# ElijahHyndman/PAPTeam_OpticalFlow

Measured on AMD Instinct MI355X. Metric: Mpix/s per frame-pair (fixed SOR iters) at 1920x1080; max-abs d(u,v) vs ref, higher is better.
Workload: dtype f64

## Files before the change

### papteam_opticalflow_amd/csrc/api.hip

```cpp
#include <algorithm>
#include <chrono>
#include <cmath>
#include <cstdio>
#include <cstdlib>
#include <cstring>
#include <mutex>
#include <random>
#include <thread>

#include "common.h"
#include "flow_internal.h"

namespace papof {

namespace {
thread_local std::string g_last_error;
}

void set_last_error(const char* what, hipError_t e, const char* file, int line) {
    char buf[512];
    std::snprintf(buf, sizeof buf, "%s failed: %s (%s:%d)", what, hipGetErrorString(e), file, line);
    g_last_error = buf;
}
const char* last_error() { return g_last_error.c_str(); }
void set_last_error_text(const std::string& text) { g_last_error = text; }

static double wall() {
    return std::chrono::duration<double>(std::chrono::steady_clock::now().time_since_epoch()).count();
}

size_t arena_bytes_for(int H, int W, int C, int levels, int n_sor_max, double ratio) {
    const size_t np = (size_t)H * W;
    const int fc = (C == 3) ? 5 : (C == 1 ? 3 : C);
    size_t per_level = 0;
    {
        std::vector<Level> L;
        std::vector<PyrPlan> plan;
        if (levels >= 1 && pyramid_plan(H, W, ratio, levels, L, plan) == PAPOF_OK)
            for (const Level& l : L) per_level += ((size_t)l.w * l.h * fc * sizeof(double) + 256) * 3;
    }
    size_t sor_cells = 0, sor_cells_d = 0;
    skew_capacity(H, W, n_sor_max, sor_cells, sor_cells_d);
    size_t planes = 0;
    planes += (size_t)2 * C * 5;
    if (levels > 8) planes += (size_t)2 * C * levels;
    planes += (size_t)2 * C + 2 * C;
    planes += (size_t)7 * fc;
    planes += 8;
    planes += (size_t)3 * C + C;
    planes += (size_t)3 * fc;
    size_t bytes = planes * np * sizeof(double);
    bytes += 3 * (sor_cells + 2 * kLanes) * 16 + (sor_cells_d + 2 * kLanes) * 16 + 10 * np * sizeof(double);
    bytes += per_level + np * fc * sizeof(double);
    bytes += 8 * (std::min<size_t>(kTinyMaxCells, np) * sizeof(double) + 256);
    bytes += (size_t)64 * 4096;
    return bytes;
}

static size_t sor_scratch_bytes(int H, int W, int n_sor) {
    size_t cells = 0, cells_d = 0;
    skew_capacity(H, W, n_sor, cells, cells_d);
    return 4 * (cells + 128) * 16 + (cells_d + 128) * 16;
}

int ensure_arena(papof_handle* h, size_t bytes) {
    if (bytes <= h->arena.cap) return PAPOF_OK;
    PAPOF_HIP(hipStreamSynchronize(h->stream));
    if (h->arena.base) PAPOF_HIP(hipFree(h->arena.base));
    h->arena.base = nullptr;
    h->arena.cap = 0;
    void* p = nullptr;
    hipError_t e = hipMalloc(&p, bytes);
    if (e != hipSuccess) {
        set_last_error("hipMalloc(arena)", e, __FILE__, __LINE__);
        return PAPOF_ENOMEM;
    }
    h->arena.base = static_cast<char*>(p);
    h->arena.cap = bytes;
    return PAPOF_OK;
}

int check_params(const papof_params& P, int levels) {
    if (levels < 1) return PAPOF_EINVAL;
    if (P.n_inner < 1) return PAPOF_EINVAL;
    if (P.n_outer + 0 < 1 || P.n_sor < 1 || P.n_outer_per_level < 0 || P.n_sor_per_level < 0) return PAPOF_EINVAL;
    if (P.sor_mode < PAPOF_SOR_EXACT || P.sor_mode > PAPOF_SOR_JACOBI) return PAPOF_EINVAL;
    if (!(P.alpha > 0) || !(P.omega > 0)) return PAPOF_EINVAL;
    if (P.interpolation != PAPOF_INTERP_BILINEAR && P.interpolation != PAPOF_INTERP_BICUBIC) return PAPOF_EINVAL;
    if (P.noise_model != PAPOF_NOISE_LAPLACIAN && P.noise_model != PAPOF_NOISE_GMIXTURE) return PAPOF_EINVAL;
    return PAPOF_OK;
}

int pyramid_plan(int H, int W, double ratio, int nlev, std::vector<Level>& L, std::vector<PyrPlan>& plan) {
    if (ratio > 0.98 || ratio < 0.4) ratio = 0.75;
    const double base_sigma = 1 / ratio - 1;
    const int n = (int)(std::log(0.25) / std::log(ratio));
    const double n_sigma = base_sigma * n;
    L.assign(nlev, Level{});
    plan.assign(nlev, PyrPlan{});
    L[0].w = W;
    L[0].h = H;
    for (int i = 1; i < nlev; i++) {
        PyrPlan p;
        if (i <= n) {
            p.src_level = 0;
            p.sigma = base_sigma * i;
            p.fsize = (int)(p.sigma * 3);
            p.rate = std::pow(ratio, i);
        } else {
            p.src_level = i - n;
            p.sigma = n_sigma;
            p.fsize = (int)(n_sigma * 3);
            p.rate = (double)std::pow(ratio, i) * W / L[i - n].w;
        }
        p.sw = L[p.src_level].w;
        p.sh = L[p.src_level].h;
        if (p.fsize > kMaxFsize) return PAPOF_EINVAL;
        L[i].w = (int)((double)p.sw * p.rate);
        L[i].h = (int)((double)p.sh * p.rate);
        if (L[i].w < 1 || L[i].h < 1) return PAPOF_EINVAL;
        plan[i] = p;
    }
    return PAPOF_OK;
}

int smooth_and_resize(papof_handle* h, const double* src, double* dst, double* tmp_a, double* tmp_b, const PyrPlan& p, int C,
                      int dh, int dw) {
    const Taps g = gaussian_taps(p.sigma, p.fsize);
    if (g.fsize == 0 && g.t[0] == 1.0) return resize(h, src, dst, p.sh, p.sw, C, dh, dw, p.rate, p.rate, false, 0.0);
    PAPOF_TRY(filter_hv(h, src, tmp_b, tmp_a, p.sh, p.sw, C, g, g));
    return resize(h, tmp_b, dst, p.sh, p.sw, C, dh, dw, p.rate, p.rate, false, 0.0);
}

int reduce_init(papof_handle* h, const papof_tensor* a, const papof_tensor* b, int pairs_a, int pairs_b, int H, int W,
                const std::vector<Level>& L, const std::vector<PyrPlan>& plan, double ratio, double* X, double* Y, double* T,
                size_t t_planes, double*& out) {
    const size_t np0 = (size_t)H * W;
    const int planes = 2 * (pairs_a + pairs_b), levels = (int)L.size();
    double* const parts[2] = {X, X + (size_t)pairs_a * 2 * np0};
    const papof_tensor* const src[2] = {a, b};
    const int n[2] = {pairs_a, pairs_b};
    for (int i = 0; i < 2; i++) {
        if (n[i] == 0) continue;
        if (src[i])
            PAPOF_TRY(ingest_frames(h, *src[i], nullptr, parts[i], H, W, 2, n[i]));
        else
            PAPOF_HIP(hipMemsetAsync(parts[i], 0, (size_t)n[i] * 2 * np0 * sizeof(double), h->stream));
    }
    PAPOF_TRY(init_sanitize(h, X, (size_t)planes * np0));
    out = X;
    if (levels == 1) return PAPOF_OK;
    std::vector<int> chain;
    for (int i = levels - 1; i > 0; i = plan[i].src_level) chain.insert(chain.begin(), i);
    double s = 1.0;
    for (int i = 1; i < levels; i++) s *= ratio;
    double *cur = X, *other = Y;
    for (const int i : chain) {
        const PyrPlan& p = plan[i];
        const bool last = i == levels - 1;
        const Taps g = gaussian_taps(p.sigma, p.fsize);
        if (g.fsize == 0 && g.t[0] == 1.0) {
            PAPOF_TRY(resize(h, cur, other, p.sh, p.sw, planes, L[i].h, L[i].w, p.rate, p.rate, last, last ? s : 0.0));
            std::swap(cur, other);
            continue;
        }
        const size_t ns = (size_t)p.sw * p.sh;
        const int chunk = filter_hv_needs_tmp(g, g) ? (int)std::min<size_t>((size_t)planes, t_planes * np0 / ns) : planes;
        if (chunk < 1) return PAPOF_EINVAL;
        for (int c0 = 0; c0 < planes; c0 += chunk)
            PAPOF_TRY(filter_hv(h, cur + c0 * ns, other + c0 * ns, T, p.sh, p.sw, std::min(chunk, planes - c0), g, g));
        PAPOF_TRY(resize(h, other, cur, p.sh, p.sw, planes, L[i].h, L[i].w, p.rate, p.rate, last, last ? s : 0.0));
    }
    out = cur;
    return PAPOF_OK;
}

int build_pyramid(papof_handle* h, const std::vector<Level>& L, const std::vector<PyrPlan>& plan, int C, bool second,
                  double* tmp_a, double* tmp_b) {
    for (size_t i = 1; i < L.size(); i++) {
        const PyrPlan& p = plan[i];
        const double* src = second ? L[p.src_level].p2 : L[p.src_level].p1;
        double* dst = second ? L[i].p2 : L[i].p1;
        PAPOF_TRY(smooth_and_resize(h, src, dst, tmp_a, tmp_b, p, C, L[i].h, L[i].w));
    }
    return PAPOF_OK;
}

struct SolveBuffers {
    double *im1s, *tmp, *blend, *imdt, *phi;
    SorPlanes sp;
    SorPlanes sp_tiny{};
    double *bgx = nullptr, *bgy = nullptr, *bgxy = nullptr;
    double *gm = nullptr, *gm_scratch = nullptr;
};

int alloc_solve_buffers(Arena& A, int H, int W, int fc, int mode, int n_sor_cap, SolveBuffers& B) {
    const size_t np = (size_t)H * W;
    B.im1s = A.f64(np * fc);
    B.tmp = A.f64(np * fc);
    B.blend = A.f64(np * fc);
    B.imdt = A.f64(np * fc);
    B.phi = A.f64(np);
    PAPOF_TRY(sor_alloc_planes(A, H, W, mode, n_sor_cap, B.sp));
    if (mode == PAPOF_SOR_EXACT)
        PAPOF_TRY(sor_alloc_tiny_planes(A, std::min<size_t>(kTinyMaxCells, (size_t)H * W), B.sp_tiny));
    return A.overflow ? PAPOF_ENOMEM : PAPOF_OK;
}

int alloc_branch_buffers(papof_handle* h, Arena& A, int H, int W, int fc, int interpolation, int noise_model,
                         SolveBuffers& B) {
    const size_t np = (size_t)H * W;
    if (interpolation == PAPOF_INTERP_BICUBIC) {
        B.bgx = A.f64(np * fc);
        B.bgy = A.f64(np * fc);
        B.bgxy = A.f64(np * fc);
    }
    if (noise_model == PAPOF_NOISE_GMIXTURE) {
        B.gm = A.f64(5 * 8);
        B.gm_scratch = A.f64((size_t)gm_scratch_doubles());
        if (A.overflow || fc > 8) return fc > 8 ? PAPOF_EINVAL : PAPOF_ENOMEM;
        double init[40];
        for (int k = 0; k < fc; k++) {
            init[k] = 0.95;
            init[fc + k] = 0.05;
            init[2 * fc + k] = 0.5;
            init[3 * fc + k] = 0.05 * 0.05;
            init[4 * fc + k] = 0.5 * 0.5;
        }
        PAPOF_HIP(hipMemcpyAsync(B.gm, init, sizeof(double) * 5 * fc, hipMemcpyHostToDevice, h->stream));
        PAPOF_HIP(hipStreamSynchronize(h->stream));
    }
    return A.overflow ? PAPOF_ENOMEM : PAPOF_OK;
}

int bicubic_planes(papof_handle* h, const double* f2, int H, int W, int fc, SolveBuffers& B) {
    PAPOF_TRY(central3_planes(h, f2, B.bgx, B.bgy, B.bgxy, H, W, fc));
    return PAPOF_OK;
}

struct LapGuard {
    bool on = false;
    bool exact = false;
    bool collect = false;
    bool nz_known = false;
    unsigned* flags = nullptr;
    double* lap = nullptr;
    double* scratch = nullptr;
    unsigned epoch = 0;
    int slot = 0;
    std::vector<int> slot_level, slot_channels;
    unsigned* wit(int s) const { return on && collect && s >= 0 && s < kLapMaxSlots ? flags + lap_wit_word(s) : nullptr; }
    unsigned* nz(int level) const { return on && collect && nz_known ? flags + lap_nz_word(level) : nullptr; }
    const double* guard() const { return on && exact ? lap : nullptr; }
    int unknown(const unsigned* host_flags) const {
        if (!on || !collect) return 0;
        if (slot > kLapMaxSlots) return 1;
        int n = 0;
        for (int s = 0; s + 1 < slot; s++)
            for (int c = 0; c < slot_channels[s]; c++) {
                const unsigned w = host_flags[lap_wit_word(s) + c];
                const bool witness = w == epoch || w == (epoch ^ kLapNone);
                const bool all_zero = nz_known && host_flags[lap_nz_word(slot_level[s]) + c] != epoch;
                n += !(witness || all_zero);
                if (!(witness || all_zero) && std::getenv("PAPOF_LAP_TRACE"))
                    std::fprintf(stderr, "[lap guard] no proof: slot %d of %d, level %d, channel %d\n", s, slot, slot_level[s], c);
            }
        return n;
    }
};

int smooth_flow(papof_handle* h, const double* f1, const double* f2, double* warp, double*& u, double*& v, double*& ua,
                double*& va, int H, int W, int fc, double alpha, int n_outer, int n_inner, int n_sor, double omega,
                int mode, SolveBuffers& B, PhaseClock& clk, const double* im1s_ready = nullptr,
                bool final_warp = true, unsigned* prog = nullptr, size_t prog_per_solve = 0, double* out_u = nullptr,
                double* out_v = nullptr, bool fold_warp = false, LapGuard* lg = nullptr, int level = 0) {
    const Taps g = smooth5_taps();
    int solve_idx = 0;
    const bool tiny = mode == PAPOF_SOR_EXACT && B.sp_tiny.phi && (size_t)H * W <= kTinyMaxCells && sor_tiny_fits(h, H, W, n_sor);
    SorPlanes& SP = tiny ? B.sp_tiny : B.sp;
    const double* im1s = im1s_ready;
    if (!im1s) {
        clk.phase(PAPOF_T_PHASE1_GENERATE);
        PAPOF_TRY(filter_hv(h, f1, B.im1s, B.tmp, H, W, fc, g, g));
        im1s = B.im1s;
    }
    const char* const fused_sw = std::getenv("PAPOF_FUSED_SYSTEM");
    const bool fused_env = !(fused_sw && fused_sw[0] == '0');
    const bool fused_system = fused_env && fold_warp && n_inner == 1 && !B.gm && (fc == 5 || fc == 3) &&
                              !(lg && lg->guard()) && !(lg && lg->on && lap_one_block_level(H, W));
    for (int count = 0; count < n_outer; count++) {
        clk.phase(fused_system ? kTimerFused : (int)PAPOF_T_PHASE1_GENERATE);
        if (fused_system)
            PAPOF_TRY(flow_system(h, f1, f2, u, v, im1s, H, W, fc, alpha, omega, SP,
                                  lg && count > 0 ? lg->wit(lg->slot - 1) : nullptr));
        else if (fold_warp)
            PAPOF_TRY(warp_smooth_blend(h, f1, f2, u, v, im1s, B.blend, B.imdt, H, W, fc,
                                        lg && count > 0 && !B.gm ? lg->wit(lg->slot - 1) : nullptr,
                                        B.phi));
        else
            PAPOF_TRY(smooth_hv_blend(h, warp, im1s, B.blend, B.imdt, H, W, fc));
        for (int hh = 0; hh < n_inner; hh++) {
            const SorPlanes* prev = hh == 0 ? nullptr : &SP;
            if ((count == 0 && !fold_warp) || hh > 0) {
                clk.phase(PAPOF_T_PHASE2_DERIVATIVES);
                PAPOF_TRY(compute_phi(h, u, v, prev, B.phi, H, W));
            }
            if (!fused_system) clk.phase(PAPOF_T_PHASE4_LINEARSYSTEM);
            if (!fused_system)
                PAPOF_TRY(assemble_system(h, B.blend, B.imdt, B.phi, u, v, H, W, fc, alpha, omega, SP, nullptr, nullptr,
                                          prev, nullptr, B.gm, lg ? lg->guard() : nullptr));
            h->sor_mark = [](void* c, int on) {
                static_cast<PhaseClock*>(c)->phase(on ? PAPOF_T_PHASE5_SOR : PAPOF_T_PHASE6_UPDATE);
            };
            h->sor_mark_ctx = &clk;
            h->sor_prog_next = prog ? prog + (size_t)solve_idx * prog_per_solve : nullptr;
            solve_idx++;
            const int rc_solve = sor_solve(h, SP, H, W, alpha, omega, n_sor, mode);
            h->sor_prog_next = nullptr;
            h->sor_mark = nullptr;
            h->sor_mark_ctx = nullptr;
            PAPOF_TRY(rc_solve);
        }
        double* const phi_next = count + 1 < n_outer && !fold_warp ? B.phi : nullptr;
        const bool rewarp = !fold_warp && !B.bgx && (final_warp || count + 1 < n_outer || B.gm);
        const bool wit_later = fold_warp && count + 1 < n_outer;
        const bool wit_small = fold_warp && !wit_later && lap_one_block_level(H, W);
        unsigned* const wit = lg && !B.gm && !B.bgx && !wit_later && !wit_small ? lg->wit(lg->slot) : nullptr;
        if (out_u && out_v && count + 1 == n_outer) {
            PAPOF_TRY(update_warp_phi(h, SP, u, v, out_u, out_v, f1, f2, warp, phi_next, H, W, fc, rewarp, 0, -1, wit));
            u = out_u;
            v = out_v;
        } else {
            PAPOF_TRY(update_warp_phi(h, SP, u, v, ua, va, f1, f2, warp, phi_next, H, W, fc, rewarp, 0, -1, wit));
            std::swap(u, ua);
            std::swap(v, va);
        }
        if (B.bgx)
            PAPOF_TRY(bicubic_warp(h, f1, f2, B.bgx, B.bgy, B.bgxy, u, v, warp, H, W, fc, nullptr, true, true));
        if (lg && lg->on && !B.gm && wit_small && lg->wit(lg->slot))
            PAPOF_TRY(lap_small_check(h, f1, f2, u, v, H, W, fc, lg->wit(lg->slot)));
        if (lg && lg->on && !B.gm) {
            lg->slot_level.push_back(level);
            lg->slot_channels.push_back(fc);
            lg->slot++;
            if (lg->exact) {
                if (B.bgx)
                    PAPOF_TRY(est_laplacian_noise(h, f1, warp, nullptr, nullptr, H, W, fc, lg->lap, lg->scratch));
                else
                    PAPOF_TRY(est_laplacian_noise(h, f1, f2, u, v, H, W, fc, lg->lap, lg->scratch));
            }
        }
        if (B.gm) PAPOF_TRY(est_gaussian_mixture(h, f1, warp, H, W, fc, B.gm, B.gm_scratch));
    }
    clk.phase(-1);
    return PAPOF_OK;
}

int feature_channels(int C) { return C == 3 ? 5 : (C == 1 ? 3 : C); }

struct FrameIn {
    const void* d;
    bool u8;
    bool planar = false;
};
int load_frame(papof_handle* h, const FrameIn& f, double* planar, int H, int W, int C) {
    if (f.planar) {
        PAPOF_HIP(hipMemcpyAsync(planar, f.d, (size_t)H * W * C * sizeof(double), hipMemcpyDeviceToDevice, h->stream));
        return PAPOF_OK;
    }
    if (f.u8) return hwc_u8_to_planar(h, static_cast<const unsigned char*>(f.d), planar, H, W, C);
    return hwc_to_planar(h, static_cast<const double*>(f.d), planar, H, W, C);
}

enum SeqOp { kPair, kSeqPrime, kSeqNext };

bool seq_matches(const papof_handle* h, int H, int W, int C, int levels, double ratio, size_t need) {
    const papof_handle::Seq& q = h->seq;
    return q.valid && q.h == H && q.w == W && q.c == C && q.levels == levels && q.ratio == ratio &&
           q.arena_base == h->arena.base && need <= h->arena.cap;
}

int flow_pass(papof_handle* h, const FrameIn& fa, const FrameIn& fb, SeqOp op, int H, int W, int C, int levels,
              const papof_params& P, double* d_vx, double* d_vy, double* d_warp, double* timing, LapGuard* lg,
              const papof_tensor* init = nullptr) {
    const double t_entry = wall();
    PAPOF_TRY(check_params(P, levels));
    double ratio = P.ratio;
    if (ratio > 0.98 || ratio < 0.4) ratio = 0.75;
    std::vector<Level> L;
    std::vector<PyrPlan> plan;
    PAPOF_TRY(pyramid_plan(H, W, P.ratio, levels, L, plan));
    const int n_sor_max = P.n_sor + (levels - 1) * P.n_sor_per_level;
    const size_t need = arena_bytes_for(H, W, C, levels, n_sor_max, P.ratio);
    if (op == kSeqNext && !seq_matches(h, H, W, C, levels, ratio, need)) {
        g_last_error = "sequence push does not continue the primed sequence (shape, levels, ratio or arena changed)";
        return PAPOF_EINVAL;
    }
    const int slot1 = op == kSeqNext ? h->seq.slot : 0;
    h->seq.valid = false;
    PAPOF_TRY(ensure_arena(h, need));
    Arena& A = h->arena;
    A.off = 0;
    A.overflow = false;
    h->events_used = 0;
    const size_t np0 = (size_t)H * W;
    const int fc = feature_channels(C);
    double tm[PAPOF_N_TIMERS + 1];
    std::memset(tm, 0, sizeof tm);
    const size_t tm_bytes = PAPOF_N_TIMERS * sizeof(double);
    const auto keep_seq = [&](int slot) {
        h->seq.valid = true;
        h->seq.h = H;
        h->seq.w = W;
        h->seq.c = C;
        h->seq.levels = levels;
        h->seq.ratio = ratio;
        h->seq.slot = slot;
        h->seq.arena_base = A.base;
    };
    PhaseClock clk{h, true};
    PhaseClock pclk{h, true};
    PhaseClock total{h, true};
    clk.only_sor = pclk.only_sor = (!h->phase_events && P.phase_timing == 0) || P.phase_timing == 2;
    h->sor_launches = 0;
    h->sor_log.clear();
    clk.stamps = true;
    h->stamps_used = 0;
    h->next_stamp = nullptr;
    h->stamp_stream = h->stream;

    total.phase(PAPOF_T_TOTAL);
    for (int i = 0; i < levels; i++) {
        double* slot[2];
        slot[0] = A.f64((size_t)L[i].w * L[i].h * C);
        slot[1] = A.f64((size_t)L[i].w * L[i].h * C);
        L[i].p1 = slot[slot1];
        L[i].p2 = slot[slot1 ^ 1];
    }
    double* tmp_a = A.f64(np0 * C);
    double* tmp_b = A.f64(np0 * C);
    if (A.overflow) return PAPOF_ENOMEM;
    if (op == kSeqPrime) {
        PAPOF_TRY(load_frame(h, fa, L[0].p1, H, W, C));
        PAPOF_TRY(build_pyramid(h, L, plan, C, false, tmp_a, tmp_b));
        PAPOF_HIP(hipStreamSynchronize(h->stream));
        keep_seq(slot1);
        if (timing) std::memset(timing, 0, tm_bytes);
        return PAPOF_OK;
    }

    std::vector<double*> F1(levels), F2(levels), S1(levels);
    for (int k = 0; k < levels; k++) {
        const size_t n = (size_t)L[k].w * L[k].h * fc;
        F1[k] = A.f64(n);
        F2[k] = A.f64(n);
        S1[k] = A.f64(n);
    }
    double* prep_tmp = A.f64(np0 * fc);
    double* gx = A.f64(np0 * C);
    double* gy = A.f64(np0 * C);
    double* gxy = A.f64(np0 * C);
    double* warp = A.f64(np0 * fc);
    double* u = A.f64(2 * np0);
    double* v = u ? u + np0 : nullptr;
    double* u2 = A.f64(2 * np0);
    double* v2 = u2 ? u2 + np0 : nullptr;
    SolveBuffers B;
    {
        const int rc_alloc = alloc_solve_buffers(A, H, W, fc, P.sor_mode, n_sor_max, B);
        if (rc_alloc != PAPOF_OK || A.overflow) return rc_alloc != PAPOF_OK ? rc_alloc : PAPOF_ENOMEM;
    }
    PAPOF_TRY(alloc_branch_buffers(h, A, H, W, fc, P.interpolation, P.noise_model, B));

    struct LevelCounters {
        size_t prog_off = 0, prog_per = 0;
    };
    std::vector<LevelCounters> LP(levels);
    size_t prog_total = 0;
    const bool exact = P.sor_mode == PAPOF_SOR_EXACT;
    if (exact) {
        for (int k = 0; k < levels; k++) {
            LP[k].prog_per = sor_counters_words(L[k].h, L[k].w, P.n_sor + k * P.n_sor_per_level);
            LP[k].prog_off = prog_total;
            prog_total += LP[k].prog_per * (size_t)((P.n_outer + k * P.n_outer_per_level) * P.n_inner);
        }
        PAPOF_TRY(sor_counters_ensure(h, prog_total));
    }

    const bool overlap = h->overlap_prep && P.phase_timing != 1 && h->prep_stream != nullptr;
    hipStream_t const main_stream = h->stream, prep = overlap ? h->prep_stream : h->stream;
    while (h->sync_events.size() < (size_t)levels + 2) {
        hipEvent_t e;
        PAPOF_HIP(hipEventCreateWithFlags(&e, hipEventDisableTiming));
        h->sync_events.push_back(e);
    }
    struct StreamSwap {
        papof_handle* h;
        hipStream_t saved;
        StreamSwap(papof_handle* hh, hipStream_t s) : h(hh), saved(hh->stream) { h->stream = s; }
        ~StreamSwap() { h->stream = saved; }
    };
    bool from_level0 = true;
    for (int i = 1; i < levels; i++) from_level0 = from_level0 && plan[i].src_level == 0;
    const Taps g5 = smooth5_taps();
    const auto build_level = [&](int i, int second) -> int {
        if (i == 0) return PAPOF_OK;
        const PyrPlan& q = plan[i];
        const double* src = second ? L[q.src_level].p2 : L[q.src_level].p1;
        double* dst = second ? L[i].p2 : L[i].p1;
        return smooth_and_resize(h, src, dst, tmp_a, tmp_b, q, C, L[i].h, L[i].w);
    };
    const auto prepare = [&]() -> int {
        StreamSwap on_prep(h, prep);
        pclk.phase(PAPOF_T_ALLOCATION);
        if (exact && !sor_counters_clear(h, 0, prog_total)) return PAPOF_EDEVICE;
        pclk.phase(PAPOF_T_CONSTRUCTION);
        if (op != kSeqNext) PAPOF_TRY(load_frame(h, fa, L[0].p1, H, W, C));
        PAPOF_TRY(load_frame(h, fb, L[0].p2, H, W, C));
        const int first = op == kSeqNext ? 1 : 0;
        if (!from_level0)
            for (int i = 1; i < levels; i++)
                for (int second = first; second < 2; second++) PAPOF_TRY(build_level(i, second));
        for (int k = levels - 1; k >= 0; k--) {
            if (from_level0) {
                pclk.phase(PAPOF_T_CONSTRUCTION);
                for (int second = first; second < 2; second++) PAPOF_TRY(build_level(k, second));
            }
            pclk.phase(PAPOF_T_ALLOCATION);
            PAPOF_TRY(im2feature(h, L[k].p1, F1[k], L[k].h, L[k].w, C, lg ? lg->nz(k) : nullptr));
            PAPOF_TRY(im2feature(h, L[k].p2, F2[k], L[k].h, L[k].w, C, lg ? lg->nz(k) : nullptr));
            pclk.phase(PAPOF_T_PHASE1_GENERATE);
            PAPOF_TRY(filter_hv(h, F1[k], S1[k], prep_tmp, L[k].h, L[k].w, fc, g5, g5));
            pclk.phase(-1);
            if (overlap) PAPOF_HIP(hipEventRecord(h->sync_events[k], prep));
        }
        pclk.phase(PAPOF_T_POSTPROCESSING);
        PAPOF_TRY(central3_planes(h, L[0].p2, gx, gy, gxy, H, W, C));
        pclk.phase(-1);
        if (overlap) PAPOF_HIP(hipEventRecord(h->sync_events[levels], prep));
        return PAPOF_OK;
    };
    papof_handle::HostIO& io = h->hostio;
    const bool hostio = io.active && overlap && h->copy_stream && h->copy_events.size() >= 8;
    const auto prepare_hostio = [&]() -> int {
        StreamSwap on_prep(h, prep);
        hipStream_t const cs = h->copy_stream;
        pclk.phase(PAPOF_T_ALLOCATION);
        if (exact && !sor_counters_clear(h, 0, prog_total)) return PAPOF_EDEVICE;
        if (io.im1) {
            PAPOF_HIP(hipMemcpyAsync(const_cast<void*>(fa.d), io.im1, io.nb_in, hipMemcpyHostToDevice, cs));
            PAPOF_HIP(hipEventRecord(h->copy_events[0], cs));
            PAPOF_HIP(hipStreamWaitEvent(prep, h->copy_events[0], 0));
        }
        pclk.phase(PAPOF_T_CONSTRUCTION);
        if (op != kSeqNext) {
            PAPOF_TRY(load_frame(h, fa, L[0].p1, H, W, C));
            for (int i = 1; i < levels; i++) PAPOF_TRY(build_level(i, 0));
        }
        for (int k = levels - 1; k >= 0; k--) {
            pclk.phase(PAPOF_T_ALLOCATION);
            PAPOF_TRY(im2feature(h, L[k].p1, F1[k], L[k].h, L[k].w, C, lg ? lg->nz(k) : nullptr));
            pclk.phase(PAPOF_T_PHASE1_GENERATE);
            PAPOF_TRY(filter_hv(h, F1[k], S1[k], prep_tmp, L[k].h, L[k].w, fc, g5, g5));
        }
        pclk.phase(-1);
        if (io.im2) {
            PAPOF_HIP(hipMemcpyAsync(const_cast<void*>(fb.d), io.im2, io.nb_in, hipMemcpyHostToDevice, cs));
            PAPOF_HIP(hipEventRecord(h->copy_events[1], cs));
            PAPOF_HIP(hipStreamWaitEvent(prep, h->copy_events[1], 0));
        }
        pclk.phase(PAPOF_T_CONSTRUCTION);
        PAPOF_TRY(load_frame(h, fb, L[0].p2, H, W, C));
        if (!from_level0)
            for (int i = 1; i < levels; i++) PAPOF_TRY(build_level(i, 1));
        for (int k = levels - 1; k >= 0; k--) {
            if (from_level0) {
                pclk.phase(PAPOF_T_CONSTRUCTION);
                PAPOF_TRY(build_level(k, 1));
            }
            pclk.phase(PAPOF_T_ALLOCATION);
            PAPOF_TRY(im2feature(h, L[k].p2, F2[k], L[k].h, L[k].w, C, lg ? lg->nz(k) : nullptr));
            pclk.phase(-1);
            PAPOF_HIP(hipEventRecord(h->sync_events[k], prep));
        }
        pclk.phase(PAPOF_T_POSTPROCESSING);
        PAPOF_TRY(central3_planes(h, L[0].p2, gx, gy, gxy, H, W, C));
        pclk.phase(-1);
        PAPOF_HIP(hipEventRecord(h->sync_events[levels], prep));
        return PAPOF_OK;
    };
    if (io.active && !hostio) {
        if (io.im1) PAPOF_HIP(hipMemcpyAsync(const_cast<void*>(fa.d), io.im1, io.nb_in, hipMemcpyHostToDevice, main_stream));
        if (io.im2) PAPOF_HIP(hipMemcpyAsync(const_cast<void*>(fb.d), io.im2, io.nb_in, hipMemcpyHostToDevice, main_stream));
    }
    if (overlap) {
        PAPOF_HIP(hipEventRecord(h->sync_events[levels + 1], main_stream));
        PAPOF_HIP(hipStreamWaitEvent(prep, h->sync_events[levels + 1], 0));
    }
    {
        const int rc = hostio ? prepare_hostio() : prepare();
        if (rc != PAPOF_OK) {
            if (overlap) hipStreamSynchronize(prep);
            return rc;
        }
    }

    int pw = 0, ph = 0;
    const auto solve_levels = [&]() -> int {
        if (lg && lg->guard())
            PAPOF_HIP(hipMemcpyAsync(lg->lap, h->lap_init_dev, 8 * sizeof(double), hipMemcpyDeviceToDevice, main_stream));
        for (int k = levels - 1; k >= 0; k--) {
            const int lw = L[k].w, lh = L[k].h;
            const size_t np = (size_t)lw * lh;
            clk.phase(-1);
            if (overlap) PAPOF_HIP(hipStreamWaitEvent(main_stream, h->sync_events[k], 0));
            clk.phase(PAPOF_T_ALLOCATION);
            const double *f1 = F1[k], *f2 = F2[k];
            const int n_sor_k = P.n_sor + k * P.n_sor_per_level, n_outer_k = P.n_outer + k * P.n_outer_per_level;
            unsigned* prog_k = nullptr;
            if (exact) prog_k = h->sync_words + 32 + LP[k].prog_off;
            const bool tiny_k = exact && (size_t)lw * lh <= kTinyMaxCells && sor_tiny_fits(h, lh, lw, n_sor_k);
            if (!tiny_k) PAPOF_TRY(sor_bind(h, B.sp, lh, lw, n_sor_k));
            double* const out_u = k == 0 ? d_vx : nullptr;
            double* const out_v = k == 0 ? d_vy : nullptr;
            const bool fold_warp = !B.bgx && !B.gm;
            if (k == levels - 1 && init) {
                double* r = nullptr;
                PAPOF_TRY(reduce_init(h, init, nullptr, 1, 0, H, W, L, plan, ratio, u, u2, warp, (size_t)fc, r));
                if (r != u) std::swap(u, u2);
                v = u + np;
                v2 = u2 + np;
                if (B.bgx) {
                    PAPOF_TRY(bicubic_planes(h, f2, lh, lw, fc, B));
                    PAPOF_TRY(bicubic_warp(h, f1, f2, B.bgx, B.bgy, B.bgxy, u, v, warp, lh, lw, fc, nullptr, true, false));
                } else if (!fold_warp) {
                    PAPOF_TRY(warp_bilinear(h, f1, f2, u, v, warp, lh, lw, fc));
                }
            } else if (k == levels - 1) {
                v = u + np;
                v2 = u2 + np;
                PAPOF_HIP(hipMemsetAsync(u, 0, 2 * np * sizeof(double), h->stream));
                if (!fold_warp)
                    PAPOF_HIP(hipMemcpyAsync(warp, f2, np * fc * sizeof(double), hipMemcpyDeviceToDevice, h->stream));
                if (B.bgx) PAPOF_TRY(bicubic_planes(h, f2, lh, lw, fc, B));
            } else {
                const double xr = (double)lw / pw, yr = (double)lh / ph, inv = 1 / ratio;
                PAPOF_TRY(resize(h, u, u2, ph, pw, 2, lh, lw, xr, yr, true, inv));
                std::swap(u, u2);
                v = u + np;
                v2 = u2 + np;
                if (B.bgx) {
                    PAPOF_TRY(bicubic_planes(h, f2, lh, lw, fc, B));
                    PAPOF_TRY(bicubic_warp(h, f1, f2, B.bgx, B.bgy, B.bgxy, u, v, warp, lh, lw, fc, nullptr, true, false));
                } else if (!fold_warp) {
                    PAPOF_TRY(warp_bilinear(h, f1, f2, u, v, warp, lh, lw, fc));
                }
            }
            if (!tiny_k) PAPOF_TRY(sor_reset_planes(h, B.sp));
            PAPOF_TRY(smooth_flow(h, f1, f2, warp, u, v, u2, v2, lh, lw, fc, P.alpha, n_outer_k, P.n_inner, n_sor_k, P.omega,
                                  P.sor_mode, B, clk, S1[k], false, prog_k, exact ? LP[k].prog_per : 0, out_u, out_v,
                                  fold_warp, lg, k));
            pw = lw;
            ph = lh;
        }
        clk.phase(-1);
        if (overlap) PAPOF_HIP(hipStreamWaitEvent(main_stream, h->sync_events[levels], 0));
        clk.phase(PAPOF_T_POSTPROCESSING);
        if (hostio && io.early_out && u == d_vx && v == d_vy) {
            hipStream_t const cs = h->copy_stream;
            PAPOF_HIP(hipEventRecord(h->copy_events[2], main_stream));
            PAPOF_HIP(hipStreamWaitEvent(cs, h->copy_events[2], 0));
            PAPOF_HIP(hipMemcpyAsync(io.vx, d_vx, io.nb_flow, hipMemcpyDeviceToHost, cs));
            PAPOF_HIP(hipMemcpyAsync(io.vy, d_vy, io.nb_flow, hipMemcpyDeviceToHost, cs));
            constexpr int kChunks = 4;
            for (int q = 0; q < kChunks; q++) {
                const Rect rc{0, (int)((long long)H * q / kChunks), W, (int)((long long)H * (q + 1) / kChunks)};
                if (rc.empty()) continue;
                PAPOF_TRY(bicubic_warp(h, L[0].p1, L[0].p2, gx, gy, gxy, u, v, d_warp, H, W, C, &rc));
                PAPOF_HIP(hipEventRecord(h->copy_events[3 + q], main_stream));
                PAPOF_HIP(hipStreamWaitEvent(cs, h->copy_events[3 + q], 0));
                const size_t off = (size_t)rc.y0 * W * C, cnt = (size_t)rc.h() * W * C;
                PAPOF_HIP(hipMemcpyAsync(io.warp + off, d_warp + off, cnt * sizeof(double), hipMemcpyDeviceToHost, cs));
            }
            io.out_issued = true;
            return PAPOF_OK;
        }
        PAPOF_TRY(bicubic_warp(h, L[0].p1, L[0].p2, gx, gy, gxy, u, v, d_warp, H, W, C));
        if (u != d_vx) PAPOF_HIP(hipMemcpyAsync(d_vx, u, np0 * sizeof(double), hipMemcpyDeviceToDevice, h->stream));
        if (v != d_vy) PAPOF_HIP(hipMemcpyAsync(d_vy, v, np0 * sizeof(double), hipMemcpyDeviceToDevice, h->stream));
        return PAPOF_OK;
    };
    const int rc_main = solve_levels();
    if (rc_main != PAPOF_OK) {
        hipStreamSynchronize(main_stream);
        if (overlap) hipStreamSynchronize(prep);
        return rc_main;
    }
    clk.phase(-1);
    PAPOF_TRY(stamp_only(h));
    total.phase(-1);
    h->stamps_fetched = 0;
    {
        const bool flags = lg && lg->on && lg->collect;
        const size_t first = flags ? lap_wit_word(std::min(lg->slot, kLapMaxSlots) - 1) : kLapFlagWords;
        const size_t bytes = (kLapFlagWords - first) * sizeof(unsigned) + (size_t)h->stamps_used * sizeof(unsigned long long);
        if (bytes > 0)
            PAPOF_HIP(hipMemcpyAsync(h->lap_flags_host + first, h->lap_flags_dev + first, bytes, hipMemcpyDeviceToHost, h->stream));
        h->stamps_fetched = h->stamps_used;
    }
    const double t_enqueued = wall();
    PAPOF_HIP(hipStreamSynchronize(h->stream));
    h->host_enqueue_sec = t_enqueued - t_entry;
    h->host_wait_sec = wall() - t_enqueued;
    h->next_stamp = nullptr;
    if (P.sor_mode == PAPOF_SOR_EXACT) PAPOF_TRY(sor_check(h));
    if (clk.err != PAPOF_OK || pclk.err != PAPOF_OK || total.err != PAPOF_OK) return PAPOF_EDEVICE;
    clk.collect(tm);
    pclk.collect(tm);
    total.collect(tm);
    if (clk.sor_span_sec.size() == h->sor_log.size())
        for (size_t i = 0; i < h->sor_log.size(); i++) h->sor_log[i].sec = clk.sor_span_sec[i];
    {
        constexpr double kPsiShare = 0.3;
        const double fused = tm[PAPOF_T_PHASE4_LINEARSYSTEM];
        tm[PAPOF_T_PHASE3_PSIDATA] += kPsiShare * fused;
        tm[PAPOF_T_PHASE4_LINEARSYSTEM] = fused - kPsiShare * fused;
    }
    {
        constexpr double kPhiShare = 0.04;
        const double fused = tm[PAPOF_T_PHASE1_GENERATE];
        tm[PAPOF_T_PHASE2_DERIVATIVES] += kPhiShare * fused;
        tm[PAPOF_T_PHASE1_GENERATE] = fused - kPhiShare * fused;
    }
    {
        const double f = tm[kTimerFused];
        tm[PAPOF_T_PHASE1_GENERATE] += 0.51 * f;
        tm[PAPOF_T_PHASE2_DERIVATIVES] += 0.02 * f;
        tm[PAPOF_T_PHASE3_PSIDATA] += 0.14 * f;
        tm[PAPOF_T_PHASE4_LINEARSYSTEM] += f - 0.51 * f - 0.02 * f - 0.14 * f;
    }
    if (timing) std::memcpy(timing, tm, tm_bytes);
    if (op == kSeqNext) keep_seq(slot1 ^ 1);
    return PAPOF_OK;
}

int flow_device(papof_handle* h, const FrameIn& fa, const FrameIn& fb, SeqOp op, int H, int W, int C, int levels,
                const papof_params& P, double* d_vx, double* d_vy, double* d_warp, double* timing,
                const papof_tensor* init = nullptr) {
    LapGuard lg;
    const int fc = feature_channels(C);
    lg.on = h->lap_guard && op != kSeqPrime && P.noise_model == PAPOF_NOISE_LAPLACIAN && fc <= 8 && levels >= 1 &&
            h->lap_flags_dev != nullptr;
    if (!lg.on) return flow_pass(h, fa, fb, op, H, W, C, levels, P, d_vx, d_vy, d_warp, timing, nullptr, init);
    lg.flags = h->lap_flags_dev;
    lg.lap = h->lap_dev;
    lg.scratch = h->lap_scratch_dev;
    lg.nz_known = (C == 1 || C == 3) && (size_t)levels * 8 <= (size_t)kLapNzWords;
    const bool always_exact = P.interpolation == PAPOF_INTERP_BICUBIC;
    lg.collect = !always_exact;
    lg.exact = always_exact || h->lap_exact;
    const papof_handle::Seq seq0 = h->seq;
    double first_pass_total = 0.0;
    for (int pass = 0; pass < 2; pass++) {
        if (++h->lap_epoch >= kLapNone) {
            PAPOF_HIP(hipMemsetAsync(h->lap_flags_dev, 0, kLapFlagWords * sizeof(unsigned), h->stream));
            h->lap_epoch = 1u;
        }
        lg.epoch = h->lap_epoch;
        lg.slot = 0;
        lg.slot_level.clear();
        lg.slot_channels.clear();
        PAPOF_TRY(flow_pass(h, fa, fb, op, H, W, C, levels, P, d_vx, d_vy, d_warp, timing, &lg, init));
        if (pass == 1 && timing) timing[PAPOF_T_TOTAL] += first_pass_total;
        if (!lg.collect) return PAPOF_OK;
        const int unknown = lg.unknown(h->lap_flags_host);
        if (lg.exact) {
            if (pass == 0) h->lap_exact_calls++;
            h->lap_exact = unknown > 0;
            return PAPOF_OK;
        }
        if (unknown == 0) return PAPOF_OK;
        h->lap_reruns++;
        lg.exact = true;
        if (timing) first_pass_total = timing[PAPOF_T_TOTAL];
        if (h->copy_stream) PAPOF_HIP(hipStreamSynchronize(h->copy_stream));
        h->seq = seq0;
        h->hostio.im1 = nullptr;
        h->hostio.im2 = nullptr;
    }
    return PAPOF_OK;
}

int flow_device_planar(papof_handle* h, const double* f1, const double* f2, int H, int W, int C, int levels,
                       const papof_params& P, double* d_vx, double* d_vy, double* d_warp, double* timing,
                       const papof_tensor* init) {
    FrameIn a{f1, false}, b{f2, false};
    a.planar = b.planar = true;
    return flow_device(h, a, b, kPair, H, W, C, levels, P, d_vx, d_vy, d_warp, timing, init);
}

}

using namespace papof;

extern "C" {

int papof_version(void) { return PAPOF_VERSION; }

void papof_default_params(papof_params* p) {
    if (!p) return;
    p->alpha = 0.012;
    p->ratio = 0.75;
    p->n_outer = 7;
    p->n_outer_per_level = 1;
    p->n_inner = 1;
    p->n_sor = 30;
    p->n_sor_per_level = 3;
    p->omega = 1.8;
    p->sor_mode = PAPOF_SOR_EXACT;
    p->phase_timing = 0;
    p->interpolation = PAPOF_INTERP_BILINEAR;
    p->noise_model = PAPOF_NOISE_LAPLACIAN;
}

const char* papof_strerror(int code) {
    switch (code) {
        case PAPOF_OK: return "ok";
        case PAPOF_EINVAL: return "invalid argument";
        case PAPOF_ENODEVICE: return "no usable gfx950 device";
        case PAPOF_ENOMEM: return "out of memory";
        case PAPOF_EDEVICE: return "HIP runtime error";
        case PAPOF_ETIMEOUT: return "device-side wait timed out";
    }
    return "unknown error";
}

const char* papof_last_error(void) { return last_error(); }

const char* papof_timing_key(int i) {
    static const char* keys[PAPOF_N_TIMERS] = {"Allocation",         "Construction",        "Phase1_Generate",
                                               "Phase2_Derivatives", "Phase3_PsiData",      "Phase4_LinearSystem",
                                               "Phase5_SOR",         "Phase6_Update",       "PostProcessing",
                                               "Total C++ Execution"};
    return (i >= 0 && i < PAPOF_N_TIMERS) ? keys[i] : "";
}
// ... 637 lines not shown
    PAPOF_TRY(S.down_planar(sp.b1, rhs1, height, width, 1));
    return S.down_planar(sp.b2, rhs2, height, width, 1);
}

int papof_stage_laplacian(papof_handle* h, const double* in, const double* weight, int height, int width,
                          double* out) {
    if (!h || !in || !weight || !out || height < 1 || width < 1) return PAPOF_EINVAL;
    Scope S(h, img_bytes(height, width, 1, 6));
    PAPOF_TRY(S.rc);
    double* a = S.up_planar(in, height, width, 1);
    double* w = S.up_planar(weight, height, width, 1);
    double* o = S.dev((size_t)height * width);
    PAPOF_TRY(S.rc);
    PAPOF_TRY(laplacian(h, a, w, o, height, width));
    return S.down_planar(o, out, height, width, 1);
}

namespace {
int alloc_sor_planes(Scope& S, int H, int W, int mode, int n_sor, SorPlanes& sp) {
    if (mode == PAPOF_SOR_EXACT && (size_t)H * W <= kTinyMaxCells && sor_tiny_fits(S.h, H, W, n_sor)) {
        const int rc_t = sor_alloc_tiny_planes(S.h->arena, (size_t)H * W, sp);
        if (rc_t != PAPOF_OK) S.rc = rc_t;
        return S.rc;
    }
    int rc = sor_alloc_planes(S.h->arena, H, W, mode, n_sor, sp);
    if (rc == PAPOF_OK) rc = sor_bind(S.h, sp, H, W, n_sor);
    if (rc != PAPOF_OK) S.rc = rc;
    return S.rc;
}
}

int papof_stage_sor(papof_handle* h, const double* phi, const double* imdxy, const double* imdx2,
                    const double* imdy2, const double* rhs1, const double* rhs2, int height, int width,
                    double alpha, double omega, int n_sor, int sor_mode, double* du, double* dv) {
    if (!h || !phi || !imdxy || !imdx2 || !imdy2 || !rhs1 || !rhs2 || !du || !dv || height < 1 || width < 1 ||
        n_sor < 1 || sor_mode < PAPOF_SOR_EXACT || sor_mode > PAPOF_SOR_JACOBI)
        return PAPOF_EINVAL;
    const size_t np = (size_t)height * width;
    Scope S(h, img_bytes(height, width, 1, 16) + sor_scratch_bytes(height, width, n_sor) +
                   12 * (size_t)height * width * sizeof(double));
    PAPOF_TRY(S.rc);
    double* p = S.up_planar(phi, height, width, 1);
    double* xy = S.up_planar(imdxy, height, width, 1);
    double* x2 = S.up_planar(imdx2, height, width, 1);
    double* y2 = S.up_planar(imdy2, height, width, 1);
    double* r1 = S.up_planar(rhs1, height, width, 1);
    double* r2 = S.up_planar(rhs2, height, width, 1);
    double *ou = S.dev(np), *ov = S.dev(np);
    SorPlanes sp{};
    PAPOF_TRY(alloc_sor_planes(S, height, width, sor_mode, n_sor, sp));
    PAPOF_TRY(sor_reset_planes(h, sp));
    PAPOF_TRY(sor_prep(h, p, xy, x2, y2, r1, r2, height, width, alpha, omega, sp));
    PAPOF_TRY(sor_solve(h, sp, height, width, alpha, omega, n_sor, sor_mode));
    PAPOF_TRY(sor_unpack(h, sp, ou, ov, height, width));
    PAPOF_TRY(S.down_planar(ou, du, height, width, 1));
    PAPOF_TRY(S.down_planar(ov, dv, height, width, 1));
    if (sor_mode == PAPOF_SOR_EXACT) PAPOF_TRY(sor_check(h));
    return PAPOF_OK;
}

int papof_stage_smoothflow(papof_handle* h, const double* im1, const double* im2, double* warp, double* u,
                           double* v, int height, int width, int c, double alpha, int n_outer, int n_inner,
                           int n_sor, double omega, int sor_mode) {
    return papof_stage_smoothflow_ex(h, im1, im2, warp, u, v, height, width, c, alpha, n_outer, n_inner, n_sor, omega,
                                     sor_mode, PAPOF_INTERP_BILINEAR, PAPOF_NOISE_LAPLACIAN, nullptr);
}

int papof_stage_smoothflow_ex(papof_handle* h, const double* im1, const double* im2, double* warp, double* u,
                              double* v, int height, int width, int c, double alpha, int n_outer, int n_inner,
                              int n_sor, double omega, int sor_mode, int interpolation, int noise_model, double* gm) {
    if (!h || !im1 || !im2 || !warp || !u || !v || height < 1 || width < 1 || c < 1 || n_outer < 1 || n_sor < 1 ||
        sor_mode < PAPOF_SOR_EXACT || sor_mode > PAPOF_SOR_JACOBI)
        return PAPOF_EINVAL;
    if (n_inner < 1) return PAPOF_EINVAL;
    if (interpolation < 0 || interpolation > 1 || noise_model < 0 || noise_model > 1) return PAPOF_EINVAL;
    Scope S(h, img_bytes(height, width, c, 16) + img_bytes(height, width, 1, 8) +
                   sor_scratch_bytes(height, width, n_sor) +
                   12 * (size_t)height * width * sizeof(double) + (1 << 20));
    PAPOF_TRY(S.rc);
    double* f1 = S.up_planar(im1, height, width, c);
    double* f2 = S.up_planar(im2, height, width, c);
    double* w = S.up_planar(warp, height, width, c);
    double* du = S.up_planar(u, height, width, 1);
    double* dv = S.up_planar(v, height, width, 1);
    double* du_alt = S.dev((size_t)height * width);
    double* dv_alt = S.dev((size_t)height * width);
    PAPOF_TRY(S.rc);
    SolveBuffers B;
    PAPOF_TRY(alloc_solve_buffers(h->arena, height, width, c, sor_mode, n_sor, B));
    PAPOF_TRY(alloc_branch_buffers(h, h->arena, height, width, c, interpolation, noise_model, B));
    if (B.gm && gm) PAPOF_HIP(hipMemcpyAsync(B.gm, gm, sizeof(double) * 5 * c, hipMemcpyHostToDevice, h->stream));
    if (B.bgx) PAPOF_TRY(bicubic_planes(h, f2, height, width, c, B));
    PAPOF_TRY(sor_bind(h, B.sp, height, width, n_sor));
    PAPOF_TRY(sor_reset_planes(h, B.sp));
    PhaseClock clk{h, false};
    LapGuard lg;
    lg.on = h->lap_guard && noise_model == PAPOF_NOISE_LAPLACIAN && c <= 8 && h->lap_dev != nullptr;
    lg.exact = true;
    lg.lap = h->lap_dev;
    lg.scratch = h->lap_scratch_dev;
    if (lg.on) PAPOF_HIP(hipMemcpyAsync(lg.lap, h->lap_init_dev, 8 * sizeof(double), hipMemcpyDeviceToDevice, h->stream));
    PAPOF_TRY(smooth_flow(h, f1, f2, w, du, dv, du_alt, dv_alt, height, width, c, alpha, n_outer, n_inner, n_sor, omega,
                          sor_mode, B, clk, nullptr, true, nullptr, 0, nullptr, nullptr, false, &lg, 0));
    PAPOF_TRY(S.down_planar(w, warp, height, width, c));
    PAPOF_TRY(S.down_planar(du, u, height, width, 1));
    PAPOF_TRY(S.down_planar(dv, v, height, width, 1));
    if (B.gm && gm) {
        PAPOF_HIP(hipMemcpyAsync(gm, B.gm, sizeof(double) * 5 * c, hipMemcpyDeviceToHost, h->stream));
        PAPOF_HIP(hipStreamSynchronize(h->stream));
    }
    if (sor_mode == PAPOF_SOR_EXACT) PAPOF_TRY(sor_check(h));
    return PAPOF_OK;
}

int papof_stage_est_gaussian_mixture(papof_handle* h, const double* im1, const double* im2, int height, int width,
                                     int c, double* gm) {
    if (!h || !im1 || !im2 || !gm || height < 1 || width < 1 || c < 1 || c > 8) return PAPOF_EINVAL;
    Scope S(h, img_bytes(height, width, c, 6) + (1 << 20));
    PAPOF_TRY(S.rc);
    double* a = S.up_planar(im1, height, width, c);
    double* b = S.up_planar(im2, height, width, c);
    double* g = S.dev(40);
    double* scratch = S.dev((size_t)gm_scratch_doubles());
    PAPOF_TRY(S.rc);
    PAPOF_HIP(hipMemcpyAsync(g, gm, sizeof(double) * 5 * c, hipMemcpyHostToDevice, h->stream));
    PAPOF_TRY(est_gaussian_mixture(h, a, b, height, width, c, g, scratch));
    PAPOF_HIP(hipMemcpyAsync(gm, g, sizeof(double) * 5 * c, hipMemcpyDeviceToHost, h->stream));
    PAPOF_HIP(hipStreamSynchronize(h->stream));
    return PAPOF_OK;
}

int papof_pyramid_levels_for_min_width(int width, double ratio, int min_width, int* levels) {
    if (width < 1 || min_width < 1 || !levels) return PAPOF_EINVAL;
    if (ratio > 0.98 || ratio < 0.4) ratio = 0.75;
    *levels = (int)(std::log((double)min_width / width) / std::log(ratio));
    return PAPOF_OK;
}

int papof_stage_bicubic_warp(papof_handle* h, const double* im1, const double* im2, const double* vx,
                             const double* vy, int height, int width, int c, double* out) {
    return papof_stage_bicubic_warp_ex(h, im1, im2, vx, vy, height, width, c, 1, out);
}

int papof_stage_bicubic_warp_ex(papof_handle* h, const double* im1, const double* im2, const double* vx,
                                const double* vy, int height, int width, int c, int clamp, double* out) {
    if (!h || !im1 || !im2 || !vx || !vy || !out || height < 1 || width < 1 || c < 1) return PAPOF_EINVAL;
    Scope S(h, img_bytes(height, width, c, 10) + img_bytes(height, width, 1, 4));
    PAPOF_TRY(S.rc);
    const size_t n = (size_t)height * width * c;
    double* a = S.up_planar(im1, height, width, c);
    double* b = S.up_planar(im2, height, width, c);
    double* fx = S.up_planar(vx, height, width, 1);
    double* fy = S.up_planar(vy, height, width, 1);
    double *gx = S.dev(n), *gy = S.dev(n), *gxy = S.dev(n), *o = S.dev(n);
    PAPOF_TRY(S.rc);
    PAPOF_TRY(central3_planes(h, b, gx, gy, gxy, height, width, c));
    PAPOF_TRY(bicubic_warp(h, a, b, gx, gy, gxy, fx, fy, o, height, width, c, nullptr, false, clamp != 0));
    PAPOF_HIP(hipMemcpyAsync(out, o, n * sizeof(double), hipMemcpyDeviceToHost, h->stream));
    PAPOF_HIP(hipStreamSynchronize(h->stream));
    return PAPOF_OK;
}

int papof_flow_quantize16(papof_handle* h, const double* vx, const double* vy, int height, int width,
                          unsigned short* out) {
    if (!h || !vx || !vy || !out || height < 1 || width < 1) return PAPOF_EINVAL;
    const size_t n = (size_t)height * width;
    Scope S(h, n * (2 * sizeof(double) + 2 * sizeof(unsigned short)) + 4096);
    PAPOF_TRY(S.rc);
    double* a = S.up_planar(vx, height, width, 1);
    double* b = S.up_planar(vy, height, width, 1);
    unsigned short* q = reinterpret_cast<unsigned short*>(S.dev((n * 2 * sizeof(unsigned short) + 7) / 8));
    PAPOF_TRY(S.rc);
    PAPOF_TRY(flow_quantize16(h, a, b, q, n));
    PAPOF_HIP(hipMemcpyAsync(out, q, n * 2 * sizeof(unsigned short), hipMemcpyDeviceToHost, h->stream));
    PAPOF_HIP(hipStreamSynchronize(h->stream));
    return PAPOF_OK;
}

int papof_flow_dequantize16(papof_handle* h, const unsigned short* q, int height, int width, double* vx,
                            double* vy) {
    if (!h || !q || !vx || !vy || height < 1 || width < 1) return PAPOF_EINVAL;
    const size_t n = (size_t)height * width;
    Scope S(h, n * (2 * sizeof(double) + 2 * sizeof(unsigned short)) + 4096);
    PAPOF_TRY(S.rc);
    unsigned short* dq = reinterpret_cast<unsigned short*>(S.dev((n * 2 * sizeof(unsigned short) + 7) / 8));
    double* a = S.dev(n);
    double* b = S.dev(n);
    PAPOF_TRY(S.rc);
    PAPOF_HIP(hipMemcpyAsync(dq, q, n * 2 * sizeof(unsigned short), hipMemcpyHostToDevice, h->stream));
    PAPOF_TRY(flow_dequantize16(h, dq, a, b, n));
    PAPOF_HIP(hipMemcpyAsync(vx, a, n * sizeof(double), hipMemcpyDeviceToHost, h->stream));
    PAPOF_HIP(hipMemcpyAsync(vy, b, n * sizeof(double), hipMemcpyDeviceToHost, h->stream));
    PAPOF_HIP(hipStreamSynchronize(h->stream));
    return PAPOF_OK;
}

int papof_flow_to_bgr(papof_handle* h, const double* vx, const double* vy, int height, int width,
                      unsigned char* bgr) {
    if (!h || !vx || !vy || !bgr || height < 1 || width < 1) return PAPOF_EINVAL;
    const size_t n = (size_t)height * width;
    Scope S(h, n * (2 * sizeof(double) + 3) + 16384);
    PAPOF_TRY(S.rc);
    double* a = S.up_planar(vx, height, width, 1);
    double* b = S.up_planar(vy, height, width, 1);
    double* partial = S.dev(512);
    unsigned char* out = reinterpret_cast<unsigned char*>(S.dev((n * 3 + 7) / 8));
    PAPOF_TRY(S.rc);
    PAPOF_TRY(flow_to_bgr(h, a, b, n, partial, out));
    PAPOF_HIP(hipMemcpyAsync(bgr, out, n * 3, hipMemcpyDeviceToHost, h->stream));
    PAPOF_HIP(hipStreamSynchronize(h->stream));
    return PAPOF_OK;
}

int papof_sor_plan(papof_handle* h, int height, int width, int n_sor, int sor_mode, int* launches, int* depth) {
    return sor_plan(h, height, width, n_sor, sor_mode, launches, depth);
}

int papof_last_sor_stats(papof_handle* h, int* launches, double* strip_streams_sec) {
    if (!h) return PAPOF_EINVAL;
    if (launches) *launches = h->sor_launches;
    if (strip_streams_sec) *strip_streams_sec = 0.0;
    return PAPOF_OK;
}

int papof_lap_guard_stats(papof_handle* h, int out[4]) {
    if (!h || !out) return PAPOF_EINVAL;
    out[0] = h->lap_reruns;
    out[1] = h->lap_exact_calls;
    out[2] = h->lap_exact ? 1 : 0;
    out[3] = h->lap_guard ? 1 : 0;
    return PAPOF_OK;
}

int papof_last_host_times(papof_handle* h, double out[3]) {
    if (!h || !out) return PAPOF_EINVAL;
    out[0] = h->host_enqueue_sec;
    out[1] = h->host_wait_sec;
    out[2] = 0.0;
    return PAPOF_OK;
}

int papof_last_sor_solves(papof_handle* h, int cap, int* n, int* info, double* sec) {
    if (!h || !n) return PAPOF_EINVAL;
    *n = (int)h->sor_log.size();
    for (int i = 0; i < *n && i < cap; i++) {
        const papof_handle::SorSolveLog& e = h->sor_log[i];
        if (info) {
            int* o = info + (size_t)i * 6;
            o[0] = e.H;
            o[1] = e.W;
            o[2] = e.n_sor;
            o[3] = e.kind;
            o[4] = e.depth;
            o[5] = e.launches;
        }
        if (sec) sec[i] = e.sec;
    }
    return PAPOF_OK;
}

int papof_test_sor_strips(papof_handle* h, int height, int width, int n_sor, int split_band, int reps, int delay_us,
                          long long* mismatches, int* bands) {
    if (!h || !mismatches) return PAPOF_EINVAL;
    const size_t np = (size_t)height * width;
    Scope S(h, img_bytes(height, width, 1, 16) + sor_scratch_bytes(height, width, n_sor) +
                   12 * (size_t)height * width * sizeof(double));
    PAPOF_TRY(S.rc);
    std::vector<double> host(np * 6);
    std::mt19937_64 rng(2);
    auto fill = [&](size_t k, double lo, double hi) {
        std::uniform_real_distribution<double> d(lo, hi);
        for (size_t i = 0; i < np; i++) host[k * np + i] = d(rng);
    };
    fill(0, 0.5, 50.0);
    fill(1, -0.02, 0.02);
    fill(2, 0.0, 0.05);
    fill(3, 0.0, 0.05);
    fill(4, -0.01, 0.01);
    fill(5, -0.01, 0.01);
    double* planes[6];
    for (int k = 0; k < 6; k++) planes[k] = S.up_planar(host.data() + k * np, height, width, 1);
    SorPlanes sp{};
    PAPOF_TRY(alloc_sor_planes(S, height, width, PAPOF_SOR_EXACT, n_sor, sp));
    PAPOF_TRY(sor_reset_planes(h, sp));
    PAPOF_TRY(sor_prep(h, planes[0], planes[1], planes[2], planes[3], planes[4], planes[5], height, width, 0.012, 1.8, sp));
    if (bands) *bands = sp.sd.nb;
    const size_t cells = sp.sd.nd;
    std::vector<double> want(cells * 2), got(cells * 2);
    PAPOF_TRY(sor_solve(h, sp, height, width, 0.012, 1.8, n_sor, PAPOF_SOR_EXACT));
    PAPOF_HIP(hipStreamSynchronize(h->stream));
    PAPOF_TRY(sor_check(h));
    PAPOF_HIP(hipMemcpy(want.data(), sp.du, cells * 16, hipMemcpyDeviceToHost));
    *mismatches = 0;
    if (!sor_strips_supported(h, sp, n_sor) || split_band < 1 || split_band >= sp.sd.nb) return PAPOF_EINVAL;
    struct Owned {
        hipStream_t top = nullptr;
        hipEvent_t ev = nullptr;
        ~Owned() {
            if (top) {
                hipStreamSynchronize(top);
                hipStreamDestroy(top);
            }
            if (ev) hipEventDestroy(ev);
        }
    } own;
    PAPOF_HIP(hipStreamCreateWithFlags(&own.top, hipStreamNonBlocking));
    PAPOF_HIP(hipEventCreateWithFlags(&own.ev, hipEventDisableTiming));
    hipStream_t const main_stream = h->stream, top = own.top;
    hipEvent_t const ev = own.ev;
// ... 125 lines not shown
```

### papteam_opticalflow_amd/csrc/batch.hip

```cpp
#include <algorithm>
#include <chrono>
#include <cmath>
#include <cstring>

#include "common.h"
#include "flow_internal.h"

namespace papof {

namespace {

double now_sec() { return std::chrono::duration<double>(std::chrono::steady_clock::now().time_since_epoch()).count(); }

struct BatchOut {
    const double* uv = nullptr;
    const double* warp = nullptr;
    std::vector<int> unproven;
};

struct BatchFrames {
    const void* const* host = nullptr;
    bool u8 = false;
    const papof_tensor* a = nullptr;
    const papof_tensor* b = nullptr;
    const papof_tensor* init_fw = nullptr;
    const papof_tensor* init_bw = nullptr;
};

bool batch_applies(const papof_handle* h, int B, int H, int W, int C, int levels, const papof_params& P) {
    if (B < 2 || !h->use_dpp) return false;
    if (P.sor_mode != PAPOF_SOR_EXACT || P.n_inner != 1 || P.interpolation != PAPOF_INTERP_BILINEAR ||
        P.noise_model != PAPOF_NOISE_LAPLACIAN)
        return false;
    if (C != 1 && C != 3) return false;
    const int n_sor_max = P.n_sor + (levels - 1) * P.n_sor_per_level;
    if (skew_dims(H, W, n_sor_max, 1, 1).nb >= 16) return false;
    long slots = 0;
    for (int k = 0; k < levels; k++) slots += P.n_outer + (long)k * P.n_outer_per_level;
    return slots <= kLapMaxSlots;
}

int batch_max(int H, int W, int C, int levels, const papof_params& P) {
    const int nb0 = skew_dims(H, W, P.n_sor + (levels - 1) * P.n_sor_per_level, 1, 1).nb;
    const size_t per_pair = arena_bytes_for(H, W, C, levels, P.n_sor + (levels - 1) * P.n_sor_per_level, P.ratio);
    int max_b = (int)std::max<size_t>(2, std::min<size_t>((size_t)1024 / (size_t)nb0, ((size_t)24 << 30) / per_pair));
    if (const char* e = std::getenv("PAPOF_BATCH_MAX")) max_b = std::max(2, std::min(max_b, std::atoi(e)));
    return max_b;
}

int flow_batch_device(papof_handle* h, int B, int sequence, bool with_bw, const BatchFrames& frames, int H, int W, int C, int levels,
                      const papof_params& P, double* timing, BatchOut& out) {
    PAPOF_TRY(check_params(P, levels));
    double ratio = P.ratio;
    if (ratio > 0.98 || ratio < 0.4) ratio = 0.75;
    std::vector<Level> L;
    std::vector<PyrPlan> plan;
    PAPOF_TRY(pyramid_plan(H, W, P.ratio, levels, L, plan));
    const int fstep = sequence ? 1 : 2, nF = sequence ? B + 1 : 2 * B;
    const int NP = with_bw ? 2 * B : B;
    const int fc = feature_channels(C);
    const size_t np0 = (size_t)H * W;
    const int n_sor_max = P.n_sor + (levels - 1) * P.n_sor_per_level;
    const bool guard = h->lap_guard && h->lap_flags_dev != nullptr;
    const bool u8 = frames.u8, staged = frames.host != nullptr;
    size_t pyr_px = 0;
    for (const Level& l : L) pyr_px += (size_t)l.w * l.h;
    size_t cells = 0, cells_d = 0;
    skew_capacity(H, W, n_sor_max, cells, cells_d);
    const size_t tiny_cells = std::min<size_t>(kTinyMaxCells, np0);
    size_t bytes = 0;
    if (staged) bytes += (size_t)nF * np0 * C * (u8 ? 1 : 8) + 4096;
    bytes += (size_t)nF * pyr_px * (C + 2 * fc) * 8 + (size_t)levels * 3 * 4096;
    bytes += (size_t)nF * np0 * C * 8 * 5 + 5 * 4096;
    bytes += (size_t)NP * (4 * np0 * 8 + np0 * C * 8) + 3 * 4096;
    bytes += (size_t)NP * ((3 * 2 * ((cells + kLanes + 63) / 64 * 64) + 2 * (cells_d + kLanes)) * 8 + 2 * 4096);
    bytes += (size_t)NP * (8 * (tiny_cells * 8 + 256));
    bytes += (size_t)(NP + nF) * kLapFlagWords * 4 + 8192;
    bytes += (size_t)1 << 20;
    h->seq.valid = false;
    PAPOF_TRY(ensure_arena(h, bytes));
    Arena& A = h->arena;
    A.off = 0;
    A.overflow = false;
    h->events_used = 0;
    h->sor_log.clear();
    h->sor_launches = 0;
    hipStream_t const st = h->stream;

    unsigned char* stage = staged ? static_cast<unsigned char*>(A.alloc((size_t)nF * np0 * C * (u8 ? 1 : 8))) : nullptr;
    std::vector<double*> Lp(levels), F(levels), S(levels);
    for (int k = 0; k < levels; k++) {
        const size_t n = (size_t)L[k].w * L[k].h;
        Lp[k] = A.f64((size_t)nF * n * C);
        F[k] = A.f64((size_t)nF * n * fc);
        S[k] = A.f64((size_t)nF * n * fc);
    }
    double* tmp_a = A.f64((size_t)nF * np0 * C);
    double* tmp_b = A.f64((size_t)nF * np0 * C);
    double* gx = A.f64((size_t)nF * np0 * C);
    double* gy = A.f64((size_t)nF * np0 * C);
    double* gxy = A.f64((size_t)nF * np0 * C);
    double* uvA = A.f64((size_t)NP * 2 * np0);
    double* uvB = A.f64((size_t)NP * 2 * np0);
    double* warp = A.f64((size_t)NP * np0 * C);
    unsigned* wit = reinterpret_cast<unsigned*>(A.alloc((size_t)NP * kLapFlagWords * sizeof(unsigned)));
    unsigned* nzf = reinterpret_cast<unsigned*>(A.alloc((size_t)nF * kLapNzWords * sizeof(unsigned)));
    if (A.overflow) return PAPOF_ENOMEM;
    std::vector<SorPlanes> SP(NP), ST(NP);
    for (int p = 0; p < NP; p++) PAPOF_TRY(sor_alloc_planes(A, H, W, PAPOF_SOR_EXACT, n_sor_max, SP[p]));
    for (int p = 0; p < NP; p++) PAPOF_TRY(sor_alloc_tiny_planes(A, tiny_cells, ST[p]));
    if (A.overflow) return PAPOF_ENOMEM;
    const size_t sp_stride = (size_t)(SP[1].phi - SP[0].phi), spd_stride = (size_t)(SP[1].du - SP[0].du);
    const size_t st_stride = (size_t)(ST[1].phi - ST[0].phi);
    for (int p = 1; p < NP; p++)
        if ((size_t)(SP[p].phi - SP[0].phi) != p * sp_stride || (size_t)(SP[p].du - SP[0].du) != p * spd_stride ||
            (size_t)(ST[p].phi - ST[0].phi) != p * st_stride || (size_t)(ST[p].du - ST[0].du) != p * st_stride)
            return PAPOF_EDEVICE;

    struct LevelCounters {
        size_t off, per;
        bool tiny;
    };
    std::vector<LevelCounters> LC(levels);
    size_t prog_total = 0;
    for (int k = 0; k < levels; k++) {
        const int Kk = P.n_sor + k * P.n_sor_per_level, n_outer = P.n_outer + k * P.n_outer_per_level;
        LC[k].tiny = (size_t)L[k].w * L[k].h <= kTinyMaxCells && sor_tiny_fits(h, L[k].h, L[k].w, Kk);
        LC[k].per = LC[k].tiny ? 0 : (size_t)skew_dims(L[k].h, L[k].w, Kk, 1, 1).nb * Kk * 32;
        LC[k].off = prog_total;
        prog_total += LC[k].per * (size_t)n_outer * NP;
    }
    PAPOF_TRY(sor_counters_ensure(h, prog_total));

    PhaseClock total{h, true}, sorclk{h, true};
    sorclk.only_sor = true;
    double tm[PAPOF_N_TIMERS + 1];
    std::memset(tm, 0, sizeof tm);
    total.phase(PAPOF_T_TOTAL);

    const size_t frame_bytes = np0 * C * (u8 ? 1 : 8);
    if (staged) {
        const void* const* hf = frames.host;
        bool flat_in = true;
        for (int f = 1; f < nF && flat_in; f++)
            flat_in = (const unsigned char*)hf[f] == (const unsigned char*)hf[0] + (size_t)f * frame_bytes;
        if (flat_in) {
            PAPOF_HIP(hipMemcpyAsync(stage, hf[0], (size_t)nF * frame_bytes, hipMemcpyHostToDevice, st));
        } else {
            for (int f = 0; f < nF; f++)
                PAPOF_HIP(hipMemcpyAsync(stage + (size_t)f * frame_bytes, hf[f], frame_bytes, hipMemcpyHostToDevice, st));
        }
    }
    if (prog_total && !sor_counters_clear(h, 0, prog_total)) return PAPOF_EDEVICE;
    if (++h->lap_epoch >= kLapNone) {
        if (h->lap_flags_dev) PAPOF_HIP(hipMemsetAsync(h->lap_flags_dev, 0, kLapFlagWords * sizeof(unsigned), st));
        h->lap_epoch = 1u;
    }
    const unsigned epoch = h->lap_epoch;
    if (guard) {
        PAPOF_HIP(hipMemsetAsync(wit, 0, (size_t)NP * kLapFlagWords * sizeof(unsigned), st));
        PAPOF_HIP(hipMemsetAsync(nzf, 0, (size_t)nF * kLapNzWords * sizeof(unsigned), st));
    }
    if (!staged)
        PAPOF_TRY(ingest_frames(h, *frames.a, sequence ? nullptr : frames.b, Lp[0], H, W, C, nF));
    else if (u8)
        PAPOF_TRY(hwc_u8_to_planar(h, stage, Lp[0], H, W, C, nF));
    else
        PAPOF_TRY(hwc_to_planar(h, reinterpret_cast<const double*>(stage), Lp[0], H, W, C, nF));
    for (int i = 1; i < levels; i++)
        PAPOF_TRY(smooth_and_resize(h, Lp[plan[i].src_level], Lp[i], tmp_a, tmp_b, plan[i], C * nF, L[i].h, L[i].w));
    const Taps g5 = smooth5_taps();
    const bool nz_known = guard && (size_t)levels * 8 <= (size_t)kLapNzWords;
    for (int k = 0; k < levels; k++) {
        PAPOF_TRY(im2feature(h, Lp[k], F[k], L[k].h, L[k].w, C, nz_known ? nzf + (size_t)k * 8 : nullptr, nF, kLapNzWords));
        PAPOF_TRY(filter_hv(h, F[k], S[k], nullptr, L[k].h, L[k].w, fc * nF, g5, g5));
    }
    PAPOF_TRY(central3_planes(h, Lp[0], gx, gy, gxy, H, W, C * nF));

    double *uv = uvA, *uv2 = uvB;
    int pw = 0, ph = 0, slot = 0;
    std::vector<int> slot_level;
    h->sor_mark = [](void* c, int on) { static_cast<PhaseClock*>(c)->phase(on ? PAPOF_T_PHASE5_SOR : -1); };
    h->sor_mark_ctx = &sorclk;
    const auto levels_loop = [&]() -> int {
        for (int k = levels - 1; k >= 0; k--) {
            const int lw = L[k].w, lh = L[k].h;
            const size_t np = (size_t)lw * lh;
            const int K = P.n_sor + k * P.n_sor_per_level, n_outer = P.n_outer + k * P.n_outer_per_level;
            if (k == levels - 1 && (frames.init_fw || frames.init_bw)) {
                double* r = nullptr;
                PAPOF_TRY(reduce_init(h, frames.init_fw, frames.init_bw, B, with_bw ? B : 0, H, W, L, plan, ratio, uvB, uvA, warp,
                                      (size_t)NP * C, r));
                if (r != uv) std::swap(uv, uv2);
            } else if (k == levels - 1) {
                PAPOF_HIP(hipMemsetAsync(uv, 0, (size_t)NP * 2 * np * sizeof(double), st));
            } else {
                PAPOF_TRY(resize(h, uv, uv2, ph, pw, 2 * NP, lh, lw, (double)lw / pw, (double)lh / ph, true, 1 / ratio));
                std::swap(uv, uv2);
            }
            const bool tiny = LC[k].tiny;
            SorPlanes sp = tiny ? ST[0] : SP[0];
            if (!tiny) {
                PAPOF_TRY(sor_bind_plain(h, sp, lh, lw, K));
                PAPOF_TRY(sor_reset_planes_batch(h, sp, NP, sp_stride));
            }
            BatchK bk{};
            bk.im = (size_t)fstep * np * fc;
            bk.uv = 2 * np;
            bk.sp = tiny ? st_stride : sp_stride;
            bk.d = tiny ? st_stride : spd_stride;
            bk.wit = kLapFlagWords;
            bk.bw = with_bw ? B : 0;
            bk.fr = np * fc;
            const SorBatch bt{NP, sp_stride, spd_stride, LC[k].per, st_stride};
            const double *f1 = F[k], *f2 = F[k] + np * fc, *s1 = S[k];
            const bool exhaustive = guard && np <= 4096;
            for (int count = 0; count < n_outer; count++) {
                unsigned* const w_prev = guard && !exhaustive && count > 0 ? wit + lap_wit_word(slot - 1) : nullptr;
                PAPOF_TRY(flow_system(h, f1, f2, uv, uv + np, s1, lh, lw, fc, P.alpha, P.omega, sp, w_prev, 0, -1, NP, &bk));
                h->sor_prog_next = tiny ? nullptr : h->sync_words + 32 + LC[k].off + (size_t)count * LC[k].per * NP;
                const int rc = sor_solve(h, sp, lh, lw, P.alpha, P.omega, K, PAPOF_SOR_EXACT, &bt);
                h->sor_prog_next = nullptr;
                PAPOF_TRY(rc);
                unsigned* const w_now = guard && !exhaustive && count + 1 == n_outer ? wit + lap_wit_word(slot) : nullptr;
                PAPOF_TRY(update_warp_phi(h, sp, uv, uv + np, uv2, uv2 + np, f1, f2, nullptr, nullptr, lh, lw, fc, false, 0, -1,
                                          w_now, NP, &bk));
                std::swap(uv, uv2);
                if (exhaustive) PAPOF_TRY(lap_small_check(h, f1, f2, uv, uv + np, lh, lw, fc, wit + lap_wit_word(slot), NP, &bk));
                slot_level.push_back(k);
                slot++;
            }
            pw = lw;
            ph = lh;
        }
        BatchK bk{};
        bk.im = (size_t)fstep * np0 * C;
        bk.uv = 2 * np0;
        bk.out = np0 * C;
        bk.bw = with_bw ? B : 0;
        bk.fr = np0 * C;
        PAPOF_TRY(bicubic_warp(h, Lp[0], Lp[0] + np0 * C, gx + np0 * C, gy + np0 * C, gxy + np0 * C, uv, uv + np0, warp, H, W, C,
                               nullptr, false, true, NP, &bk));
        return PAPOF_OK;
    };
    const int rc_levels = levels_loop();
    h->sor_mark = nullptr;
    h->sor_mark_ctx = nullptr;
    total.phase(-1);
    if (rc_levels != PAPOF_OK) {
        hipStreamSynchronize(st);
        return rc_levels;
    }
    std::vector<unsigned> hw, hn;
    PAPOF_HIP(hipStreamSynchronize(st));
    PAPOF_TRY(sor_check(h));
    if (guard) {
        hw.resize((size_t)NP * kLapFlagWords);
        hn.resize((size_t)nF * kLapNzWords);
        PAPOF_HIP(hipMemcpy(hw.data(), wit, hw.size() * sizeof(unsigned), hipMemcpyDeviceToHost));
        PAPOF_HIP(hipMemcpy(hn.data(), nzf, hn.size() * sizeof(unsigned), hipMemcpyDeviceToHost));
        for (int p = 0; p < NP; p++) {
            bool open = true;
            const bool back = p >= B;
            const int f1 = (back ? p - B : p) * fstep, fa = back ? f1 + 1 : f1, fb = back ? f1 : f1 + 1;
            for (int s = 0; s + 1 < slot && open; s++)
                for (int c = 0; c < fc; c++) {
                    const unsigned w = hw[(size_t)p * kLapFlagWords + lap_wit_word(s) + c];
                    const bool witness = w == epoch || w == (epoch ^ kLapNone);
                    const size_t nzw = (size_t)slot_level[s] * 8 + c;
                    const bool all_zero = nz_known && hn[(size_t)fa * kLapNzWords + nzw] != epoch &&
                                          hn[(size_t)fb * kLapNzWords + nzw] != epoch;
                    if (!(witness || all_zero)) open = false;
                }
            if (!open) out.unproven.push_back(p);
        }
    }
    if (total.err != PAPOF_OK || sorclk.err != PAPOF_OK) return PAPOF_EDEVICE;
    sorclk.collect(tm);
    total.collect(tm);
    if (timing) std::memcpy(timing, tm, PAPOF_N_TIMERS * sizeof(double));
    out.uv = uv;
    out.warp = warp;
    return PAPOF_OK;
}

}

int flow_batch_host(papof_handle* h, int n_pairs, int sequence, const void* const* frames, bool u8, int H, int W, int C, int levels,
                    const papof_params* params, double* const* vx, double* const* vy, double* const* warpI2, double* timing_sec) {
    if (!h || n_pairs < 1 || !frames || !vx || !vy || !warpI2 || H < 1 || W < 1 || C < 1 || levels < 1) return PAPOF_EINVAL;
    const int nF = sequence ? n_pairs + 1 : 2 * n_pairs;
    for (int f = 0; f < nF; f++)
        if (!frames[f]) return PAPOF_EINVAL;
    for (int p = 0; p < n_pairs; p++)
        if (!vx[p] || !vy[p] || !warpI2[p]) return PAPOF_EINVAL;
    papof_params P;
    if (params)
        P = *params;
    else
        papof_default_params(&P);
    PAPOF_TRY(check_params(P, levels));
    PAPOF_HIP(hipSetDevice(h->device));
    const double t0 = now_sec();
    double tm[PAPOF_N_TIMERS];
    std::memset(tm, 0, sizeof tm);
    const auto single = [&](int p) -> int {
        const void* a = frames[sequence ? p : 2 * p];
        const void* b = frames[sequence ? p + 1 : 2 * p + 1];
        double t1[PAPOF_N_TIMERS];
        const int rc = u8 ? papof_flow_u8(h, (const unsigned char*)a, (const unsigned char*)b, H, W, C, levels, &P, vx[p], vy[p],
                                          warpI2[p], t1)
                          : papof_flow(h, (const double*)a, (const double*)b, H, W, C, levels, &P, vx[p], vy[p], warpI2[p], t1);
        if (rc == PAPOF_OK)
            for (int i = 0; i < PAPOF_N_TIMERS; i++) tm[i] += t1[i];
        return rc;
    };
    if (!batch_applies(h, n_pairs, H, W, C, levels, P)) {
        for (int p = 0; p < n_pairs; p++) PAPOF_TRY(single(p));
        if (timing_sec) std::memcpy(timing_sec, tm, sizeof tm);
        return PAPOF_OK;
    }
    {
        const int max_b = batch_max(H, W, C, levels, P);
        if (n_pairs > max_b) {
            const int step = sequence ? 1 : 2;
            for (int p0 = 0; p0 < n_pairs;) {
                int nb_ = std::min(max_b, n_pairs - p0);
                if (n_pairs - (p0 + nb_) == 1 && nb_ > 2) nb_ -= 1;
                double t1[PAPOF_N_TIMERS];
                PAPOF_TRY(flow_batch_host(h, nb_, sequence, frames + (size_t)p0 * step, u8, H, W, C, levels, &P, vx + p0, vy + p0,
                                          warpI2 + p0, t1));
                for (int i = 0; i < PAPOF_N_TIMERS; i++) tm[i] += t1[i];
                p0 += nb_;
            }
            if (timing_sec) std::memcpy(timing_sec, tm, sizeof tm);
            return PAPOF_OK;
        }
    }
    BatchOut out;
    {
        BatchFrames bf;
        bf.host = frames;
        bf.u8 = u8;
        const int rc = flow_batch_device(h, n_pairs, sequence, false, bf, H, W, C, levels, P, tm, out);
        if (rc == PAPOF_ENOMEM) {
            std::memset(tm, 0, sizeof tm);
            for (int p = 0; p < n_pairs; p++) PAPOF_TRY(single(p));
            if (timing_sec) std::memcpy(timing_sec, tm, sizeof tm);
            return PAPOF_OK;
        }
        PAPOF_TRY(rc);
    }
    const size_t np0 = (size_t)H * W;
    bool flat = true;
    for (int p = 0; p < n_pairs && flat; p++)
        flat = vx[p] == vx[0] + (size_t)p * 2 * np0 && vy[p] == vx[p] + np0 && warpI2[p] == warpI2[0] + (size_t)p * np0 * C;
    if (flat) {
        PAPOF_HIP(hipMemcpyAsync(vx[0], out.uv, (size_t)n_pairs * 2 * np0 * sizeof(double), hipMemcpyDeviceToHost, h->stream));
        PAPOF_HIP(hipMemcpyAsync(warpI2[0], out.warp, (size_t)n_pairs * np0 * C * sizeof(double), hipMemcpyDeviceToHost, h->stream));
    } else {
        for (int p = 0; p < n_pairs; p++) {
            PAPOF_HIP(hipMemcpyAsync(vx[p], out.uv + (size_t)p * 2 * np0, np0 * sizeof(double), hipMemcpyDeviceToHost, h->stream));
            PAPOF_HIP(hipMemcpyAsync(vy[p], out.uv + (size_t)p * 2 * np0 + np0, np0 * sizeof(double), hipMemcpyDeviceToHost,
                                     h->stream));
            PAPOF_HIP(hipMemcpyAsync(warpI2[p], out.warp + (size_t)p * np0 * C, np0 * C * sizeof(double), hipMemcpyDeviceToHost,
                                     h->stream));
        }
    }
    PAPOF_HIP(hipStreamSynchronize(h->stream));
    for (int p : out.unproven) {
        h->lap_reruns++;
        PAPOF_TRY(single(p));
    }
    tm[PAPOF_T_TOTAL] = now_sec() - t0;
    if (timing_sec) std::memcpy(timing_sec, tm, sizeof tm);
    return PAPOF_OK;
}

namespace {

papof_tensor shifted(const papof_tensor& t, long long items) {
    papof_tensor r = t;
    r.data = static_cast<char*>(t.data) + items * t.stride[0] * dtype_bytes(t.dtype);
    return r;
}

const std::initializer_list<int> kAxes = {0, 1, 2, 3}, kFloat = {PAPOF_DTYPE_F32, PAPOF_DTYPE_F64};
bool valid_frames(const papof_tensor* t) {
    return described(t, {PAPOF_DTYPE_U8, PAPOF_DTYPE_F32, PAPOF_DTYPE_F64}, kAxes, false);
}
bool valid_output(const papof_tensor* t) { return described(t, kFloat, kAxes, true); }

struct TensorOut {
    const papof_tensor* flow = nullptr;
    const papof_tensor* warp = nullptr;
// ... 280 lines not shown
```

### papteam_opticalflow_amd/csrc/common.h

```cpp
#pragma once
#include <cstdlib>

#include <hip/hip_runtime.h>

#include <algorithm>
#include <cmath>
#include <cstddef>
#include <cstdint>
#include <initializer_list>
#include <string>
#include <vector>

#include "../../include/papof.h"

namespace papof {

constexpr int kLanes = 64;
constexpr int kMaxFsize = 8;

struct Rect {
    int x0, y0, x1, y1;
    __host__ __device__ bool empty() const { return x1 <= x0 || y1 <= y0; }
    __host__ __device__ int w() const { return x1 - x0; }
    __host__ __device__ int h() const { return y1 - y0; }
// ... 100 lines not shown
        d.nb = (h + 2 * last + 1 + kFusedRows - 1) / kFusedRows;
        d.qt = n_sor + 3;
        d.rt = (d.qt + 7) / 8 * 8;
        d.hp = (d.rt + kFusedRows * d.nb + 4 + 7) / 8 * 8;
        d.npos = d.qt + d.ns + 2 * kSorMaxDepth + 2 + kFusedRows * (d.nb - 1) + 2;
        d.dpar = last & 1;
        d.koff = 2 * last + 1;
        d.poff = 3;
        d.nh = 0;
    } else {
        d.band_rows = kBandRows;
        d.nb = (h + n_sor - 1 + kBandRows - 1) / kBandRows;
        d.qt = n_sor + 1;
        d.rt = (d.qt + 7) / 8 * 8;
        d.hp = (d.rt + kBandRows * d.nb + 2 + 7) / 8 * 8;
        d.npos = d.qt + d.ns + 2 * kSorMaxDepth + 2 + kBandRows * (d.nb - 1) + 2;
        d.dpar = d.group == 1 ? ((n_sor - 1) & 1) : (((n_sor + d.group - 1) / d.group - 1) & 1);
        d.koff = n_sor - 1;
        d.poff = 1;
        d.nh = d.group == 1 ? 0 : (size_t)n_sor * d.nb * d.npos_d;
    }
    d.n = (size_t)d.npos * d.hp;
    d.nd = (size_t)2 * d.npos_d * d.nb * kLanes;
    return d;
}
inline void skew_capacity(int h, int w, int n_sor, size_t& cells, size_t& cells_d) {
    const SkewDims a = skew_dims(h, w, n_sor, 2), b = skew_dims(h, w, n_sor, 1, 2);
    cells = a.n > b.n ? a.n : b.n;
    cells_d = (a.nd + a.nh) > (b.nd + b.nh) ? (a.nd + a.nh) : (b.nd + b.nh);
}

struct SorPlanes {
    double *phi, *xy, *a1, *a2, *b1, *b2;
    double *du, *dv;
    double *du2, *dv2;
    bool skew;
    SkewDims sd;
    size_t cap_cells, cap_cells_d;
};

}

struct papof_handle {
    int device = 0;
    hipStream_t stream = nullptr;
    papof::Arena arena;
    unsigned* sync_words = nullptr;
    size_t sync_cap = 0;
    std::vector<hipEvent_t> events;
    size_t events_used = 0;
    int cu_count = 0;
    double* stage_dev = nullptr;
    size_t stage_dev_bytes = 0;
    double* tensor_scratch = nullptr;
    size_t tensor_scratch_bytes = 0;
    hipEvent_t entry_event = nullptr;
    unsigned* init_flag_dev = nullptr;
    bool use_dpp = false;
    int sor_depth = 0;
    unsigned long long* sor_dbg = nullptr;
    void (*sor_mark)(void*, int) = nullptr;
    void* sor_mark_ctx = nullptr;
    int sor_fuse = 0;
    int sor_group = 0;
    int rb_depth = 0;
    int rb_shape = 0;
    int rb_naive = 0;
    int sor_resident = 0;
    int sor_skip_dead = 1;
    unsigned* sor_prog_next = nullptr;
    int sor_launches = 0;
    struct SorSolveLog {
        int H, W, n_sor, kind, depth, launches;
        double sec;
    };
    std::vector<SorSolveLog> sor_log;
    hipStream_t prep_stream = nullptr;
    unsigned* lap_flags_dev = nullptr;
    unsigned* lap_flags_host = nullptr;
    double* lap_dev = nullptr;
    double* lap_init_dev = nullptr;
    double* lap_scratch_dev = nullptr;
    bool lap_guard = true;
    bool lap_exact = false;
    unsigned lap_epoch = 0;
    int lap_reruns = 0, lap_exact_calls = 0;
    double host_enqueue_sec = 0.0, host_wait_sec = 0.0;
    struct HostIO {
        bool active = false;
        const void *im1 = nullptr, *im2 = nullptr;
        size_t nb_in = 0;
        double *vx = nullptr, *vy = nullptr, *warp = nullptr;
        size_t nb_flow = 0, nb_img = 0;
        bool early_out = false;
        bool out_issued = false;
    } hostio;
    hipStream_t copy_stream = nullptr;
    std::vector<hipEvent_t> copy_events;
    std::vector<hipEvent_t> sync_events;
    bool overlap_prep = true;
    unsigned long long* stamps_dev = nullptr;
    unsigned long long* stamps = nullptr;
    int stamps_cap = 0, stamps_used = 0, stamps_fetched = 0;
    unsigned long long* next_stamp = nullptr;
    hipStream_t stamp_stream = nullptr;
    bool phase_events = true;
    int sor_xcd_affine = 1;
    struct Seq {
        bool valid = false;
        int h = 0, w = 0, c = 0, levels = 0, slot = 0;
        double ratio = 0;
        const char* arena_base = nullptr;
    } seq;
};

namespace papof {

inline unsigned long long* take_stamp(papof_handle* h) {
    if (h->stamp_stream && h->stream != h->stamp_stream) return nullptr;
    unsigned long long* s = h->next_stamp;
    h->next_stamp = nullptr;
    return s;
}
int stamp_only(papof_handle* h);

inline bool described(const papof_tensor* t, std::initializer_list<int> dtypes, std::initializer_list<int> axes, bool positive) {
    if (!t || !t->data || std::find(dtypes.begin(), dtypes.end(), t->dtype) == dtypes.end()) return false;
    for (int i : axes)
        if (t->stride[i] < 0 || (positive && t->stride[i] == 0)) return false;
    return true;
}
inline bool valid_alphas(double a1, double a2) { return std::isfinite(a1) && std::isfinite(a2) && a1 >= 0 && a2 >= 0; }
inline long long dtype_bytes(int dtype) { return dtype == PAPOF_DTYPE_U8 ? 1 : dtype == PAPOF_DTYPE_F32 ? 4 : 8; }

int hwc_to_planar(papof_handle* h, const double* hwc, double* planar, int H, int W, int C, int frames = 1);
int hwc_u8_to_planar(papof_handle* h, const unsigned char* hwc, double* planar, int H, int W, int C, int frames = 1);
int planar_to_hwc(papof_handle* h, const double* planar, double* hwc, int H, int W, int C);
int ingest_frames(papof_handle* h, const papof_tensor& a, const papof_tensor* b, double* planar, int H, int W, int C,
                  int frames);
int emit_outputs(papof_handle* h, const double* src, const papof_tensor& dst, bool comp_major, int H, int W, int K, int pairs);
int init_check(papof_handle* h, const papof_tensor& t, int pairs, int H, int W, unsigned* flag);
int init_sanitize(papof_handle* h, double* planar, size_t n);
int fb_check(papof_handle* h, hipStream_t st, const papof_tensor& fw, const papof_tensor& bw, const papof_tensor& mask,
             int pairs, int H, int W, double a1, double a2);
int filter_h(papof_handle* h, const double* src, double* dst, int H, int W, int planes, const Taps& f,
             const Rect* rc = nullptr);
int filter_v(papof_handle* h, const double* src, double* dst, int H, int W, int planes, const Taps& f,
             const Rect* rc = nullptr);
int filter_hv(papof_handle* h, const double* src, double* dst, double* tmp, int H, int W, int planes, const Taps& fh,
              const Taps& fv);
bool filter_hv_needs_tmp(const Taps& fh, const Taps& fv);
int resize(papof_handle* h, const double* src, double* dst, int sh, int sw, int planes, int dh, int dw, double xr,
           double yr, bool use_post, double post, const Rect* rc = nullptr);
int im2feature(papof_handle* h, const double* im, double* feat, int H, int W, int C, unsigned* nz = nullptr, int frames = 1,
               size_t nz_stride = 0);
int central3_planes(papof_handle* h, const double* src, double* gx, double* gy, double* gxy, int H, int W, int planes);
int warp_bilinear(papof_handle* h, const double* im1, const double* im2, const double* vx, const double* vy,
                  double* out, int H, int W, int planes, const Rect* rc = nullptr);
int smooth_v_blend(papof_handle* h, const double* tmp, const double* im1s, double* blend, double* imdt, int H,
                   int W, int planes, const Rect* rc = nullptr);
int smooth_hv_blend(papof_handle* h, const double* warp, const double* im1s, double* blend, double* imdt, int H,
                    int W, int planes, int row0 = 0, int row1 = -1);
int warp_smooth_blend(papof_handle* h, const double* im1, const double* im2, const double* u, const double* v,
                      const double* im1s, double* blend, double* imdt, int H, int W, int planes, unsigned* wit = nullptr,
                      double* phi_out = nullptr);
int compute_phi(papof_handle* h, const double* u, const double* v, const SorPlanes* prev, double* phi, int H, int W,
                const Rect* rc = nullptr);
int assemble_system(papof_handle* h, const double* blend, const double* imdt, const double* phi, const double* u,
                    const double* v, int H, int W, int planes, double alpha, double omega, const SorPlanes& out,
                    double* opt_imdx2, double* opt_imdy2, const SorPlanes* prev, const Rect* rc = nullptr,
                    const double* gm = nullptr, const double* lap = nullptr);
int flow_system(papof_handle* h, const double* im1, const double* im2, const double* u, const double* v, const double* im1s,
                int H, int W, int planes, double alpha, double omega, const SorPlanes& out, unsigned* wit = nullptr,
                int row0 = 0, int row1 = -1,
                int batch = 1, const BatchK* bk = nullptr);
int lap_scratch_doubles();
int lap_rows_check(papof_handle* h, const double* im1, const double* im2, const double* u, const double* v, int H, int W,
                   int C, int r0, int r1, unsigned* wit, unsigned* val, unsigned mark);
bool lap_one_block_level(int H, int W);
int lap_small_check(papof_handle* h, const double* im1, const double* im2, const double* u, const double* v, int H, int W,
                    int C, unsigned* wit, int batch = 1, const BatchK* bk = nullptr);
int est_laplacian_noise(papof_handle* h, const double* im1, const double* im2, const double* u, const double* v, int H,
                        int W, int C, double* lap, double* scratch);
int gm_scratch_doubles();
int est_gaussian_mixture(papof_handle* h, const double* im1, const double* im2, int H, int W, int C, double* gm,
                         double* scratch);
int laplacian(papof_handle* h, const double* in, const double* weight, double* out, int H, int W);
int update_and_warp(papof_handle* h, const SorPlanes& sp, double* u, double* v, const double* im1,
                    const double* im2, double* warp, int H, int W, int planes, bool do_warp = true);
int bicubic_warp(papof_handle* h, const double* im1, const double* im2, const double* gx, const double* gy,
                 const double* gxy, const double* vx, const double* vy, double* out_hwc, int H, int W, int C,
                 const Rect* rc = nullptr, bool planar_out = false, bool clamp = true, int batch = 1, const BatchK* bk = nullptr);
int flow_quantize16(papof_handle* h, const double* vx, const double* vy, unsigned short* q, size_t n);
int flow_dequantize16(papof_handle* h, const unsigned short* q, double* vx, double* vy, size_t n);
int flow_to_bgr(papof_handle* h, const double* vx, const double* vy, size_t n, double* partial, unsigned char* bgr);
int update_warp_phi(papof_handle* h, const SorPlanes& sp, const double* u, const double* v, double* u_out, double* v_out,
                    const double* im1, const double* im2, double* warp, double* phi_out, int H, int W, int planes,
                    bool do_warp = true, int row0 = 0, int row1 = -1, unsigned* wit = nullptr, int batch = 1,
                    const BatchK* bk = nullptr);
int update_flow(papof_handle* h, const SorPlanes& sp, double* u, double* v, int H, int W, const Rect& r);
int sor_prep(papof_handle* h, const double* phi, const double* imdxy, const double* imdx2, const double* imdy2,
             const double* rhs1, const double* rhs2, int H, int W, double alpha, double omega, const SorPlanes& out);
int sor_unpack(papof_handle* h, const SorPlanes& sp, double* du, double* dv, int H, int W);
Taps gaussian_taps(double sigma, int fsize);
Taps smooth5_taps();
Taps deriv5_taps();
Taps central3_taps();

struct SorBatch {
    int n;
    size_t coef, d, prog, tiny;
};
int sor_solve(papof_handle* h, const SorPlanes& sp, int H, int W, double alpha, double omega, int n_sor, int mode,
              const SorBatch* bt = nullptr);
int sor_redblack_halfsweep(papof_handle* h, const SorPlanes& sp, int H, int W, double alpha, double omega, int colour,
                           const Rect& r);
int sor_blocked_depth(const papof_handle* h, int mode, int H, int W);
int sor_blocked_launch(papof_handle* h, const SorPlanes& sp, int H, int W, double alpha, double omega, int mode, int g,
                       int hs0, const Rect& out, const double* su, const double* sv, double* du, double* dv);
int sor_plan(const papof_handle* h, int H, int W, int n_sor, int mode, int* launches, int* depth);
int sor_check(papof_handle* h);
bool sor_strips_supported(const papof_handle* h, const SorPlanes& sp, int n_sor);
int sor_strips_begin(papof_handle* h, const SorPlanes& sp, int n_sor, int n_solves);
struct SorSplit {
    double* peer_du;
    unsigned* peer_prog;
    bool top_cut, bot_cut;
};
int sor_solve_bands(papof_handle* h, const SorPlanes& sp, int H, int W, double alpha, double omega, int n_sor,
                    unsigned* prog, int b0, int b1, const SorSplit* split = nullptr, int k0 = 0, int k1 = -1);
int sor_bind_plain(papof_handle* h, SorPlanes& sp, int H, int W, int n_sor);
bool sor_tiny_fits(const papof_handle* h, int H, int W, int n_sor);
constexpr size_t kTinyMaxCells = 8192;
int sor_alloc_tiny_planes(Arena& A, size_t cells, SorPlanes& sp);
size_t sor_counters_words(int H, int W, int n_sor);
int sor_counters_ensure(papof_handle* h, size_t words);
unsigned* sor_counters_clear(papof_handle* h, size_t offset_words, size_t words);
int sor_alloc_planes(Arena& A, int H, int W, int mode, int n_sor_cap, SorPlanes& sp);
int sor_bind(papof_handle* h, SorPlanes& sp, int H, int W, int n_sor);
int sor_group_size(const papof_handle* h, int H, int W, int n_sor);
int sor_reset_planes(papof_handle* h, const SorPlanes& sp);
int sor_reset_planes_batch(papof_handle* h, const SorPlanes& sp, int batch, size_t stride);
int sor_probe_dpp(papof_handle* h);

}
```

### papteam_opticalflow_amd/csrc/flow_internal.h

```cpp
#pragma once

#include <string>
#include <utility>
#include <vector>

#include "common.h"

namespace papof {

void set_last_error_text(const std::string& text);

constexpr int kTimerFused = PAPOF_N_TIMERS;
struct PhaseClock {
    papof_handle* h;
    bool on;
    std::vector<std::pair<int, std::pair<size_t, size_t>>> spans;
    size_t open = 0;
    int open_idx = -1;
    int err = PAPOF_OK;
    bool only_sor = false;
    bool stamps = false;
    std::vector<std::pair<int, int>> marks;
    std::vector<double> sor_span_sec;
    std::vector<int> sor_owner;
    size_t new_event() {
        if (h->events_used == h->events.size()) {
            hipEvent_t e;
            if (hipEventCreate(&e) != hipSuccess) {
                err = PAPOF_EDEVICE;
                return 0;
            }
            h->events.push_back(e);
        }
        hipEventRecord(h->events[h->events_used], h->stream);
        return h->events_used++;
    }
    void phase(int idx) {
        if (!on) return;
        if (stamps) {
            if (open_idx == PAPOF_T_PHASE5_SOR) {
                const size_t e = new_event();
                spans.push_back({PAPOF_T_PHASE5_SOR, {open, e}});
            }
            if (idx == PAPOF_T_PHASE5_SOR) {
                open = new_event();
                sor_owner.push_back(marks.empty() ? PAPOF_T_PHASE4_LINEARSYSTEM : marks.back().second);
            }
            const bool sor_edge = idx == PAPOF_T_PHASE5_SOR;
            open_idx = idx;
            if (only_sor || !h->stamps_dev || sor_edge) return;
            if (h->next_stamp && !marks.empty()) {
                marks.back().second = idx;
            } else if (h->stamps_used < h->stamps_cap) {
                const int slot = h->stamps_used++;
                h->next_stamp = h->stamps_dev + slot;
                marks.push_back({slot, idx});
            }
            return;
        }
        if (only_sor && idx != PAPOF_T_PHASE5_SOR && idx != PAPOF_T_TOTAL) {
            if (open_idx < 0) return;
            idx = -1;
        }
        const size_t e = new_event();
        if (open_idx >= 0) spans.push_back({open_idx, {open, e}});
        open = e;
        open_idx = idx;
    }
    void collect(double* t) {
        if (!on) return;
        for (auto& s : spans) {
            float ms = 0;
            if (hipEventElapsedTime(&ms, h->events[s.second.first], h->events[s.second.second]) == hipSuccess)
                t[s.first] += ms * 1e-3;
            if (s.first == PAPOF_T_PHASE5_SOR) sor_span_sec.push_back(ms * 1e-3);
        }
        for (size_t i = 0; i + 1 < marks.size(); i++) {
            const int idx = marks[i].second;
            if (marks[i + 1].first >= h->stamps_fetched) break;
            const unsigned long long a = h->stamps[marks[i].first], b = h->stamps[marks[i + 1].first];
            if (idx >= 0 && idx != PAPOF_T_PHASE5_SOR && b >= a) t[idx] += (double)(b - a) * 1e-8;
        }
        if (stamps && !marks.empty()) {
            for (size_t i = 0; i < sor_span_sec.size() && i < sor_owner.size(); i++)
                if (sor_owner[i] >= 0) t[sor_owner[i]] -= sor_span_sec[i];
            for (int own : {(int)PAPOF_T_PHASE4_LINEARSYSTEM, kTimerFused})
                if (t[own] < 0.0) t[own] = 0.0;
        }
    }
};

struct Level {
    int w, h;
    double *p1, *p2;
};


struct PyrPlan {
    int sw, sh, src_level, fsize;
    double sigma, rate;
};


size_t arena_bytes_for(int H, int W, int C, int levels, int n_sor_max, double ratio);
int ensure_arena(papof_handle* h, size_t bytes);
int check_params(const papof_params& P, int levels);
int pyramid_plan(int H, int W, double ratio, int nlev, std::vector<Level>& L, std::vector<PyrPlan>& plan);
int build_pyramid(papof_handle* h, const std::vector<Level>& L, const std::vector<PyrPlan>& plan, int C, bool second,
                  double* tmp_a, double* tmp_b);
int smooth_and_resize(papof_handle* h, const double* src, double* dst, double* tmp_a, double* tmp_b, const PyrPlan& p, int C,
                      int dh, int dw);
int feature_channels(int C);
int flow_batch_host(papof_handle* h, int n_pairs, int sequence, const void* const* frames, bool u8, int H, int W, int C, int levels,
                    const papof_params* params, double* const* vx, double* const* vy, double* const* warpI2, double* timing_sec);
int flow_device_planar(papof_handle* h, const double* f1, const double* f2, int H, int W, int C, int levels,
                       const papof_params& P, double* d_vx, double* d_vy, double* d_warp, double* timing,
                       const papof_tensor* init = nullptr);
int reduce_init(papof_handle* h, const papof_tensor* a, const papof_tensor* b, int pairs_a, int pairs_b, int H, int W,
                const std::vector<Level>& L, const std::vector<PyrPlan>& plan, double ratio, double* X, double* Y, double* T,
                size_t t_planes, double*& out);

}
```

### papteam_opticalflow_amd/csrc/kernels.hip

```cpp
#include "common.h"
#include "sampler.h"

#include <cmath>

namespace papof {

namespace {

constexpr int BX = 64, BY = 4;

inline dim3 grid2d(int W, int H, int planes = 1) { return dim3((W + BX - 1) / BX, (H + BY - 1) / BY, planes); }
inline Rect region(const Rect* rc, int W, int H) { return rc ? *rc : Rect{0, 0, W, H}; }
inline dim3 grid2d(const Rect& r, int planes = 1) { return grid2d(r.x1 - r.x0, r.y1 - r.y0, planes); }

__device__ __forceinline__ void stamp_now(unsigned long long* s) {
    if (s && (blockIdx.x | blockIdx.y | blockIdx.z | threadIdx.x | threadIdx.y) == 0u) *s = __builtin_amdgcn_s_memrealtime();
}
__global__ void k_stamp(unsigned long long* s) { stamp_now(s); }

__device__ __forceinline__ int clampi(int x, int n) {
    x = x < 0 ? 0 : x;
    return x > n - 1 ? n - 1 : x;
}

// ... 98 lines not shown
    const papof_tensor& b = dir ? fw : bw;
    const long long of = p * f.stride[0] + r * f.stride[1] + x * f.stride[2];
    const double u = load_flow(f, of), v = load_flow(f, of + f.stride[3]);
    const double X = (double)x + u, Y = (double)r + v;
    bool occluded = true;
    if (X >= 0 && X <= (double)(W - 1) && Y >= 0 && Y <= (double)(H - 1)) {
        double bu, bv;
        sample_flow(b, p * b.stride[0], taps_at(X, Y, H, W), bu, bv);
        occluded = !fb_passes(u, v, bu, bv, a1, a2);
    }
    static_cast<unsigned char*>(mask.data)[p * mask.stride[0] + r * mask.stride[1] + x * mask.stride[2] + dir * mask.stride[3]] =
        occluded ? 1 : 0;
}

__global__ void k_filter_h(const double* __restrict__ src, double* __restrict__ dst, int H, int W, Taps f, Rect rc) {
    const int j = rc.x0 + blockIdx.x * BX + threadIdx.x, i = rc.y0 + blockIdx.y * BY + threadIdx.y;
    if (j >= rc.x1 || i >= rc.y1) return;
    const size_t np = (size_t)H * W;
    const double* row = src + blockIdx.z * np + (size_t)i * W;
    double acc = 0.0;
    for (int l = -f.fsize; l <= f.fsize; l++) acc += row[clampi(j + l, W)] * f.t[l + f.fsize];
    dst[blockIdx.z * np + (size_t)i * W + j] = acc;
}

__global__ void k_filter_v(const double* __restrict__ src, double* __restrict__ dst, int H, int W, Taps f, Rect rc) {
    const int j = rc.x0 + blockIdx.x * BX + threadIdx.x, i = rc.y0 + blockIdx.y * BY + threadIdx.y;
    if (j >= rc.x1 || i >= rc.y1) return;
    const size_t np = (size_t)H * W;
    const double* p = src + blockIdx.z * np + j;
    double acc = 0.0;
    for (int l = -f.fsize; l <= f.fsize; l++) acc += p[(size_t)clampi(i + l, H) * W] * f.t[l + f.fsize];
    dst[blockIdx.z * np + (size_t)i * W + j] = acc;
}

#ifndef PAPOF_V_HVROWS
#define PAPOF_V_HVROWS 64
#endif
constexpr int kHvRows = PAPOF_V_HVROWS, kHvMaxF = 4;
template <int F>
__global__ __launch_bounds__(256) void k_filter_hv(const double* __restrict__ src, double* __restrict__ dst, int H, int W,
                                                   Taps fh, Taps fv) {
    __shared__ double hs[kHvRows + 2 * kHvMaxF][BX];
    const int j = blockIdx.x * BX + threadIdx.x, i0 = blockIdx.y * kHvRows;
    const int f = F >= 0 ? F : fv.fsize, fx = F >= 0 ? F : fh.fsize;
    const size_t np = (size_t)H * W;
    const double* plane = src + blockIdx.z * np;
    if (j < W) {
        for (int r = threadIdx.y; r < kHvRows + 2 * f; r += BY) {
            const double* row = plane + (size_t)clampi(i0 + r - f, H) * W;
            double acc = 0.0;
#pragma unroll
            for (int l = -fx; l <= fx; l++) acc += row[clampi(j + l, W)] * fh.t[l + fx];
            hs[r][threadIdx.x] = acc;
        }
    }
    __syncthreads();
    if (j >= W) return;
    for (int r = threadIdx.y; r < kHvRows; r += BY) {
        const int i = i0 + r;
        if (i >= H) break;
        double acc = 0.0;
#pragma unroll
        for (int l = -f; l <= f; l++) acc += hs[r + l + f][threadIdx.x] * fv.t[l + f];
        dst[blockIdx.z * np + (size_t)i * W + j] = acc;
    }
}

#ifndef PAPOF_V_HVSTAGED
#define PAPOF_V_HVSTAGED 1
#endif
#ifndef PAPOF_V_HVSROWS
#define PAPOF_V_HVSROWS 16
#endif
constexpr int kHvsRows = PAPOF_V_HVSROWS;
template <int F>
__global__ __launch_bounds__(256) void k_filter_hv_staged(const double* __restrict__ src, double* __restrict__ dst, int H,
                                                          int W, Taps fh, Taps fv) {
    __shared__ double raw[kHvsRows + 2 * F][BX + 2 * F];
    __shared__ double hs[kHvsRows + 2 * F][BX];
    int tx, ty;
    if (!xcd_tile((W + BX - 1) / BX, (H + kHvsRows - 1) / kHvsRows, tx, ty)) return;
    const int j0 = tx * BX, i0 = ty * kHvsRows;
    const size_t np = (size_t)H * W;
    const double* plane = src + blockIdx.z * np;
    constexpr int kCells = (kHvsRows + 2 * F) * (BX + 2 * F);
    for (int c = threadIdx.y * BX + threadIdx.x; c < kCells; c += BX * BY) {
        const int r = c / (BX + 2 * F), cc = c - r * (BX + 2 * F);
        raw[r][cc] = plane[(size_t)clampi(i0 + r - F, H) * W + clampi(j0 + cc - F, W)];
    }
    __syncthreads();
    for (int r = threadIdx.y; r < kHvsRows + 2 * F; r += BY) {
        double acc = 0.0;
#pragma unroll
        for (int l = -F; l <= F; l++) acc += raw[r][threadIdx.x + F + l] * fh.t[l + F];
        hs[r][threadIdx.x] = acc;
    }
    __syncthreads();
    const int j = j0 + threadIdx.x;
    if (j >= W) return;
    for (int r = threadIdx.y; r < kHvsRows; r += BY) {
        const int i = i0 + r;
        if (i >= H) break;
        double acc = 0.0;
#pragma unroll
        for (int l = -F; l <= F; l++) acc += hs[r + l + F][threadIdx.x] * fv.t[l + F];
        dst[blockIdx.z * np + (size_t)i * W + j] = acc;
    }
}

struct BilinearTaps {
    int o[4];
    double s[4];
};

__device__ __forceinline__ BilinearTaps bilinear_taps(int W, int H, double x, double y) {
    BilinearTaps b;
    const int xx = (int)x, yy = (int)y;
    double dx = x - xx, dy = y - yy;
    dx = dx > 1 ? 1.0 : dx;
    dx = dx < 0 ? 0.0 : dx;
    dy = dy > 1 ? 1.0 : dy;
    dy = dy < 0 ? 0.0 : dy;
#pragma unroll
    for (int m = 0; m <= 1; m++)
#pragma unroll
        for (int n = 0; n <= 1; n++) {
            const int u = clampi(xx + m, W), v = clampi(yy + n, H);
            b.o[m * 2 + n] = v * W + u;
            b.s[m * 2 + n] = fabs((double)(1 - m) - dx) * fabs((double)(1 - n) - dy);
        }
    return b;
}

__device__ __forceinline__ double bilinear_apply(const double* __restrict__ p, const BilinearTaps& b) {
    double acc = 0.0;
#pragma unroll
    for (int t = 0; t < 4; t++) acc += p[b.o[t]] * b.s[t];
    return acc;
}

__global__ void k_resize(const double* __restrict__ src, double* __restrict__ dst, int sh, int sw, int dh, int dw,
                         double xr, double yr, int use_post, double post, Rect rc, unsigned long long* stamp) {
    stamp_now(stamp);
    int tbx, tby;
    if (!xcd_tile((rc.x1 - rc.x0 + BX - 1) / BX, (rc.y1 - rc.y0 + BY - 1) / BY, tbx, tby)) return;
    const int j = rc.x0 + tbx * BX + threadIdx.x, i = rc.y0 + tby * BY + threadIdx.y;
    if (j >= rc.x1 || i >= rc.y1) return;
    const double x = (double)(j + 1) / xr - 1;
    const double y = (double)(i + 1) / yr - 1;
    const BilinearTaps b = bilinear_taps(sw, sh, x, y);
    double r = bilinear_apply(src + blockIdx.z * (size_t)sh * sw, b);
    if (use_post) r *= post;
    dst[blockIdx.z * (size_t)dh * dw + (size_t)i * dw + j] = r;
}

template <int C>
__device__ __forceinline__ double gray_at(const double* __restrict__ im, size_t np, size_t o) {
    if (C == 3) return im[o] * .299 + im[np + o] * .587 + im[2 * np + o] * .114;
    return im[o];
}

template <int C>
__global__ void k_im2feature(const double* __restrict__ im, double* __restrict__ feat, int H, int W, Taps d) {
    const int j = blockIdx.x * BX + threadIdx.x, i = blockIdx.y * BY + threadIdx.y;
    if (j >= W || i >= H) return;
    const size_t np = (size_t)H * W, o = (size_t)i * W + j;
    double gx = 0.0, gy = 0.0;
#pragma unroll
    for (int l = -2; l <= 2; l++) gx += gray_at<C>(im, np, (size_t)i * W + clampi(j + l, W)) * d.t[l + 2];
#pragma unroll
    for (int l = -2; l <= 2; l++) gy += gray_at<C>(im, np, (size_t)clampi(i + l, H) * W + j) * d.t[l + 2];
    feat[o] = gray_at<C>(im, np, o);
    feat[np + o] = gx;
    feat[2 * np + o] = gy;
    if (C == 3) {
        feat[3 * np + o] = im[np + o] - im[o];
        feat[4 * np + o] = im[np + o] - im[2 * np + o];
    }
}

#ifndef PAPOF_V_FEATROWS
#define PAPOF_V_FEATROWS 16
#endif
constexpr int kFeatRows = PAPOF_V_FEATROWS;
template <int C, bool BATCH = false>
__global__ __launch_bounds__(256) void k_im2feature_tiled(const double* __restrict__ im, double* __restrict__ feat, int H,
                                                          int W, Taps d, unsigned* __restrict__ nz, unsigned mark,
                                                          size_t b_im, size_t b_feat, size_t b_nz) {
    __shared__ double g[kFeatRows + 4][BX + 4];
    int tx, ty;
    if (!xcd_tile((W + BX - 1) / BX, (H + kFeatRows - 1) / kFeatRows, tx, ty)) return;
    const int j0 = tx * BX, i0 = ty * kFeatRows;
    const size_t np = (size_t)H * W;
    if (BATCH) {
        im += blockIdx.y * b_im;
        feat += blockIdx.y * b_feat;
        if (nz != nullptr) nz += blockIdx.y * b_nz;
    }
    for (int c = threadIdx.y * BX + threadIdx.x; c < (kFeatRows + 4) * (BX + 4); c += BX * BY) {
        const int r = c / (BX + 4), cc = c - r * (BX + 4);
        g[r][cc] = gray_at<C>(im, np, (size_t)clampi(i0 + r - 2, H) * W + clampi(j0 + cc - 2, W));
    }
    __syncthreads();
    const int j = j0 + threadIdx.x;
    bool any[5] = {false, false, false, false, false};
    if (j < W) {
        for (int r = threadIdx.y; r < kFeatRows; r += BY) {
            const int i = i0 + r;
            if (i >= H) break;
            const size_t o = (size_t)i * W + j;
            double gx = 0.0, gy = 0.0;
#pragma unroll
            for (int l = -2; l <= 2; l++) gx += g[r + 2][threadIdx.x + 2 + l] * d.t[l + 2];
#pragma unroll
            for (int l = -2; l <= 2; l++) gy += g[r + 2 + l][threadIdx.x + 2] * d.t[l + 2];
            const double f0 = g[r + 2][threadIdx.x + 2];
            feat[o] = f0;
            feat[np + o] = gx;
            feat[2 * np + o] = gy;
            any[0] |= f0 != 0.0;
            any[1] |= gx != 0.0;
            any[2] |= gy != 0.0;
            if (C == 3) {
                const double gg = im[np + o];
                const double f3 = gg - im[o], f4 = gg - im[2 * np + o];
                feat[3 * np + o] = f3;
                feat[4 * np + o] = f4;
                any[3] |= f3 != 0.0;
                any[4] |= f4 != 0.0;
            }
        }
    }
    if (nz != nullptr) {
#pragma unroll
        for (int k = 0; k < (C == 3 ? 5 : 3); k++)
            if (__ballot(any[k]) != 0ull && threadIdx.x == 0) nz[k] = mark;
    }
}

__global__ void k_central3_all(const double* __restrict__ src, double* __restrict__ gx, double* __restrict__ gy,
                               double* __restrict__ gxy, int H, int W, Taps c3) {
    int tbx, tby;
    if (!xcd_tile((W + BX - 1) / BX, (H + BY - 1) / BY, tbx, tby)) return;
    const int j = tbx * BX + threadIdx.x, i = tby * BY + threadIdx.y;
    if (j >= W || i >= H) return;
    const size_t np = (size_t)H * W;
    const double* p = src + blockIdx.z * np;
    const auto hrow = [&](int ii) {
        const double* row = p + (size_t)ii * W;
        double acc = 0.0;
#pragma unroll
        for (int l = -1; l <= 1; l++) acc += row[clampi(j + l, W)] * c3.t[l + 1];
        return acc;
    };
    const double hx[3] = {hrow(clampi(i - 1, H)), hrow(i), hrow(clampi(i + 1, H))};
    double vy = 0.0, vxy = 0.0;
#pragma unroll
    for (int l = -1; l <= 1; l++) vy += p[(size_t)clampi(i + l, H) * W + j] * c3.t[l + 1];
#pragma unroll
    for (int l = -1; l <= 1; l++) vxy += hx[l + 1] * c3.t[l + 1];
    const size_t o = blockIdx.z * np + (size_t)i * W + j;
    gx[o] = hx[1];
    gy[o] = vy;
    gxy[o] = vxy;
}

__device__ __forceinline__ void warp_pixel(const double* __restrict__ im1, const double* __restrict__ im2,
                                           double* __restrict__ out, double fx, double fy, int i, int j, int H,
                                           int W, int planes) {
    const size_t np = (size_t)H * W, o = (size_t)i * W + j;
    const double y = i + fy;
    const double x = j + fx;
    if (x < 0 || x > W - 1 || y < 0 || y > H - 1) {
        for (int k = 0; k < planes; k++) out[k * np + o] = im1[k * np + o];
        return;
    }
    const BilinearTaps b = bilinear_taps(W, H, x, y);
    for (int k = 0; k < planes; k++) out[k * np + o] = bilinear_apply(im2 + k * np, b);
}

__global__ void k_warp(const double* __restrict__ im1, const double* __restrict__ im2, const double* __restrict__ vx,
                       const double* __restrict__ vy, double* __restrict__ out, int H, int W, int planes, Rect rc,
                       unsigned long long* stamp) {
    stamp_now(stamp);
    const int j = rc.x0 + blockIdx.x * BX + threadIdx.x, i = rc.y0 + blockIdx.y * BY + threadIdx.y;
    if (j >= rc.x1 || i >= rc.y1) return;
    const size_t o = (size_t)i * W + j;
    warp_pixel(im1, im2, out, vx[o], vy[o], i, j, H, W, planes);
}

__global__ void k_smooth_v_blend(const double* __restrict__ tmp, const double* __restrict__ im1s,
                                 double* __restrict__ blend, double* __restrict__ imdt, int H, int W, Taps g, Rect rc) {
    const int j = rc.x0 + blockIdx.x * BX + threadIdx.x, i = rc.y0 + blockIdx.y * BY + threadIdx.y;
    if (j >= rc.x1 || i >= rc.y1) return;
    const size_t np = (size_t)H * W, o = blockIdx.z * np + (size_t)i * W + j;
    const double* p = tmp + blockIdx.z * np + j;
    double s2 = 0.0;
#pragma unroll
    for (int l = -2; l <= 2; l++) s2 += p[(size_t)clampi(i + l, H) * W] * g.t[l + 2];
    const double s1 = im1s[o];
    double t = s1;
    t *= 0.4;
    t += s2 * 0.6;
    blend[o] = t;
    imdt[o] = s2 - s1;
}
// ... 794 lines not shown
                           const double* __restrict__ imdx2, const double* __restrict__ imdy2,
                           const double* __restrict__ rhs1, const double* __restrict__ rhs2, int H, int W,
                           double alpha, double omega, SkewIdx sk, double* __restrict__ o_phi,
                           double* __restrict__ o_xy, double* __restrict__ o_a1, double* __restrict__ o_a2,
                           double* __restrict__ o_b1, double* __restrict__ o_b2) {
    const int j = blockIdx.x * BX + threadIdx.x, i = blockIdx.y * BY + threadIdx.y;
    if (j >= W || i >= H) return;
    const size_t o = (size_t)i * W + j;
    double a1, a2;
    sor_diagonals(phi, i, j, H, W, imdx2[o], imdy2[o], alpha, omega, a1, a2);
    const size_t q = sor_index<SKEW>(i, j, W, sk);
    o_phi[q] = phi[o];
    o_xy[q] = imdxy[o];
    o_a1[q] = a1;
    o_a2[q] = a2;
    o_b1[q] = rhs1[o];
    o_b2[q] = rhs2[o];
}

template <bool SKEW>
__global__ void k_sor_unpack(const double* __restrict__ sdu, const double* __restrict__ sdv,
                             double* __restrict__ du, double* __restrict__ dv, int H, int W, SkewIdx sk) {
    const int j = blockIdx.x * BX + threadIdx.x, i = blockIdx.y * BY + threadIdx.y;
    if (j >= W || i >= H) return;
    const size_t o = (size_t)i * W + j;
    if (SKEW) {
        const size_t q = 2 * dudv_cell(i, j, sk);
        du[o] = sdu[q];
        dv[o] = sdu[q + 1];
    } else {
        du[o] = sdu[o];
        dv[o] = sdv[o];
    }
}

__global__ void k_update_warp(const double* __restrict__ sdu, const double* __restrict__ sdv, double* __restrict__ u,
                              double* __restrict__ v, const double* __restrict__ im1,
                              const double* __restrict__ im2, double* __restrict__ warp, int H, int W, int planes, Rect rc,
                              int do_warp, unsigned long long* stamp) {
    stamp_now(stamp);
    const int j = rc.x0 + blockIdx.x * BX + threadIdx.x, i = rc.y0 + blockIdx.y * BY + threadIdx.y;
    if (j >= rc.x1 || i >= rc.y1) return;
    const size_t o = (size_t)i * W + j;
    double fu = u[o], fv = v[o];
    fu += sdu[o];
    fv += sdv[o];
    u[o] = fu;
    v[o] = fv;
    if (do_warp) warp_pixel(im1, im2, warp, fu, fv, i, j, H, W, planes);
}

template <bool SKEW, bool BATCH = false>
__global__ void k_update_warp_phi(const double* __restrict__ sdu, const double* __restrict__ sdv, SkewIdx sk,
                                  const double* __restrict__ u, const double* __restrict__ v,
                                  double* __restrict__ u_out, double* __restrict__ v_out,
                                  const double* __restrict__ im1, const double* __restrict__ im2,
                                  double* __restrict__ warp, double* __restrict__ phi_out, int H, int W, int planes,
                                  int do_warp, unsigned long long* stamp, int row0, int row1, unsigned* __restrict__ wit,
                                  double wit_thr, unsigned mark, BatchK bk) {
    stamp_now(stamp);
    if (BATCH) {
        const size_t p = blockIdx.y;
        sdu += p * bk.d;
        sdv += p * bk.d;
        u += p * bk.uv;
        v += p * bk.uv;
        u_out += p * bk.uv;
        v_out += p * bk.uv;
        batch_frames(bk, p, im1, im2);
        if (wit != nullptr) wit += p * bk.wit;
    }
    int tbx, tby;
    if (!xcd_tile((W + BX - 1) / BX, (row1 - row0 + BY - 1) / BY, tbx, tby)) return;
    const int j = tbx * BX + threadIdx.x, i = row0 + tby * BY + threadIdx.y;
    if (j >= W || i >= row1) return;
    const size_t o = (size_t)i * W + j;
    const auto inc = [&](int ii, int jj, double& a, double& b) {
        if (SKEW) {
            const double2s c = reinterpret_cast<const double2s*>(sdu)[dudv_cell(ii, jj, sk)];
            a = c.x;
            b = c.y;
        } else {
            a = sdu[(size_t)ii * W + jj];
            b = sdv[(size_t)ii * W + jj];
        }
    };
    double a, b;
    inc(i, j, a, b);
    double fu = u[o], fv = v[o];
    fu += a;
    fv += b;
    u_out[o] = fu;
    v_out[o] = fv;
    if (wit != nullptr) {
        const int bw = min(W - tbx * BX, BX), bh = min(row1 - (row0 + tby * BY), BY);
        const int lin = threadIdx.y * bw + threadIdx.x;
        const size_t np = (size_t)H * W;
        if (np <= 65536) {
            for (int k = bw * bh >= planes ? lin % planes : lin; k < planes; k += bw * bh) {
                const double w = warp_value(im1 + k * np, im2 + k * np, fu, fv, i, j, H, W);
                const double d = fabs(im1[k * np + o] - w);
                if (d >= wit_thr && d < 1000000) wit[k] = mark;
            }
        } else if (((tbx + 5 * tby) & 15) == 0)
        for (int k = lin; k < planes; k += bw * bh) {
            const double w = warp_value(im1 + k * np, im2 + k * np, fu, fv, i, j, H, W);
            const double d = fabs(im1[k * np + o] - w);
            if (d >= wit_thr && d < 1000000) wit[k] = mark;
        }
    }
    if (phi_out != nullptr) {
        double ur = 0.0, vr = 0.0, ud = 0.0, vd = 0.0;
        if (j < W - 1) {
            inc(i, j + 1, a, b);
            ur = u[o + 1];
            vr = v[o + 1];
            ur += a;
            vr += b;
        }
        if (i < H - 1) {
            inc(i + 1, j, a, b);
            ud = u[o + W];
            vd = v[o + W];
            ud += a;
            vd += b;
        }
        const double ux = j < W - 1 ? ur - fu : 0.0;
        const double uy = i < H - 1 ? ud - fu : 0.0;
        const double vx = j < W - 1 ? vr - fv : 0.0;
        const double vy = i < H - 1 ? vd - fv : 0.0;
        const double t = ux * ux + uy * uy + vx * vx + vy * vy;
        phi_out[o] = 0.5 / sqrt(t + 0.001 * 0.001);
    }
    if (do_warp) warp_pixel(im1, im2, warp, fu, fv, i, j, H, W, planes);
}

__global__ void k_update_warp_skew(const double2s* __restrict__ pd, double* __restrict__ u, double* __restrict__ v,
                                   const double* __restrict__ im1, const double* __restrict__ im2,
                                   double* __restrict__ warp, int H, int W, int planes, SkewIdx sk,
                                   unsigned long long* stamp, int do_warp) {
    stamp_now(stamp);
    const int j = blockIdx.x * BX + threadIdx.x, i = blockIdx.y * BY + threadIdx.y;
    if (j >= W || i >= H) return;
    const size_t o = (size_t)i * W + j;
    const double2s c = pd[dudv_cell(i, j, sk)];
    double fu = u[o], fv = v[o];
    fu += c.x;
    fv += c.y;
    u[o] = fu;
    v[o] = fv;
    if (do_warp) warp_pixel(im1, im2, warp, fu, fv, i, j, H, W, planes);
}

template <bool BATCH>
__global__ void k_bicubic(const double* __restrict__ im1, const double* __restrict__ im2,
                          const double* __restrict__ gx, const double* __restrict__ gy,
                          const double* __restrict__ gxy, const double* __restrict__ vx,
                          const double* __restrict__ vy, double* __restrict__ out, int H, int W, int C, Rect rc,
                          unsigned long long* stamp, int planar_out, int clamp, BatchK bk) {
    if (BATCH) {
        const size_t p = blockIdx.y;
        const ptrdiff_t o1 = (ptrdiff_t)batch_frames(bk, p, im1, im2);
        const ptrdiff_t o2 = bk.bw != 0 && p >= bk.bw ? o1 - 2 * (ptrdiff_t)bk.fr : o1;
        gx += o2;
        gy += o2;
        gxy += o2;
        vx += p * bk.uv;
        vy += p * bk.uv;
        out += p * bk.out;
    }
    stamp_now(stamp);
    int tbx, tby;
    if (!xcd_tile((rc.x1 - rc.x0 + BX - 1) / BX, (rc.y1 - rc.y0 + BY - 1) / BY, tbx, tby)) return;
    const int j = rc.x0 + tbx * BX + threadIdx.x, i = rc.y0 + tby * BY + threadIdx.y;
    if (j >= rc.x1 || i >= rc.y1) return;
    const size_t np = (size_t)H * W, o = (size_t)i * W + j;
    const size_t ostride = planar_out ? np : 1, obase = planar_out ? o : o * C;
    const double x = j + vx[o];
    const double y = i + vy[o];
    if (x < 0 || x > W - 1 || y < 0 || y > H - 1) {
        for (int k = 0; k < C; k++) {
            double r = im1[k * np + o];
            if (clamp) {
                r = r < 0 ? 0.0 : r;
                r = r > 1 ? 1.0 : r;
            }
            out[obase + k * ostride] = r;
        }
        return;
    }
    int x0 = (int)x, y0 = (int)y;
    int x1 = x0 + 1, y1 = y0 + 1;
    x0 = clampi(x0, W);
    x1 = clampi(x1, W);
    y0 = clampi(y0, H);
    y1 = clampi(y1, H);
    const double dx = x - x0, dy = y - y0;
    const double dx2 = dx * dx, dy2 = dy * dy;
    const double dx3 = dx * dx2, dy3 = dy * dy2;
    const size_t a = (size_t)y0 * W + x0, b = (size_t)y0 * W + x1, c = (size_t)y1 * W + x0, d = (size_t)y1 * W + x1;
    for (int k = 0; k < C; k++) {
        const double *f = im2 + k * np, *px = gx + k * np, *py = gy + k * np, *pz = gxy + k * np;
        const double fA = f[a], fB = f[b], fC = f[c], fD = f[d];
        const double xA = px[a], xB = px[b], xC = px[c], xD = px[d];
        const double yA = py[a], yB = py[b], yC = py[c], yD = py[d];
        const double zA = pz[a], zB = pz[b], zC = pz[c], zD = pz[d];
        const double c00 = fA;
        const double c10 = xA;
        const double c20 = -3 * fA + 3 * fB - 2 * xA - xB;
        const double c30 = 2 * fA - 2 * fB + xA + xB;
        const double c01 = yA;
        const double c11 = zA;
        const double c21 = -3 * yA + 3 * yB - 2 * zA - zB;
        const double c31 = 2 * yA - 2 * yB + zA + zB;
        const double c02 = -3 * fA + 3 * fC - 2 * yA - yC;
        const double c12 = -3 * xA + 3 * xC - 2 * zA - zC;
        const double c22 = 9 * fA - 9 * fB - 9 * fC + 9 * fD + 6 * xA + 3 * xB - 6 * xC - 3 * xD + 6 * yA - 6 * yB +
                           3 * yC - 3 * yD + 4 * zA + 2 * zB + 2 * zC + zD;
        const double c32 = -6 * fA + 6 * fB + 6 * fC - 6 * fD - 3 * xA - 3 * xB + 3 * xC + 3 * xD - 4 * yA + 4 * yB -
                           2 * yC + 2 * yD - 2 * zA - 2 * zB - zC - zD;
        const double c03 = 2 * fA - 2 * fC + yA + yC;
        const double c13 = 2 * xA - 2 * xC + zA + zC;
        const double c23 = -6 * fA + 6 * fB + 6 * fC - 6 * fD - 4 * xA - 2 * xB + 4 * xC + 2 * xD - 3 * yA + 3 * yB -
                           3 * yC + 3 * yD - 2 * zA - zB - 2 * zC - zD;
        const double c33 = 4 * fA - 4 * fB - 4 * fC + 4 * fD + 2 * xA + 2 * xB - 2 * xC - 2 * xD + 2 * yA - 2 * yB +
                           2 * yC - 2 * yD + zA + zB + zC + zD;
        double r = c00 + c01 * dy + c02 * dy2 + c03 * dy3 + c10 * dx + c11 * dx * dy + c12 * dx * dy2 +
                   c13 * dx * dy3 + c20 * dx2 + c21 * dx2 * dy + c22 * dx2 * dy2 + c23 * dx2 * dy3 + c30 * dx3 +
                   c31 * dx3 * dy + c32 * dx3 * dy2 + c33 * dx3 * dy3;
        if (clamp) {
            r = r < 0 ? 0.0 : r;
            r = r > 1 ? 1.0 : r;
        }
        out[obase + k * ostride] = r;
    }
}

__global__ void k_flow_quantize16(const double* __restrict__ vx, const double* __restrict__ vy,
                                  unsigned short* __restrict__ q, size_t n) {
    const size_t i = (size_t)blockIdx.x * blockDim.x + threadIdx.x;
    if (i >= n) return;
    double a = vx[i], b = vy[i];
    a = (a < -200) ? -200.0 : a;
    a = (a > 200) ? 200.0 : a;
    b = (b < -200) ? -200.0 : b;
    b = (b > 200) ? 200.0 : b;
    q[i * 2] = (unsigned short)((a + 200) * 160);
    q[i * 2 + 1] = (unsigned short)((b + 200) * 160);
}

__global__ void k_flow_dequantize16(const unsigned short* __restrict__ q, double* __restrict__ vx,
                                    double* __restrict__ vy, size_t n) {
    const size_t i = (size_t)blockIdx.x * blockDim.x + threadIdx.x;
    if (i >= n) return;
    vx[i] = (double)q[i * 2] / 160 - 200;
    vy[i] = (double)q[i * 2 + 1] / 160 - 200;
}

__global__ void k_flow_mag_minmax(const double* __restrict__ vx, const double* __restrict__ vy, size_t n,
                                  double* __restrict__ partial) {
    __shared__ double smin[256], smax[256];
    double lo = INFINITY, hi = -INFINITY;
    for (size_t i = (size_t)blockIdx.x * blockDim.x + threadIdx.x; i < n; i += (size_t)gridDim.x * blockDim.x) {
        const double m = sqrt(vx[i] * vx[i] + vy[i] * vy[i]);
        lo = m < lo ? m : lo;
        hi = m > hi ? m : hi;
    }
    smin[threadIdx.x] = lo;
    smax[threadIdx.x] = hi;
    __syncthreads();
    for (int s = 128; s > 0; s >>= 1) {
        if ((int)threadIdx.x < s) {
            smin[threadIdx.x] = fmin(smin[threadIdx.x], smin[threadIdx.x + s]);
            smax[threadIdx.x] = fmax(smax[threadIdx.x], smax[threadIdx.x + s]);
        }
        __syncthreads();
    }
    if (threadIdx.x == 0) {
        partial[2 * blockIdx.x] = smin[0];
        partial[2 * blockIdx.x + 1] = smax[0];
    }
}

__global__ void k_flow_bgr(const double* __restrict__ vx, const double* __restrict__ vy, size_t n,
                           const double* __restrict__ partial, int nblocks, unsigned char* __restrict__ bgr) {
    const size_t i = (size_t)blockIdx.x * blockDim.x + threadIdx.x;
    if (i >= n) return;
    double lo = INFINITY, hi = -INFINITY;
    for (int b = 0; b < nblocks; b++) {
        lo = fmin(lo, partial[2 * b]);
        hi = fmax(hi, partial[2 * b + 1]);
    }
    const double x = vx[i], y = vy[i];
    const double mag = sqrt(x * x + y * y);
    double ang = atan2(y, x);
    if (ang < 0) ang += 2 * M_PI;
    const unsigned char H = (unsigned char)(int)(ang * 180 / M_PI / 2);
    const double scale = hi > lo ? 255.0 / (hi - lo) : 0.0;
    const unsigned char V = (unsigned char)(int)((mag - lo) * scale);
    const float v = V * (1.f / 255.f);
    float h = H * (6.f / 180.f);
    int sector = (int)floorf(h);
    h -= sector;
    sector = ((sector % 6) + 6) % 6;
    const float tab[4] = {v, 0.f, v * (1.f - h), v * h};
    const int sd[6][3] = {{1, 3, 0}, {1, 0, 2}, {3, 0, 1}, {0, 2, 1}, {0, 1, 3}, {2, 1, 0}};
    bgr[i * 3] = (unsigned char)(int)rintf(tab[sd[sector][0]] * 255.f);
    bgr[i * 3 + 1] = (unsigned char)(int)rintf(tab[sd[sector][1]] * 255.f);
    bgr[i * 3 + 2] = (unsigned char)(int)rintf(tab[sd[sector][2]] * 255.f);
}

}

Taps gaussian_taps(double sigma, int fsize) {
    Taps f{};
    f.fsize = fsize;
    double sum = 0;
    const double s2 = sigma * sigma * 2;
    for (int i = -fsize; i <= fsize; i++) {
        f.t[i + fsize] = std::exp(-(double)(i * i) / s2);
        sum += f.t[i + fsize];
    }
    for (int i = 0; i < 2 * fsize + 1; i++) f.t[i] /= sum;
    return f;
}

Taps smooth5_taps() {
    Taps f{};
    f.fsize = 2;
    const double g[5] = {0.02, 0.11, 0.74, 0.11, 0.02};
    for (int i = 0; i < 5; i++) f.t[i] = g[i];
    return f;
}

Taps deriv5_taps() {
    Taps f{};
    f.fsize = 2;
    const double d[5] = {1, -8, 0, 8, -1};
    for (int i = 0; i < 5; i++) {
        f.t[i] = d[i];
        f.t[i] /= 12;
    }
    return f;
}

Taps central3_taps() {
    Taps f{};
    f.fsize = 1;
    f.t[0] = -0.5;
    f.t[1] = 0;
    f.t[2] = 0.5;
    return f;
}

#define LAUNCH_CHECK() PAPOF_HIP(hipGetLastError())

int hwc_to_planar(papof_handle* h, const double* hwc, double* planar, int H, int W, int C, int frames) {
    hipLaunchKernelGGL(k_hwc_to_planar, grid2d(W, H, frames), dim3(BX, BY), 0, h->stream, hwc, planar, H, W, C);
    LAUNCH_CHECK();
    return PAPOF_OK;
}

int hwc_u8_to_planar(papof_handle* h, const unsigned char* hwc, double* planar, int H, int W, int C, int frames) {
    hipLaunchKernelGGL(k_hwc_u8_to_planar, grid2d(W, H, frames), dim3(BX, BY), 0, h->stream, hwc, planar, H, W, C);
    LAUNCH_CHECK();
    return PAPOF_OK;
}

int ingest_frames(papof_handle* h, const papof_tensor& a, const papof_tensor* b, double* planar, int H, int W, int C,
                  int frames) {
    const long long total = (long long)frames * H * W * C, blocks = (total + 255) / 256;
    if (total <= 0) return PAPOF_OK;
    if (blocks > 0x7fffffffLL) return PAPOF_EINVAL;
    hipLaunchKernelGGL(k_ingest_frames, dim3((unsigned)blocks), dim3(256), 0, h->stream, a, b ? *b : a, b ? 1 : 0, planar,
                       (long long)H, (long long)W, (long long)C, total);
    LAUNCH_CHECK();
    return PAPOF_OK;
}

int init_check(papof_handle* h, const papof_tensor& t, int pairs, int H, int W, unsigned* flag) {
    const long long total = (long long)pairs * H * W * 2, blocks = (total + 255) / 256;
    if (total <= 0) return PAPOF_OK;
    if (blocks > 0x7fffffffLL) return PAPOF_EINVAL;
    hipLaunchKernelGGL(k_init_check, dim3((unsigned)blocks), dim3(256), 0, h->stream, t, (long long)H, (long long)W, total,
                       flag);
    LAUNCH_CHECK();
    return PAPOF_OK;
}

int init_sanitize(papof_handle* h, double* planar, size_t n) {
    const long long total = (long long)n, blocks = (total + 255) / 256;
    if (total <= 0) return PAPOF_OK;
    if (blocks > 0x7fffffffLL) return PAPOF_EINVAL;
    hipLaunchKernelGGL(k_init_sanitize, dim3((unsigned)blocks), dim3(256), 0, h->stream, planar, total);
    LAUNCH_CHECK();
    return PAPOF_OK;
}

bool filter_hv_needs_tmp(const Taps& fh, const Taps& fv) { return fh.fsize > kHvMaxF || fv.fsize > kHvMaxF; }

int emit_outputs(papof_handle* h, const double* src, const papof_tensor& dst, bool comp_major, int H, int W, int K, int pairs) {
    const long long total = (long long)pairs * H * W * K, blocks = (total + 255) / 256;
    if (total <= 0) return PAPOF_OK;
    if (blocks > 0x7fffffffLL) return PAPOF_EINVAL;
    hipLaunchKernelGGL(k_emit_outputs, dim3((unsigned)blocks), dim3(256), 0, h->stream, src, dst, comp_major ? 1 : 0,
                       (long long)H, (long long)W, (long long)K, total);
    LAUNCH_CHECK();
    return PAPOF_OK;
}

int fb_check(papof_handle* h, hipStream_t st, const papof_tensor& fw, const papof_tensor& bw, const papof_tensor& mask,
             int pairs, int H, int W, double a1, double a2) {
    const long long tiles = (long long)((W + kFbTX - 1) / kFbTX) * ((H + kFbTY - 1) / kFbTY);
    if (pairs <= 0 || tiles <= 0) return PAPOF_OK;
    if (tiles > kMaxTiles) return PAPOF_EINVAL;
    const auto at = [](const papof_tensor& t, long long items) {
        papof_tensor r = t;
        r.data = static_cast<char*>(t.data) + items * t.stride[0] * dtype_bytes(t.dtype);
        return r;
    };
    for (int p0 = 0; p0 < pairs; p0 += 32767) {
        const int n = std::min(32767, pairs - p0);
        hipLaunchKernelGGL(k_fb_check, dim3((unsigned)tiles, 2 * n), dim3(kFbTX, kFbTY), 0, st, at(fw, p0), at(bw, p0),
                           at(mask, p0), H, W, a1, a2);
        LAUNCH_CHECK();
    }
    return PAPOF_OK;
}

int planar_to_hwc(papof_handle* h, const double* planar, double* hwc, int H, int W, int C) {
    hipLaunchKernelGGL(k_planar_to_hwc, grid2d(W, H), dim3(BX, BY), 0, h->stream, planar, hwc, H, W, C);
    LAUNCH_CHECK();
    return PAPOF_OK;
}

int filter_h(papof_handle* h, const double* src, double* dst, int H, int W, int planes, const Taps& f, const Rect* rc) {
    const Rect r = region(rc, W, H);
    if (r.empty()) return PAPOF_OK;
    hipLaunchKernelGGL(k_filter_h, grid2d(r, planes), dim3(BX, BY), 0, h->stream, src, dst, H, W, f, r);
    LAUNCH_CHECK();
    return PAPOF_OK;
}

int filter_v(papof_handle* h, const double* src, double* dst, int H, int W, int planes, const Taps& f, const Rect* rc) {
    const Rect r = region(rc, W, H);
    if (r.empty()) return PAPOF_OK;
    hipLaunchKernelGGL(k_filter_v, grid2d(r, planes), dim3(BX, BY), 0, h->stream, src, dst, H, W, f, r);
    LAUNCH_CHECK();
    return PAPOF_OK;
}

int central3_planes(papof_handle* h, const double* src, double* gx, double* gy, double* gxy, int H, int W, int planes) {
    hipLaunchKernelGGL(k_central3_all, dim3(xcd_grid((W + BX - 1) / BX, (H + BY - 1) / BY), 1, planes), dim3(BX, BY), 0, h->stream, src, gx, gy, gxy, H, W,
                       central3_taps());
    LAUNCH_CHECK();
    return PAPOF_OK;
}

int filter_hv(papof_handle* h, const double* src, double* dst, double* tmp, int H, int W, int planes, const Taps& fh,
              const Taps& fv) {
    if (fh.fsize > kHvMaxF || fv.fsize > kHvMaxF) {
        if (!tmp) return PAPOF_EINVAL;
        PAPOF_TRY(filter_h(h, src, tmp, H, W, planes, fh));
        return filter_v(h, tmp, dst, H, W, planes, fv);
    }
    const dim3 grid((W + BX - 1) / BX, (H + kHvRows - 1) / kHvRows, planes), block(BX, BY);
    const int f = fh.fsize == fv.fsize ? fh.fsize : -1;
    if (PAPOF_V_HVSTAGED && f >= 1 && f <= 3) {
        const dim3 sgrid(xcd_grid((W + BX - 1) / BX, (H + kHvsRows - 1) / kHvsRows), 1, planes);
        if (f == 1)
            hipLaunchKernelGGL(k_filter_hv_staged<1>, sgrid, block, 0, h->stream, src, dst, H, W, fh, fv);
        else if (f == 2)
            hipLaunchKernelGGL(k_filter_hv_staged<2>, sgrid, block, 0, h->stream, src, dst, H, W, fh, fv);
        else
            hipLaunchKernelGGL(k_filter_hv_staged<3>, sgrid, block, 0, h->stream, src, dst, H, W, fh, fv);
        LAUNCH_CHECK();
        return PAPOF_OK;
    }
    if (f == 1)
        hipLaunchKernelGGL(k_filter_hv<1>, grid, block, 0, h->stream, src, dst, H, W, fh, fv);
    else if (f == 2)
        hipLaunchKernelGGL(k_filter_hv<2>, grid, block, 0, h->stream, src, dst, H, W, fh, fv);
    else if (f == 3)
        hipLaunchKernelGGL(k_filter_hv<3>, grid, block, 0, h->stream, src, dst, H, W, fh, fv);
    else
        hipLaunchKernelGGL(k_filter_hv<-1>, grid, block, 0, h->stream, src, dst, H, W, fh, fv);
    LAUNCH_CHECK();
    return PAPOF_OK;
}

int resize(papof_handle* h, const double* src, double* dst, int sh, int sw, int planes, int dh, int dw, double xr,
           double yr, bool use_post, double post, const Rect* rc) {
    const Rect r = region(rc, dw, dh);
    if (r.empty()) return PAPOF_OK;
    hipLaunchKernelGGL(k_resize, dim3(xcd_grid((r.x1 - r.x0 + BX - 1) / BX, (r.y1 - r.y0 + BY - 1) / BY), 1, planes), dim3(BX, BY), 0, h->stream, src, dst, sh, sw, dh, dw, xr, yr,
                       use_post ? 1 : 0, post, r, take_stamp(h));
    LAUNCH_CHECK();
    return PAPOF_OK;
}

int im2feature(papof_handle* h, const double* im, double* feat, int H, int W, int C, unsigned* nz, int frames, size_t nz_stride) {
    const size_t np = (size_t)H * W;
    if (C == 3) {
        hipLaunchKernelGGL((frames > 1 ? k_im2feature_tiled<3, true> : k_im2feature_tiled<3, false>), dim3(xcd_grid((W + BX - 1) / BX, (H + kFeatRows - 1) / kFeatRows), frames), dim3(BX, BY), 0,
                           h->stream, im, feat, H, W, deriv5_taps(), nz, h->lap_epoch, 3 * np, 5 * np, nz_stride);
    } else if (C == 1) {
        hipLaunchKernelGGL((frames > 1 ? k_im2feature_tiled<1, true> : k_im2feature_tiled<1, false>), dim3(xcd_grid((W + BX - 1) / BX, (H + kFeatRows - 1) / kFeatRows), frames), dim3(BX, BY), 0,
                           h->stream, im, feat, H, W, deriv5_taps(), nz, h->lap_epoch, np, 3 * np, nz_stride);
    } else {
        if (frames != 1) return PAPOF_EINVAL;
        PAPOF_HIP(hipMemcpyAsync(feat, im, sizeof(double) * (size_t)H * W * C, hipMemcpyDeviceToDevice, h->stream));
        return PAPOF_OK;
    }
    LAUNCH_CHECK();
    return PAPOF_OK;
}

int warp_bilinear(papof_handle* h, const double* im1, const double* im2, const double* vx, const double* vy,
                  double* out, int H, int W, int planes, const Rect* rc) {
    const Rect r = region(rc, W, H);
    if (r.empty()) return PAPOF_OK;
    hipLaunchKernelGGL(k_warp, grid2d(r), dim3(BX, BY), 0, h->stream, im1, im2, vx, vy, out, H, W, planes, r,
                       take_stamp(h));
    LAUNCH_CHECK();
    return PAPOF_OK;
}

int smooth_v_blend(papof_handle* h, const double* tmp, const double* im1s, double* blend, double* imdt, int H,
                   int W, int planes, const Rect* rc) {
    const Rect r = region(rc, W, H);
    if (r.empty()) return PAPOF_OK;
    hipLaunchKernelGGL(k_smooth_v_blend, grid2d(r, planes), dim3(BX, BY), 0, h->stream, tmp, im1s, blend, imdt, H, W,
                       smooth5_taps(), r);
    LAUNCH_CHECK();
    return PAPOF_OK;
}

static SkewIdx skew_idx(const SorPlanes& sp) {
    return SkewIdx{sp.sd.hp, sp.sd.qt, sp.sd.rt, sp.sd.nb, sp.sd.npos_d, sp.sd.dpar, sp.sd.band_rows, sp.sd.koff, sp.sd.poff};
}

static Increment increment_of(const SorPlanes* prev, const double* gm = nullptr, const double* lap = nullptr) {
    if (!prev) return Increment{nullptr, nullptr, 0, SkewIdx{0, 0, 0, 0, 0, 0, 0}, gm, lap};
    return Increment{prev->du, prev->dv, prev->skew ? 1 : 0, prev->skew ? skew_idx(*prev) : SkewIdx{0, 0, 0, 0, 0, 0, 0},
                     gm, lap};
}

int smooth_hv_blend(papof_handle* h, const double* warp, const double* im1s, double* blend, double* imdt, int H,
                    int W, int planes, int row0, int row1) {
    if (row1 < 0) row1 = H;
    if (row0 < 0 || row1 > H) return PAPOF_EINVAL;
    if (row1 <= row0) return PAPOF_OK;
    hipLaunchKernelGGL(k_smooth_hv_blend, dim3((W + BX - 1) / BX, (row1 - row0 + kFuseRows - 1) / kFuseRows, planes),
                       dim3(BX, BY), 0, h->stream, warp, im1s, blend, imdt, H, W, smooth5_taps(), take_stamp(h), row0,
                       row1);
    LAUNCH_CHECK();
    return PAPOF_OK;
}

int warp_smooth_blend(papof_handle* h, const double* im1, const double* im2, const double* u, const double* v,
                      const double* im1s, double* blend, double* imdt, int H, int W, int planes, unsigned* wit,
                      double* phi_out) {
    hipLaunchKernelGGL(k_warp_smooth_blend, dim3((W + BX - 1) / BX, (H + kWsRows - 1) / kWsRows, planes), dim3(BX, BY), 0,
                       h->stream, im1, im2, u, v, im1s, blend, imdt, H, W, smooth5_taps(), take_stamp(h), wit,
                       2e-20 * (double)H * (double)W, h->lap_epoch, phi_out);
    LAUNCH_CHECK();
    return PAPOF_OK;
}

int compute_phi(papof_handle* h, const double* u, const double* v, const SorPlanes* prev, double* phi, int H, int W,
                const Rect* rc) {
    const Rect r = region(rc, W, H);
    if (r.empty()) return PAPOF_OK;
    hipLaunchKernelGGL(k_phi, grid2d(r), dim3(BX, BY), 0, h->stream, u, v, increment_of(prev), phi, H, W, r,
                       take_stamp(h));
    LAUNCH_CHECK();
    return PAPOF_OK;
}

int assemble_system(papof_handle* h, const double* blend, const double* imdt, const double* phi, const double* u,
                    const double* v, int H, int W, int planes, double alpha, double omega, const SorPlanes& out,
                    double* opt_imdx2, double* opt_imdy2, const SorPlanes* prev, const Rect* rc, const double* gm,
                    const double* lap) {
    const Increment I = increment_of(prev, gm, lap);
    const Rect r = region(rc, W, H);
    if (r.empty()) return PAPOF_OK;
    if (out.skew) {
        if (rc && (r.x0 != 0 || r.x1 != W)) return PAPOF_EINVAL;
        const bool fast = I.du == nullptr && I.gm == nullptr && I.lap == nullptr;
        const auto kern = planes == 5   ? (fast ? k_assemble_skew<5, true> : k_assemble_skew<5, false>)
                          : planes == 3 ? (fast ? k_assemble_skew<3, true> : k_assemble_skew<3, false>)
                                        : k_assemble_skew<0, false>;
        hipLaunchKernelGGL(kern, dim3((W + kTileJ - 1) / kTileJ, (r.y1 - r.y0 + kAsmRows - 1) / kAsmRows),
                           dim3(256), 0, h->stream, blend, imdt, phi, u, v, H, W, planes, alpha, omega, skew_idx(out),
                           (double2s*)out.phi, (double2s*)out.a1, (double2s*)out.b1, opt_imdx2, opt_imdy2,
                           deriv5_taps(), I, take_stamp(h), r.y0, r.y1);
    } else {
        hipLaunchKernelGGL(k_assemble, grid2d(r), dim3(BX, BY), 0, h->stream, blend, imdt, phi, u, v, H, W, planes,
                           alpha, omega, out.phi, out.xy, out.a1, out.a2, out.b1, out.b2, opt_imdx2, opt_imdy2,
                           deriv5_taps(), I, r, take_stamp(h));
    }
    LAUNCH_CHECK();
    return PAPOF_OK;
}

int flow_system(papof_handle* h, const double* im1, const double* im2, const double* u, const double* v, const double* im1s,
                int H, int W, int planes, double alpha, double omega, const SorPlanes& out, unsigned* wit, int row0, int row1,
                int batch, const BatchK* bk) {
    if (planes != 5 && planes != 3) return PAPOF_EINVAL;
    if (row1 < 0) row1 = H;
    if (row0 < 0 || row1 > H) return PAPOF_EINVAL;
    if (row1 <= row0) return PAPOF_OK;
    static const int tx_env = std::getenv("PAPOF_FS_TX") ? std::atoi(std::getenv("PAPOF_FS_TX")) : 0;
    const int TXr = tx_env == 32 ? 32 : (tx_env == 16 ? 16 : kFlowSystemTX);
    const int ntiles = ((W + TXr - 1) / TXr) * ((row1 - row0 + kFT - 1) / kFT);
    const dim3 grid(8 * ((ntiles + 7) / 8), batch);
    const SixPlanes six{{out.phi, out.xy, out.a1, out.a2, out.b1, out.b2}};
    const BatchK bk0{0, 0, 0, 0, 0, 0};
    const auto kern16 = batch > 1 ? (out.skew ? (planes == 5 ? k_flow_system<5, true, true> : k_flow_system<3, true, true>)
                                              : (planes == 5 ? k_flow_system<5, false, true> : k_flow_system<3, false, true>))
                                  : (out.skew ? (planes == 5 ? k_flow_system<5, true> : k_flow_system<3, true>)
                                              : (planes == 5 ? k_flow_system<5, false> : k_flow_system<3, false>));
    const auto kern32 = batch > 1 ? (out.skew ? (planes == 5 ? k_flow_system<5, true, true, 32> : k_flow_system<3, true, true, 32>)
                                              : (planes == 5 ? k_flow_system<5, false, true, 32> : k_flow_system<3, false, true, 32>))
                                  : (out.skew ? (planes == 5 ? k_flow_system<5, true, false, 32> : k_flow_system<3, true, false, 32>)
                                              : (planes == 5 ? k_flow_system<5, false, false, 32> : k_flow_system<3, false, false, 32>));
    const auto kern = TXr == 32 ? kern32 : kern16;
    hipLaunchKernelGGL(kern, grid, dim3(TXr * kFT), 0, h->stream, im1, im2, u, v, im1s, H, W, alpha, omega,
                       out.skew ? skew_idx(out) : SkewIdx{0, 0, 0, 0, 0, 0, 0, 0, 0}, six, smooth5_taps(), deriv5_taps(),
                       take_stamp(h), wit, 2e-20 * (double)H * (double)W, h->lap_epoch, row0, row1, bk ? *bk : bk0);
    LAUNCH_CHECK();
    return PAPOF_OK;
}

int laplacian(papof_handle* h, const double* in, const double* weight, double* out, int H, int W) {
    hipLaunchKernelGGL(k_laplacian, grid2d(W, H), dim3(BX, BY), 0, h->stream, in, weight, out, H, W);
    LAUNCH_CHECK();
    return PAPOF_OK;
}

int update_and_warp(papof_handle* h, const SorPlanes& sp, double* u, double* v, const double* im1,
                    const double* im2, double* warp, int H, int W, int planes, bool do_warp) {
    if (sp.skew) {
        hipLaunchKernelGGL(k_update_warp_skew, grid2d(W, H), dim3(BX, BY), 0, h->stream, (const double2s*)sp.du, u, v,
                           im1, im2, warp, H, W, planes, skew_idx(sp), take_stamp(h), do_warp ? 1 : 0);
    } else {
        hipLaunchKernelGGL(k_update_warp, grid2d(W, H), dim3(BX, BY), 0, h->stream, sp.du, sp.dv, u, v, im1, im2, warp,
                           H, W, planes, Rect{0, 0, W, H}, do_warp ? 1 : 0, take_stamp(h));
    }
    LAUNCH_CHECK();
    return PAPOF_OK;
}

int update_warp_phi(papof_handle* h, const SorPlanes& sp, const double* u, const double* v, double* u_out, double* v_out,
                    const double* im1, const double* im2, double* warp, double* phi_out, int H, int W, int planes,
                    bool do_warp, int row0, int row1, unsigned* wit, int batch, const BatchK* bk) {
    const double wit_thr = 2e-20 * (double)H * (double)W;
    const BatchK bk0{0, 0, 0, 0, 0, 0};
    if (batch > 1 && (warp || phi_out || do_warp)) return PAPOF_EINVAL;
    if (u == u_out || v == v_out) return PAPOF_EINVAL;
    if (row1 < 0) row1 = H;
    if (row0 < 0 || row1 > H) return PAPOF_EINVAL;
    if (row1 <= row0) return PAPOF_OK;
    const dim3 grid(xcd_grid((W + BX - 1) / BX, (row1 - row0 + BY - 1) / BY), batch);
    if (sp.skew)
        hipLaunchKernelGGL((batch > 1 ? k_update_warp_phi<true, true> : k_update_warp_phi<true, false>), grid, dim3(BX, BY), 0,
                           h->stream, sp.du, sp.dv, skew_idx(sp),
                           u, v, u_out, v_out, im1, im2, warp, phi_out, H, W, planes, do_warp ? 1 : 0, take_stamp(h),
                           row0, row1, wit, wit_thr, h->lap_epoch, bk ? *bk : bk0);
    else
        hipLaunchKernelGGL((batch > 1 ? k_update_warp_phi<false, true> : k_update_warp_phi<false, false>), grid, dim3(BX, BY), 0, h->stream, sp.du, sp.dv,
                           SkewIdx{0, 0, 0, 0, 0, 0, 0, 0, 0}, u, v, u_out, v_out, im1, im2, warp, phi_out, H, W, planes,
                           do_warp ? 1 : 0, take_stamp(h), row0, row1, wit, wit_thr, h->lap_epoch, bk ? *bk : bk0);
    LAUNCH_CHECK();
    return PAPOF_OK;
}

int update_flow(papof_handle* h, const SorPlanes& sp, double* u, double* v, int H, int W, const Rect& r) {
    if (sp.skew) return PAPOF_EINVAL;
    if (r.empty()) return PAPOF_OK;
    hipLaunchKernelGGL(k_update_warp, grid2d(r), dim3(BX, BY), 0, h->stream, sp.du, sp.dv, u, v, nullptr, nullptr, nullptr,
                       H, W, 0, r, 0, take_stamp(h));
    LAUNCH_CHECK();
    return PAPOF_OK;
}

int flow_quantize16(papof_handle* h, const double* vx, const double* vy, unsigned short* q, size_t n) {
    if (!n) return PAPOF_OK;
    hipLaunchKernelGGL(k_flow_quantize16, dim3((unsigned)((n + 255) / 256)), dim3(256), 0, h->stream, vx, vy, q, n);
    LAUNCH_CHECK();
    return PAPOF_OK;
}

int flow_dequantize16(papof_handle* h, const unsigned short* q, double* vx, double* vy, size_t n) {
    if (!n) return PAPOF_OK;
    hipLaunchKernelGGL(k_flow_dequantize16, dim3((unsigned)((n + 255) / 256)), dim3(256), 0, h->stream, q, vx, vy, n);
    LAUNCH_CHECK();
    return PAPOF_OK;
}

int flow_to_bgr(papof_handle* h, const double* vx, const double* vy, size_t n, double* partial ,
                unsigned char* bgr) {
    if (!n) return PAPOF_OK;
    const int nblocks = 256;
    hipLaunchKernelGGL(k_flow_mag_minmax, dim3(nblocks), dim3(256), 0, h->stream, vx, vy, n, partial);
    hipLaunchKernelGGL(k_flow_bgr, dim3((unsigned)((n + 255) / 256)), dim3(256), 0, h->stream, vx, vy, n, partial,
                       nblocks, bgr);
    LAUNCH_CHECK();
    return PAPOF_OK;
}

int bicubic_warp(papof_handle* h, const double* im1, const double* im2, const double* gx, const double* gy,
                 const double* gxy, const double* vx, const double* vy, double* out_hwc, int H, int W, int C,
                 const Rect* rc, bool planar_out, bool clamp, int batch, const BatchK* bk) {
    const Rect r = region(rc, W, H);
    if (r.empty()) return PAPOF_OK;
    const BatchK bk0{0, 0, 0, 0, 0, 0};
    hipLaunchKernelGGL(batch > 1 ? k_bicubic<true> : k_bicubic<false>, dim3(xcd_grid((r.x1 - r.x0 + BX - 1) / BX, (r.y1 - r.y0 + BY - 1) / BY), batch), dim3(BX, BY), 0, h->stream, im1, im2, gx, gy, gxy, vx, vy, out_hwc, H, W,
                       C, r, take_stamp(h), planar_out ? 1 : 0, clamp ? 1 : 0, bk ? *bk : bk0);
    LAUNCH_CHECK();
    return PAPOF_OK;
}

constexpr int kGmBlocks = 256, kGmThreads = 256, kGmMaxC = 8;
static __global__ __launch_bounds__(kGmThreads) void k_gm_partial(const double* __restrict__ im1,
                                                           const double* __restrict__ im2, size_t np, int C,
                                                           const double* __restrict__ gm, double* __restrict__ partial) {
    __shared__ double red[kGmThreads];
    double acc[kGmMaxC][4];
    for (int k = 0; k < kGmMaxC; k++) acc[k][0] = acc[k][1] = acc[k][2] = acc[k][3] = 0.0;
    for (size_t o = (size_t)blockIdx.x * kGmThreads + threadIdx.x; o < np; o += (size_t)kGmBlocks * kGmThreads) {
#pragma unroll
        for (int k = 0; k < kGmMaxC; k++) {
            if (k >= C) break;
            double t = im1[k * np + o] - im2[k * np + o];
            t *= t;
            const double alpha_k = gm[k], sigma = gm[C + k], beta = gm[2 * C + k], s2 = gm[3 * C + k], b2 = gm[4 * C + k];
            double w1 = exp(-t / (2 * s2)) / (2 * 3.1415927 * sigma) * alpha_k;
            double w2 = exp(-t / (2 * b2)) / (2 * 3.1415927 * beta) * (1 - alpha_k);
            const double s = w1 + w2;
            w1 /= s;
            w2 /= s;
            acc[k][0] += w1;
            acc[k][1] += w2;
            acc[k][2] += w1 * t;
            acc[k][3] += w2 * t;
        }
    }
    for (int k = 0; k < C; k++)
        for (int q = 0; q < 4; q++) {
            red[threadIdx.x] = acc[k][q];
            __syncthreads();
            for (int s = kGmThreads / 2; s > 0; s >>= 1) {
                if ((int)threadIdx.x < s) red[threadIdx.x] += red[threadIdx.x + s];
                __syncthreads();
            }
            if (threadIdx.x == 0) partial[((size_t)blockIdx.x * kGmMaxC + k) * 4 + q] = red[0];
            __syncthreads();
        }
}

static __global__ void k_gm_mstep(const double* __restrict__ partial, int C, double prior, double* __restrict__ gm) {
    const int k = threadIdx.x;
    if (k >= C) return;
    double t1 = 0.0, t2 = 0.0, s1 = 0.05, s2 = 0.5;
    for (int b = 0; b < kGmBlocks; b++) {
        const double* p = partial + ((size_t)b * kGmMaxC + k) * 4;
        t1 += p[0];
        t2 += p[1];
        s1 += p[2];
        s2 += p[3];
    }
    const double alpha = t1 / (t1 + t2) * (1 - prior) + 0.95 * prior;
    const double sigma = sqrt(s1 / t1);
    const double beta = sqrt(s2 / t2) * (1 - prior) + 0.3 * prior;
    gm[k] = alpha;
    gm[C + k] = sigma;
    gm[2 * C + k] = beta;
    gm[3 * C + k] = sigma * sigma;
    gm[4 * C + k] = beta * beta;
}

int gm_scratch_doubles() { return kGmBlocks * kGmMaxC * 4; }

int est_gaussian_mixture(papof_handle* h, const double* im1, const double* im2, int H, int W, int C, double* gm,
                         double* scratch) {
    if (C > kGmMaxC) return PAPOF_EINVAL;
    for (int it = 0; it < 3; it++) {
        hipLaunchKernelGGL(k_gm_partial, dim3(kGmBlocks), dim3(kGmThreads), 0, h->stream, im1, im2, (size_t)H * W, C, gm,
                           scratch);
        hipLaunchKernelGGL(k_gm_mstep, dim3(1), dim3(64), 0, h->stream, scratch, C, 0.9, gm);
    }
    LAUNCH_CHECK();
    return PAPOF_OK;
}

constexpr int kLapBlocks = 256, kLapThreads = 256, kLapMaxC = 8;
static __global__ __launch_bounds__(kLapThreads) void k_lap_partial(const double* __restrict__ im1,
                                                             const double* __restrict__ im2,
                                                             const double* __restrict__ u, const double* __restrict__ v,
                                                             int H, int W, int C, double* __restrict__ partial) {
    __shared__ double red[kLapThreads];
    const size_t np = (size_t)H * W;
    double acc[kLapMaxC][2];
    for (int k = 0; k < kLapMaxC; k++) acc[k][0] = acc[k][1] = 0.0;
    for (size_t o = (size_t)blockIdx.x * kLapThreads + threadIdx.x; o < np; o += (size_t)kLapBlocks * kLapThreads) {
        const int i = (int)(o / W), j = (int)(o - (size_t)i * W);
        const double fu = u ? u[o] : 0.0, fv = u ? v[o] : 0.0;
#pragma unroll
        for (int k = 0; k < kLapMaxC; k++) {
            if (k >= C) break;
            const double w = u ? warp_value(im1 + k * np, im2 + k * np, fu, fv, i, j, H, W) : im2[k * np + o];
            const double d = fabs(im1[k * np + o] - w);
            if (d > 0 && d < 1000000) {
                acc[k][0] += d;
                acc[k][1] += 1.0;
            }
        }
    }
    for (int k = 0; k < C; k++)
        for (int q = 0; q < 2; q++) {
            red[threadIdx.x] = acc[k][q];
            __syncthreads();
            for (int s = kLapThreads / 2; s > 0; s >>= 1) {
                if ((int)threadIdx.x < s) red[threadIdx.x] += red[threadIdx.x + s];
                __syncthreads();
            }
            if (threadIdx.x == 0) partial[((size_t)blockIdx.x * kLapMaxC + k) * 2 + q] = red[0];
            __syncthreads();
        }
}
static __global__ void k_lap_finish(const double* __restrict__ partial, int C, double* __restrict__ lap) {
    const int k = threadIdx.x;
    if (k >= C) return;
    double s = 0.0, n = 0.0;
    for (int b = 0; b < kLapBlocks; b++) {
        s += partial[((size_t)b * kLapMaxC + k) * 2];
        n += partial[((size_t)b * kLapMaxC + k) * 2 + 1];
    }
    lap[k] = n == 0 ? 0.001 : s / n;
}
static __global__ __launch_bounds__(256) void k_lap_small(const double* __restrict__ im1, const double* __restrict__ im2,
                                                       const double* __restrict__ u, const double* __restrict__ v, int H,
                                                       int W, unsigned* __restrict__ wit, double wit_thr, unsigned mark,
                                                       BatchK bk) {
    const int np = H * W;
    {
        const size_t p = blockIdx.y;
        batch_frames(bk, p, im1, im2);
        u += p * bk.uv;
        v += p * bk.uv;
        wit += p * bk.wit;
    }
    const double *p1 = im1 + (size_t)blockIdx.x * np, *p2 = im2 + (size_t)blockIdx.x * np;
    bool hit = false, valid = false;
    for (int o = threadIdx.x; o < np; o += 256) {
        const int i = o / W, j = o - i * W;
        const double d = fabs(p1[o] - warp_value(p1, p2, u[o], v[o], i, j, H, W));
        valid = valid || (d > 0 && d < 1000000);
        hit = hit || (d >= wit_thr && d < 1000000);
    }
    const int any_hit = __syncthreads_or(hit ? 1 : 0), any_valid = __syncthreads_or(valid ? 1 : 0);
    if (threadIdx.x == 0 && (any_hit || !any_valid)) wit[blockIdx.x] = any_hit ? mark : (mark ^ kLapNone);
}
static __global__ __launch_bounds__(256) void k_lap_rows(const double* __restrict__ im1, const double* __restrict__ im2,
                                                      const double* __restrict__ u, const double* __restrict__ v, int H,
                                                      int W, int r0, int r1, unsigned* __restrict__ wit,
                                                      unsigned* __restrict__ val, double wit_thr, unsigned mark) {
    const size_t np = (size_t)H * W;
    const double *p1 = im1 + blockIdx.y * np, *p2 = im2 + blockIdx.y * np;
    bool hit = false, valid = false;
// ... 77 lines not shown
```

Before: 205.7.

## Fuse pyramid smooth+resize, compute bicubic gradients inline, split prep to overlap solve

Adds a fused tiled kernel that does the Gaussian smoothing and bilinear downsampling of a pyramid level in one pass through shared memory. This drops the temporary filter buffers and the separate filter and resize launches. Bicubic warping can now compute the x, y and xy central-difference gradients on the fly from the image, so the precomputed gx/gy/gxy planes and the central3 pass are no longer needed. The preparation stage is split so the coarsest level is prepared first and its solve overlaps with preparing the remaining levels. The cost is extra redundant loads and arithmetic in the bicubic kernel and more complex stream scheduling.

```diff
diff --git a/papteam_opticalflow_amd/csrc/api.hip b/papteam_opticalflow_amd/csrc/api.hip
--- a/papteam_opticalflow_amd/csrc/api.hip
+++ b/papteam_opticalflow_amd/csrc/api.hip
@@ -128,8 +128,20 @@
                       int dh, int dw) {
     const Taps g = gaussian_taps(p.sigma, p.fsize);
     if (g.fsize == 0 && g.t[0] == 1.0) return resize(h, src, dst, p.sh, p.sw, C, dh, dw, p.rate, p.rate, false, 0.0);
+    if (pyramid_level_fused(g.fsize, p.sh, p.sw, dh, dw, p.rate))
+        return pyramid_level(h, src, dst, p.sh, p.sw, C, dh, dw, p.rate, g);
+    if (!tmp_b) return PAPOF_EINVAL;
     PAPOF_TRY(filter_hv(h, src, tmp_b, tmp_a, p.sh, p.sw, C, g, g));
     return resize(h, tmp_b, dst, p.sh, p.sw, C, dh, dw, p.rate, p.rate, false, 0.0);
+}
+
+bool pyramid_needs_tmp(const std::vector<Level>& L, const std::vector<PyrPlan>& plan) {
+    for (size_t i = 1; i < L.size(); i++) {
+        const Taps g = gaussian_taps(plan[i].sigma, plan[i].fsize);
+        if (!(g.fsize == 0 && g.t[0] == 1.0) && !pyramid_level_fused(g.fsize, plan[i].sh, plan[i].sw, L[i].h, L[i].w, plan[i].rate))
+            return true;
+    }
+    return false;
 }
 
 int reduce_init(papof_handle* h, const papof_tensor* a, const papof_tensor* b, int pairs_a, int pairs_b, int H, int W,
@@ -161,6 +173,11 @@
         const Taps g = gaussian_taps(p.sigma, p.fsize);
         if (g.fsize == 0 && g.t[0] == 1.0) {
             PAPOF_TRY(resize(h, cur, other, p.sh, p.sw, planes, L[i].h, L[i].w, p.rate, p.rate, last, last ? s : 0.0));
+            std::swap(cur, other);
+            continue;
+        }
+        if (pyramid_level_fused(g.fsize, p.sh, p.sw, L[i].h, L[i].w, p.rate)) {
+            PAPOF_TRY(pyramid_level(h, cur, other, p.sh, p.sw, planes, L[i].h, L[i].w, p.rate, g, last, last ? s : 0.0));
             std::swap(cur, other);
             continue;
         }
@@ -437,8 +454,9 @@
         L[i].p1 = slot[slot1];
         L[i].p2 = slot[slot1 ^ 1];
     }
-    double* tmp_a = A.f64(np0 * C);
-    double* tmp_b = A.f64(np0 * C);
+    const bool pyr_tmp = pyramid_needs_tmp(L, plan);
+    double* tmp_a = pyr_tmp ? A.f64(np0 * C) : nullptr;
+    double* tmp_b = pyr_tmp ? A.f64(np0 * C) : nullptr;
     if (A.overflow) return PAPOF_ENOMEM;
     if (op == kSeqPrime) {
         PAPOF_TRY(load_frame(h, fa, L[0].p1, H, W, C));
@@ -457,9 +475,10 @@
         S1[k] = A.f64(n);
     }
     double* prep_tmp = A.f64(np0 * fc);
-    double* gx = A.f64(np0 * C);
-    double* gy = A.f64(np0 * C);
-    double* gxy = A.f64(np0 * C);
+    constexpr bool grad_planes = !PAPOF_V_BICSELF;
+    double* gx = grad_planes ? A.f64(np0 * C) : nullptr;
+    double* gy = grad_planes ? A.f64(np0 * C) : nullptr;
+    double* gxy = grad_planes ? A.f64(np0 * C) : nullptr;
     double* warp = A.f64(np0 * fc);
     double* u = A.f64(2 * np0);
     double* v = u ? u + np0 : nullptr;
@@ -510,18 +529,20 @@
         double* dst = second ? L[i].p2 : L[i].p1;
         return smooth_and_resize(h, src, dst, tmp_a, tmp_b, q, C, L[i].h, L[i].w);
     };
-    const auto prepare = [&]() -> int {
+    const auto prepare = [&](int part) -> int {
         StreamSwap on_prep(h, prep);
-        pclk.phase(PAPOF_T_ALLOCATION);
-        if (exact && !sor_counters_clear(h, 0, prog_total)) return PAPOF_EDEVICE;
-        pclk.phase(PAPOF_T_CONSTRUCTION);
-        if (op != kSeqNext) PAPOF_TRY(load_frame(h, fa, L[0].p1, H, W, C));
-        PAPOF_TRY(load_frame(h, fb, L[0].p2, H, W, C));
         const int first = op == kSeqNext ? 1 : 0;
-        if (!from_level0)
-            for (int i = 1; i < levels; i++)
-                for (int second = first; second < 2; second++) PAPOF_TRY(build_level(i, second));
-        for (int k = levels - 1; k >= 0; k--) {
+        if (part == 0) {
+            pclk.phase(PAPOF_T_ALLOCATION);
+            if (exact && !sor_counters_clear(h, 0, prog_total)) return PAPOF_EDEVICE;
+            pclk.phase(PAPOF_T_CONSTRUCTION);
+            if (op != kSeqNext) PAPOF_TRY(load_frame(h, fa, L[0].p1, H, W, C));
+            PAPOF_TRY(load_frame(h, fb, L[0].p2, H, W, C));
+            if (!from_level0)
+                for (int i = 1; i < levels; i++)
+                    for (int second = first; second < 2; second++) PAPOF_TRY(build_level(i, second));
+        }
+        for (int k = part == 0 ? levels - 1 : levels - 2; k >= (part == 0 ? levels - 1 : 0); k--) {
             if (from_level0) {
                 pclk.phase(PAPOF_T_CONSTRUCTION);
                 for (int second = first; second < 2; second++) PAPOF_TRY(build_level(k, second));
@@ -534,46 +555,50 @@
             pclk.phase(-1);
             if (overlap) PAPOF_HIP(hipEventRecord(h->sync_events[k], prep));
         }
-        pclk.phase(PAPOF_T_POSTPROCESSING);
-        PAPOF_TRY(central3_planes(h, L[0].p2, gx, gy, gxy, H, W, C));
-        pclk.phase(-1);
-        if (overlap) PAPOF_HIP(hipEventRecord(h->sync_events[levels], prep));
+        if (grad_planes && part == 1) {
+            pclk.phase(PAPOF_T_POSTPROCESSING);
+            PAPOF_TRY(central3_planes(h, L[0].p2, gx, gy, gxy, H, W, C));
+            pclk.phase(-1);
+            if (overlap) PAPOF_HIP(hipEventRecord(h->sync_events[levels], prep));
+        }
         return PAPOF_OK;
     };
     papof_handle::HostIO& io = h->hostio;
     const bool hostio = io.active && overlap && h->copy_stream && h->copy_events.size() >= 8;
-    const auto prepare_hostio = [&]() -> int {
+    const auto prepare_hostio = [&](int part) -> int {
         StreamSwap on_prep(h, prep);
         hipStream_t const cs = h->copy_stream;
-        pclk.phase(PAPOF_T_ALLOCATION);
-        if (exact && !sor_counters_clear(h, 0, prog_total)) return PAPOF_EDEVICE;
-        if (io.im1) {
-            PAPOF_HIP(hipMemcpyAsync(const_cast<void*>(fa.d), io.im1, io.nb_in, hipMemcpyHostToDevice, cs));
-            PAPOF_HIP(hipEventRecord(h->copy_events[0], cs));
-            PAPOF_HIP(hipStreamWaitEvent(prep, h->copy_events[0], 0));
-        }
-        pclk.phase(PAPOF_T_CONSTRUCTION);
-        if (op != kSeqNext) {
-            PAPOF_TRY(load_frame(h, fa, L[0].p1, H, W, C));
-            for (int i = 1; i < levels; i++) PAPOF_TRY(build_level(i, 0));
-        }
-        for (int k = levels - 1; k >= 0; k--) {
+        if (part == 0) {
             pclk.phase(PAPOF_T_ALLOCATION);
-            PAPOF_TRY(im2feature(h, L[k].p1, F1[k], L[k].h, L[k].w, C, lg ? lg->nz(k) : nullptr));
-            pclk.phase(PAPOF_T_PHASE1_GENERATE);
-            PAPOF_TRY(filter_hv(h, F1[k], S1[k], prep_tmp, L[k].h, L[k].w, fc, g5, g5));
-        }
-        pclk.phase(-1);
-        if (io.im2) {
-            PAPOF_HIP(hipMemcpyAsync(const_cast<void*>(fb.d), io.im2, io.nb_in, hipMemcpyHostToDevice, cs));
-            PAPOF_HIP(hipEventRecord(h->copy_events[1], cs));
-            PAPOF_HIP(hipStreamWaitEvent(prep, h->copy_events[1], 0));
-        }
-        pclk.phase(PAPOF_T_CONSTRUCTION);
-        PAPOF_TRY(load_frame(h, fb, L[0].p2, H, W, C));
-        if (!from_level0)
-            for (int i = 1; i < levels; i++) PAPOF_TRY(build_level(i, 1));
-        for (int k = levels - 1; k >= 0; k--) {
+            if (exact && !sor_counters_clear(h, 0, prog_total)) return PAPOF_EDEVICE;
+            if (io.im1) {
+                PAPOF_HIP(hipMemcpyAsync(const_cast<void*>(fa.d), io.im1, io.nb_in, hipMemcpyHostToDevice, cs));
+                PAPOF_HIP(hipEventRecord(h->copy_events[0], cs));
+                PAPOF_HIP(hipStreamWaitEvent(prep, h->copy_events[0], 0));
+            }
+            pclk.phase(PAPOF_T_CONSTRUCTION);
+            if (op != kSeqNext) {
+                PAPOF_TRY(load_frame(h, fa, L[0].p1, H, W, C));
+                for (int i = 1; i < levels; i++) PAPOF_TRY(build_level(i, 0));
+            }
+            for (int k = levels - 1; k >= 0; k--) {
+                pclk.phase(PAPOF_T_ALLOCATION);
+                PAPOF_TRY(im2feature(h, L[k].p1, F1[k], L[k].h, L[k].w, C, lg ? lg->nz(k) : nullptr));
+                pclk.phase(PAPOF_T_PHASE1_GENERATE);
+                PAPOF_TRY(filter_hv(h, F1[k], S1[k], prep_tmp, L[k].h, L[k].w, fc, g5, g5));
+            }
+            pclk.phase(-1);
+            if (io.im2) {
+                PAPOF_HIP(hipMemcpyAsync(const_cast<void*>(fb.d), io.im2, io.nb_in, hipMemcpyHostToDevice, cs));
+                PAPOF_HIP(hipEventRecord(h->copy_events[1], cs));
+                PAPOF_HIP(hipStreamWaitEvent(prep, h->copy_events[1], 0));
+            }
+            pclk.phase(PAPOF_T_CONSTRUCTION);
+            PAPOF_TRY(load_frame(h, fb, L[0].p2, H, W, C));
+            if (!from_level0)
+                for (int i = 1; i < levels; i++) PAPOF_TRY(build_level(i, 1));
+        }
+        for (int k = part == 0 ? levels - 1 : levels - 2; k >= (part == 0 ? levels - 1 : 0); k--) {
             if (from_level0) {
                 pclk.phase(PAPOF_T_CONSTRUCTION);
                 PAPOF_TRY(build_level(k, 1));
@@ -583,10 +608,12 @@
             pclk.phase(-1);
             PAPOF_HIP(hipEventRecord(h->sync_events[k], prep));
         }
-        pclk.phase(PAPOF_T_POSTPROCESSING);
-        PAPOF_TRY(central3_planes(h, L[0].p2, gx, gy, gxy, H, W, C));
-        pclk.phase(-1);
-        PAPOF_HIP(hipEventRecord(h->sync_events[levels], prep));
+        if (grad_planes && part == 1) {
+            pclk.phase(PAPOF_T_POSTPROCESSING);
+            PAPOF_TRY(central3_planes(h, L[0].p2, gx, gy, gxy, H, W, C));
+            pclk.phase(-1);
+            PAPOF_HIP(hipEventRecord(h->sync_events[levels], prep));
+        }
         return PAPOF_OK;
     };
     if (io.active && !hostio) {
@@ -597,19 +624,20 @@
         PAPOF_HIP(hipEventRecord(h->sync_events[levels + 1], main_stream));
         PAPOF_HIP(hipStreamWaitEvent(prep, h->sync_events[levels + 1], 0));
     }
-    {
-        const int rc = hostio ? prepare_hostio() : prepare();
-        if (rc != PAPOF_OK) {
-            if (overlap) hipStreamSynchronize(prep);
-            return rc;
-        }
-    }
+    const auto run_prepare = [&](int part) -> int {
+        const int rc = hostio ? prepare_hostio(part) : prepare(part);
+        if (rc != PAPOF_OK && overlap) hipStreamSynchronize(prep);
+        return rc;
+    };
+    const bool split = PAPOF_V_PREPSPLIT && overlap && levels > 1;
+    PAPOF_TRY(run_prepare(0));
+    if (!split) PAPOF_TRY(run_prepare(1));
 
     int pw = 0, ph = 0;
-    const auto solve_levels = [&]() -> int {
-        if (lg && lg->guard())
+    const auto solve_levels = [&](int k_hi, int k_lo) -> int {
+        if (k_hi == levels - 1 && lg && lg->guard())
             PAPOF_HIP(hipMemcpyAsync(lg->lap, h->lap_init_dev, 8 * sizeof(double), hipMemcpyDeviceToDevice, main_stream));
-        for (int k = levels - 1; k >= 0; k--) {
+        for (int k = k_hi; k >= k_lo; k--) {
             const int lw = L[k].w, lh = L[k].h;
             const size_t np = (size_t)lw * lh;
             clk.phase(-1);
@@ -663,8 +691,9 @@
             pw = lw;
             ph = lh;
         }
+        if (k_lo > 0) return PAPOF_OK;
         clk.phase(-1);
-        if (overlap) PAPOF_HIP(hipStreamWaitEvent(main_stream, h->sync_events[levels], 0));
+        if (overlap && grad_planes) PAPOF_HIP(hipStreamWaitEvent(main_stream, h->sync_events[levels], 0));
         clk.phase(PAPOF_T_POSTPROCESSING);
         if (hostio && io.early_out && u == d_vx && v == d_vy) {
             hipStream_t const cs = h->copy_stream;
@@ -690,7 +719,9 @@
         if (v != d_vy) PAPOF_HIP(hipMemcpyAsync(d_vy, v, np0 * sizeof(double), hipMemcpyDeviceToDevice, h->stream));
         return PAPOF_OK;
     };
-    const int rc_main = solve_levels();
+    int rc_main = solve_levels(levels - 1, split ? levels - 1 : 0);
+    if (split && rc_main == PAPOF_OK) rc_main = run_prepare(1);
+    if (split && rc_main == PAPOF_OK) rc_main = solve_levels(levels - 2, 0);
     if (rc_main != PAPOF_OK) {
         hipStreamSynchronize(main_stream);
         if (overlap) hipStreamSynchronize(prep);
@@ -1634,9 +1665,11 @@
     double* b = S.up_planar(im2, height, width, c);
     double* fx = S.up_planar(vx, height, width, 1);
     double* fy = S.up_planar(vy, height, width, 1);
-    double *gx = S.dev(n), *gy = S.dev(n), *gxy = S.dev(n), *o = S.dev(n);
-    PAPOF_TRY(S.rc);
-    PAPOF_TRY(central3_planes(h, b, gx, gy, gxy, height, width, c));
+    double *gx = nullptr, *gy = nullptr, *gxy = nullptr;
+    if (!PAPOF_V_BICSELF) gx = S.dev(n), gy = S.dev(n), gxy = S.dev(n);
+    double* o = S.dev(n);
+    PAPOF_TRY(S.rc);
+    if (gx) PAPOF_TRY(central3_planes(h, b, gx, gy, gxy, height, width, c));
     PAPOF_TRY(bicubic_warp(h, a, b, gx, gy, gxy, fx, fy, o, height, width, c, nullptr, false, clamp != 0));
     PAPOF_HIP(hipMemcpyAsync(out, o, n * sizeof(double), hipMemcpyDeviceToHost, h->stream));
     PAPOF_HIP(hipStreamSynchronize(h->stream));
diff --git a/papteam_opticalflow_amd/csrc/batch.hip b/papteam_opticalflow_amd/csrc/batch.hip
--- a/papteam_opticalflow_amd/csrc/batch.hip
+++ b/papteam_opticalflow_amd/csrc/batch.hip
@@ -95,11 +95,13 @@
         F[k] = A.f64((size_t)nF * n * fc);
         S[k] = A.f64((size_t)nF * n * fc);
     }
-    double* tmp_a = A.f64((size_t)nF * np0 * C);
-    double* tmp_b = A.f64((size_t)nF * np0 * C);
-    double* gx = A.f64((size_t)nF * np0 * C);
-    double* gy = A.f64((size_t)nF * np0 * C);
-    double* gxy = A.f64((size_t)nF * np0 * C);
+    const bool pyr_tmp = pyramid_needs_tmp(L, plan);
+    double* tmp_a = pyr_tmp ? A.f64((size_t)nF * np0 * C) : nullptr;
+    double* tmp_b = pyr_tmp ? A.f64((size_t)nF * np0 * C) : nullptr;
+    constexpr bool grad_planes = !PAPOF_V_BICSELF;
+    double* gx = grad_planes ? A.f64((size_t)nF * np0 * C) : nullptr;
+    double* gy = grad_planes ? A.f64((size_t)nF * np0 * C) : nullptr;
+    double* gxy = grad_planes ? A.f64((size_t)nF * np0 * C) : nullptr;
     double* uvA = A.f64((size_t)NP * 2 * np0);
     double* uvB = A.f64((size_t)NP * 2 * np0);
     double* warp = A.f64((size_t)NP * np0 * C);
@@ -175,7 +177,7 @@
         PAPOF_TRY(im2feature(h, Lp[k], F[k], L[k].h, L[k].w, C, nz_known ? nzf + (size_t)k * 8 : nullptr, nF, kLapNzWords));
         PAPOF_TRY(filter_hv(h, F[k], S[k], nullptr, L[k].h, L[k].w, fc * nF, g5, g5));
     }
-    PAPOF_TRY(central3_planes(h, Lp[0], gx, gy, gxy, H, W, C * nF));
+    if (grad_planes) PAPOF_TRY(central3_planes(h, Lp[0], gx, gy, gxy, H, W, C * nF));
 
     double *uv = uvA, *uv2 = uvB;
     int pw = 0, ph = 0, slot = 0;
@@ -239,8 +241,9 @@
         bk.out = np0 * C;
         bk.bw = with_bw ? B : 0;
         bk.fr = np0 * C;
-        PAPOF_TRY(bicubic_warp(h, Lp[0], Lp[0] + np0 * C, gx + np0 * C, gy + np0 * C, gxy + np0 * C, uv, uv + np0, warp, H, W, C,
-                               nullptr, false, true, NP, &bk));
+        const size_t g2 = np0 * C;
+        PAPOF_TRY(bicubic_warp(h, Lp[0], Lp[0] + np0 * C, gx ? gx + g2 : nullptr, gy ? gy + g2 : nullptr, gxy ? gxy + g2 : nullptr, uv,
+                               uv + np0, warp, H, W, C, nullptr, false, true, NP, &bk));
         return PAPOF_OK;
     };
     const int rc_levels = levels_loop();
diff --git a/papteam_opticalflow_amd/csrc/common.h b/papteam_opticalflow_amd/csrc/common.h
--- a/papteam_opticalflow_amd/csrc/common.h
+++ b/papteam_opticalflow_amd/csrc/common.h
@@ -276,6 +276,9 @@
 bool filter_hv_needs_tmp(const Taps& fh, const Taps& fv);
 int resize(papof_handle* h, const double* src, double* dst, int sh, int sw, int planes, int dh, int dw, double xr,
            double yr, bool use_post, double post, const Rect* rc = nullptr);
+bool pyramid_level_fused(int fsize, int sh, int sw, int dh, int dw, double rate);
+int pyramid_level(papof_handle* h, const double* src, double* dst, int sh, int sw, int planes, int dh, int dw, double rate,
+                  const Taps& g, bool use_post = false, double post = 0.0);
 int im2feature(papof_handle* h, const double* im, double* feat, int H, int W, int C, unsigned* nz = nullptr, int frames = 1,
                size_t nz_stride = 0);
 int central3_planes(papof_handle* h, const double* src, double* gx, double* gy, double* gxy, int H, int W, int planes);
@@ -312,6 +315,9 @@
 int laplacian(papof_handle* h, const double* in, const double* weight, double* out, int H, int W);
 int update_and_warp(papof_handle* h, const SorPlanes& sp, double* u, double* v, const double* im1,
                     const double* im2, double* warp, int H, int W, int planes, bool do_warp = true);
+#ifndef PAPOF_V_BICSELF
+#define PAPOF_V_BICSELF 1
+#endif
 int bicubic_warp(papof_handle* h, const double* im1, const double* im2, const double* gx, const double* gy,
                  const double* gxy, const double* vx, const double* vy, double* out_hwc, int H, int W, int C,
                  const Rect* rc = nullptr, bool planar_out = false, bool clamp = true, int batch = 1, const BatchK* bk = nullptr);
diff --git a/papteam_opticalflow_amd/csrc/flow_internal.h b/papteam_opticalflow_amd/csrc/flow_internal.h
--- a/papteam_opticalflow_amd/csrc/flow_internal.h
+++ b/papteam_opticalflow_amd/csrc/flow_internal.h
@@ -90,6 +90,10 @@
     }
 };
 
+#ifndef PAPOF_V_PREPSPLIT
+#define PAPOF_V_PREPSPLIT 1
+#endif
+
 struct Level {
     int w, h;
     double *p1, *p2;
@@ -110,6 +114,7 @@
                   double* tmp_a, double* tmp_b);
 int smooth_and_resize(papof_handle* h, const double* src, double* dst, double* tmp_a, double* tmp_b, const PyrPlan& p, int C,
                       int dh, int dw);
+bool pyramid_needs_tmp(const std::vector<Level>& L, const std::vector<PyrPlan>& plan);
 int feature_channels(int C);
 int flow_batch_host(papof_handle* h, int n_pairs, int sequence, const void* const* frames, bool u8, int H, int W, int C, int levels,
                     const papof_params* params, double* const* vx, double* const* vy, double* const* warpI2, double* timing_sec);
diff --git a/papteam_opticalflow_amd/csrc/kernels.hip b/papteam_opticalflow_amd/csrc/kernels.hip
--- a/papteam_opticalflow_amd/csrc/kernels.hip
+++ b/papteam_opticalflow_amd/csrc/kernels.hip
@@ -274,6 +274,72 @@
     double r = bilinear_apply(src + blockIdx.z * (size_t)sh * sw, b);
     if (use_post) r *= post;
     dst[blockIdx.z * (size_t)dh * dw + (size_t)i * dw + j] = r;
+}
+
+#ifndef PAPOF_V_PYRFUSED
+#define PAPOF_V_PYRFUSED 1
+#endif
+constexpr int kPyrTW = 16, kPyrTH = 8;
+constexpr double pyr_min_rate(int F) { return F == 1 ? 0.5 : (F == 2 ? 0.36 : 0.25); }
+constexpr int pyr_span(int outputs, int F) { return (int)((outputs - 1) / pyr_min_rate(F)) + 3 + 2 * F; }
+__host__ __device__ __forceinline__ int pyr_tap(int o, double rate, int m, int n) {
+    const double x = (double)(o + 1) / rate - 1;
+    int u = (int)x + m;
+    u = u < 0 ? 0 : u;
+    return u > n - 1 ? n - 1 : u;
+}
+template <int F>
+__global__ __launch_bounds__(256) void k_pyramid_level(const double* __restrict__ src, double* __restrict__ dst, int sh, int sw,
+                                                       int dh, int dw, double xr, double yr, Taps g, int use_post,
+                                                       double post) {
+    constexpr int RH = pyr_span(kPyrTH, F), RW = pyr_span(kPyrTW, F);
+    __shared__ double raw[RH][RW];
+    __shared__ double hs[RH][2 * kPyrTW];
+    __shared__ int ucol[2 * kPyrTW], vrow[2 * kPyrTH];
+    int tx, ty;
+    if (!xcd_tile((dw + kPyrTW - 1) / kPyrTW, (dh + kPyrTH - 1) / kPyrTH, tx, ty)) return;
+    const int j0 = tx * kPyrTW, i0 = ty * kPyrTH, tid = threadIdx.y * BX + threadIdx.x;
+    if (threadIdx.y == 0 && tid < 2 * kPyrTW) ucol[tid] = pyr_tap(min(j0 + (tid >> 1), dw - 1), xr, tid & 1, sw);
+    if (threadIdx.y == 1 && threadIdx.x < 2 * kPyrTH) vrow[threadIdx.x] = pyr_tap(min(i0 + ((int)threadIdx.x >> 1), dh - 1), yr, threadIdx.x & 1, sh);
+    __syncthreads();
+    const int xmin = ucol[0], ymin = vrow[0];
+    const int nx = ucol[2 * kPyrTW - 1] - xmin + 1 + 2 * F, ny = vrow[2 * kPyrTH - 1] - ymin + 1 + 2 * F;
+    if (nx > RW || ny > RH) return;
+    const double* plane = src + blockIdx.z * (size_t)sh * sw;
+    for (int r = threadIdx.y; r < ny; r += BY) {
+        const double* row = plane + (size_t)clampi(ymin - F + r, sh) * sw;
+        for (int cc = threadIdx.x; cc < nx; cc += BX) raw[r][cc] = row[clampi(xmin - F + cc, sw)];
+    }
+    __syncthreads();
+    {
+        const int q = tid & (2 * kPyrTW - 1), c = ucol[q] - xmin + F;
+        for (int r = tid / (2 * kPyrTW); r < ny; r += BX * BY / (2 * kPyrTW)) {
+            double acc = 0.0;
+#pragma unroll
+            for (int l = -F; l <= F; l++) acc += raw[r][c + l] * g.t[l + F];
+            hs[r][q] = acc;
+        }
+    }
+    __syncthreads();
+    if (tid >= kPyrTW * kPyrTH) return;
+    const int ox = tid % kPyrTW, oy = tid / kPyrTW, j = j0 + ox, i = i0 + oy;
+    if (j >= dw || i >= dh) return;
+    const double x = (double)(j + 1) / xr - 1;
+    const double y = (double)(i + 1) / yr - 1;
+    const BilinearTaps b = bilinear_taps(sw, sh, x, y);
+    double res = 0.0;
+#pragma unroll
+    for (int m = 0; m <= 1; m++)
+#pragma unroll
+        for (int n = 0; n <= 1; n++) {
+            const int rr = vrow[2 * oy + n] - ymin + F;
+            double acc = 0.0;
+#pragma unroll
+            for (int l = -F; l <= F; l++) acc += hs[rr + l][2 * ox + m] * g.t[l + F];
+            res += acc * b.s[m * 2 + n];
+        }
+    if (use_post) res *= post;
+    dst[blockIdx.z * (size_t)dh * dw + (size_t)i * dw + j] = res;
 }
 
 template <int C>
@@ -1374,7 +1440,14 @@
     if (do_warp) warp_pixel(im1, im2, warp, fu, fv, i, j, H, W, planes);
 }
 
-template <bool BATCH>
+__device__ __forceinline__ double central3(double a, double b, double c) {
+    double acc = 0.0;
+    acc += a * -0.5;
+    acc += b * 0.0;
+    acc += c * 0.5;
+    return acc;
+}
+template <bool BATCH, bool SELF = false>
 __global__ void k_bicubic(const double* __restrict__ im1, const double* __restrict__ im2,
                           const double* __restrict__ gx, const double* __restrict__ gy,
                           const double* __restrict__ gxy, const double* __restrict__ vx,
@@ -1384,9 +1457,11 @@
         const size_t p = blockIdx.y;
         const ptrdiff_t o1 = (ptrdiff_t)batch_frames(bk, p, im1, im2);
         const ptrdiff_t o2 = bk.bw != 0 && p >= bk.bw ? o1 - 2 * (ptrdiff_t)bk.fr : o1;
-        gx += o2;
-        gy += o2;
-        gxy += o2;
+        if (!SELF) {
+            gx += o2;
+            gy += o2;
+            gxy += o2;
+        }
         vx += p * bk.uv;
         vy += p * bk.uv;
         out += p * bk.out;
@@ -1421,12 +1496,40 @@
     const double dx2 = dx * dx, dy2 = dy * dy;
     const double dx3 = dx * dx2, dy3 = dy * dy2;
     const size_t a = (size_t)y0 * W + x0, b = (size_t)y0 * W + x1, c = (size_t)y1 * W + x0, d = (size_t)y1 * W + x1;
+    const int cols[4] = {clampi(x0 - 1, W), x0, x1, clampi(x1 + 1, W)};
+    const int rows[4] = {clampi(y0 - 1, H), y0, y1, clampi(y1 + 1, H)};
+    const bool sx = x1 == x0, sy = y1 == y0;
     for (int k = 0; k < C; k++) {
-        const double *f = im2 + k * np, *px = gx + k * np, *py = gy + k * np, *pz = gxy + k * np;
-        const double fA = f[a], fB = f[b], fC = f[c], fD = f[d];
-        const double xA = px[a], xB = px[b], xC = px[c], xD = px[d];
-        const double yA = py[a], yB = py[b], yC = py[c], yD = py[d];
-        const double zA = pz[a], zB = pz[b], zC = pz[c], zD = pz[d];
+        double fA, fB, fC, fD, xA, xB, xC, xD, yA, yB, yC, yD, zA, zB, zC, zD;
+        if constexpr (SELF) {
+            const double* f = im2 + k * np;
+            double i0[4], i1[4], gA[4], gB[4];
+#pragma unroll
+            for (int r = 0; r < 4; r++) {
+                const double* row = f + (size_t)rows[r] * W;
+                const double vm = row[cols[0]], vp = row[cols[3]];
+                i0[r] = row[cols[1]];
+                i1[r] = row[cols[2]];
+                gA[r] = central3(vm, i0[r], i1[r]);
+                gB[r] = central3(sx ? vm : i0[r], i1[r], vp);
+            }
+            fA = i0[1], fB = i1[1], fC = i0[2], fD = i1[2];
+            xA = gA[1], xB = gB[1], xC = gA[2], xD = gB[2];
+            yA = central3(i0[0], i0[1], i0[2]);
+            yB = central3(i1[0], i1[1], i1[2]);
+            yC = central3(sy ? i0[0] : i0[1], i0[2], i0[3]);
+            yD = central3(sy ? i1[0] : i1[1], i1[2], i1[3]);
+            zA = central3(gA[0], gA[1], gA[2]);
+            zB = central3(gB[0], gB[1], gB[2]);
+            zC = central3(sy ? gA[0] : gA[1], gA[2], gA[3]);
+            zD = central3(sy ? gB[0] : gB[1], gB[2], gB[3]);
+        } else {
+            const double *f = im2 + k * np, *px = gx + k * np, *py = gy + k * np, *pz = gxy + k * np;
+            fA = f[a], fB = f[b], fC = f[c], fD = f[d];
+            xA = px[a], xB = px[b], xC = px[c], xD = px[d];
+            yA = py[a], yB = py[b], yC = py[c], yD = py[d];
+            zA = pz[a], zB = pz[b], zC = pz[c], zD = pz[d];
+        }
         const double c00 = fA;
         const double c10 = xA;
         const double c20 = -3 * fA + 3 * fB - 2 * xA - xB;
@@ -1721,6 +1824,32 @@
     return PAPOF_OK;
 }
 
+bool pyramid_level_fused(int fsize, int sh, int sw, int dh, int dw, double rate) {
+    if (!PAPOF_V_PYRFUSED || fsize < 1 || fsize > 3 || dh < 1 || dw < 1) return false;
+    const auto fits = [&](int outputs, int tile, int n, int cap) {
+        for (int o0 = 0; o0 < outputs; o0 += tile) {
+            const int last = std::min(o0 + tile, outputs) - 1;
+            if (pyr_tap(last, rate, 1, n) - pyr_tap(o0, rate, 0, n) + 1 + 2 * fsize > cap) return false;
+        }
+        return true;
+    };
+    return fits(dw, kPyrTW, sw, pyr_span(kPyrTW, fsize)) && fits(dh, kPyrTH, sh, pyr_span(kPyrTH, fsize));
+}
+
+int pyramid_level(papof_handle* h, const double* src, double* dst, int sh, int sw, int planes, int dh, int dw, double rate,
+                  const Taps& g, bool use_post, double post) {
+    if (!pyramid_level_fused(g.fsize, sh, sw, dh, dw, rate)) return PAPOF_EINVAL;
+    const dim3 grid(xcd_grid((dw + kPyrTW - 1) / kPyrTW, (dh + kPyrTH - 1) / kPyrTH), 1, planes), block(BX, BY);
+    if (g.fsize == 1)
+        hipLaunchKernelGGL(k_pyramid_level<1>, grid, block, 0, h->stream, src, dst, sh, sw, dh, dw, rate, rate, g, use_post ? 1 : 0, post);
+    else if (g.fsize == 2)
+        hipLaunchKernelGGL(k_pyramid_level<2>, grid, block, 0, h->stream, src, dst, sh, sw, dh, dw, rate, rate, g, use_post ? 1 : 0, post);
+    else
+        hipLaunchKernelGGL(k_pyramid_level<3>, grid, block, 0, h->stream, src, dst, sh, sw, dh, dw, rate, rate, g, use_post ? 1 : 0, post);
+    LAUNCH_CHECK();
+    return PAPOF_OK;
+}
+
 int im2feature(papof_handle* h, const double* im, double* feat, int H, int W, int C, unsigned* nz, int frames, size_t nz_stride) {
     const size_t np = (size_t)H * W;
     if (C == 3) {
@@ -1938,7 +2067,10 @@
     const Rect r = region(rc, W, H);
     if (r.empty()) return PAPOF_OK;
     const BatchK bk0{0, 0, 0, 0, 0, 0};
-    hipLaunchKernelGGL(batch > 1 ? k_bicubic<true> : k_bicubic<false>, dim3(xcd_grid((r.x1 - r.x0 + BX - 1) / BX, (r.y1 - r.y0 + BY - 1) / BY), batch), dim3(BX, BY), 0, h->stream, im1, im2, gx, gy, gxy, vx, vy, out_hwc, H, W,
+    const auto kernel = gx ? (batch > 1 ? k_bicubic<true, false> : k_bicubic<false, false>)
+                           : (batch > 1 ? k_bicubic<true, true> : k_bicubic<false, true>);
+    if (!gx && !PAPOF_V_BICSELF) return PAPOF_EINVAL;
+    hipLaunchKernelGGL(kernel, dim3(xcd_grid((r.x1 - r.x0 + BX - 1) / BX, (r.y1 - r.y0 + BY - 1) / BY), batch), dim3(BX, BY), 0, h->stream, im1, im2, gx, gy, gxy, vx, vy, out_hwc, H, W,
                        C, r, take_stamp(h), planar_out ? 1 : 0, clamp ? 1 : 0, bk ? *bk : bk0);
     LAUNCH_CHECK();
     return PAPOF_OK;
```

Result: no change. 206.7, median of 6 (+0.5%).
